# rustformers/llm

Hardware: AMD Instinct MI355X
Metric: decode tokens/s LLaMA-7B Q4_0 (higher is better)
Workload: dtype i8*i4->i32 block dots, f32 accumulate (W4A8 = ggml's Q4_0·Q8_0)

## Files before the change

### include/ggml_hip.h

```cpp
#ifndef GGML_HIP_H
#define GGML_HIP_H

#include <stdbool.h>
#include <stddef.h>
#include <stdint.h>

#ifdef __cplusplus
extern "C" {
#endif

#define GGML_API __attribute__((visibility("default")))

#define GGML_FILE_MAGIC 0x67676d6c
#define GGML_FILE_VERSION 1
#define GGML_QNT_VERSION 2
#define GGML_QNT_VERSION_FACTOR 1000
#define GGML_MAX_DIMS 4
#define GGML_MAX_NODES 4096
#define GGML_MAX_PARAMS 256
#define GGML_MAX_CONTEXTS 64
#define GGML_MAX_SRC 6
#define GGML_MAX_NAME 48
#define GGML_MAX_OP_PARAMS 32
#define GGML_DEFAULT_N_THREADS 4
// ... 358 lines not shown
GGML_API size_t ggml_hip_mul_mat_get_wsize(const struct ggml_tensor *src0, const struct ggml_tensor *src1,
                                           struct ggml_tensor *dst);
GGML_API void ggml_hip_mul_mat(const struct ggml_tensor *src0, const struct ggml_tensor *src1,
                               struct ggml_tensor *dst, void *wdata, size_t wsize);
GGML_API void *ggml_hip_host_malloc(size_t size);
GGML_API void ggml_hip_host_free(void *ptr);
GGML_API void ggml_hip_transform_tensor(void *data, struct ggml_tensor *tensor);
GGML_API void ggml_hip_free_data(struct ggml_tensor *tensor);
GGML_API void ggml_hip_assign_buffers(struct ggml_tensor *tensor);
GGML_API void ggml_hip_assign_buffers_no_scratch(struct ggml_tensor *tensor);
GGML_API void ggml_hip_assign_buffers_force_inplace(struct ggml_tensor *tensor);
GGML_API void ggml_hip_set_main_device(int main_device);
GGML_API void ggml_hip_set_mul_mat_q(bool mul_mat_q);
GGML_API void ggml_hip_set_scratch_size(size_t scratch_size);
GGML_API void ggml_hip_free_scratch(void);
GGML_API bool ggml_hip_compute_forward(struct ggml_compute_params *params, struct ggml_tensor *tensor);

GGML_API void ggml_init_cublas(void);
GGML_API void ggml_cuda_set_tensor_split(const float *tensor_split);
GGML_API void ggml_cuda_mul(const struct ggml_tensor *, const struct ggml_tensor *, struct ggml_tensor *);
GGML_API bool ggml_cuda_can_mul_mat(const struct ggml_tensor *, const struct ggml_tensor *, struct ggml_tensor *);
GGML_API size_t ggml_cuda_mul_mat_get_wsize(const struct ggml_tensor *, const struct ggml_tensor *,
                                            struct ggml_tensor *);
GGML_API void ggml_cuda_mul_mat(const struct ggml_tensor *, const struct ggml_tensor *, struct ggml_tensor *,
                                void *, size_t);
GGML_API void *ggml_cuda_host_malloc(size_t size);
GGML_API void ggml_cuda_host_free(void *ptr);
GGML_API void ggml_cuda_transform_tensor(void *data, struct ggml_tensor *tensor);
GGML_API void ggml_cuda_free_data(struct ggml_tensor *tensor);
GGML_API void ggml_cuda_assign_buffers(struct ggml_tensor *tensor);
GGML_API void ggml_cuda_assign_buffers_no_scratch(struct ggml_tensor *tensor);
GGML_API void ggml_cuda_assign_buffers_force_inplace(struct ggml_tensor *tensor);
GGML_API void ggml_cuda_set_main_device(int main_device);
GGML_API void ggml_cuda_set_mul_mat_q(bool mul_mat_q);
GGML_API void ggml_cuda_set_scratch_size(size_t scratch_size);
GGML_API void ggml_cuda_free_scratch(void);
GGML_API bool ggml_cuda_compute_forward(struct ggml_compute_params *params, struct ggml_tensor *tensor);

GGML_API int ggml_hip_device_count(void);
GGML_API int ggml_hip_slot_physical_device(int slot);
GGML_API int ggml_hip_thread_session_slot(void);
GGML_API int ggml_hip_get_main_device(void);
GGML_API void ggml_hip_bind_thread_device(int device);
GGML_API int ggml_hip_thread_pinned_device(void);
GGML_API void ggml_hip_unbind_thread_device(void);
GGML_API int ggml_hip_get_tensor_split(float *out, int cap);
GGML_API void ggml_hip_set_layer_split(const float *fractions, int n);
GGML_API int ggml_hip_get_layer_split(float *out, int cap);
GGML_API void ggml_hip_copy_between_devices(int dst_device, void *dst, int src_device, const void *src, size_t nbytes);
GGML_API void ggml_hip_synchronize(void);
GGML_API void ggml_hip_tensor_get(const struct ggml_tensor *tensor, void *host_dst, size_t offset, size_t nbytes);
GGML_API void ggml_hip_tensor_set(struct ggml_tensor *tensor, const void *host_src, size_t offset, size_t nbytes);
GGML_API void ggml_hip_memcpy(void *dst, const void *src, size_t nbytes, int kind);
GGML_API void *ggml_hip_tensor_device_ptr(const struct ggml_tensor *tensor);
enum ggml_hip_kclass {
    GGML_HIP_KCLASS_MMVQ = 0,
    GGML_HIP_KCLASS_MMQ_MFMA,
    GGML_HIP_KCLASS_ATTN,
    GGML_HIP_KCLASS_OTHER,
    GGML_HIP_KCLASS_COUNT
};
GGML_API void ggml_hip_timing_begin(void);
GGML_API void ggml_hip_timing_end(void);
GGML_API void ggml_hip_timing_query(int kclass, double *ms, int64_t *launches, double *algo_bytes);
GGML_API void ggml_hip_set_option(const char *key, int value);
GGML_API int ggml_hip_get_option(const char *key);
#define GGML_HIP_KKIND_BASE 16
GGML_API int ggml_hip_bench_plan_class(int kclass, int replays, double *ms_total, int64_t *launches_per_replay,
                                       double *algo_bytes_per_replay);
#define GGML_HIP_COMM_ID_BYTES 128
GGML_API int ggml_hip_comm_unique_id(void *id_out );
GGML_API int ggml_hip_comm_init(int rank, int world, const void *id);
GGML_API void ggml_hip_comm_destroy(void);
GGML_API int ggml_hip_comm_ranks(void);
GGML_API void ggml_hip_comm_send(const void *dev_src, size_t nbytes, int peer);
GGML_API void ggml_hip_comm_recv(void *dev_dst, size_t nbytes, int peer);
GGML_API void ggml_hip_comm_sendrecv(const void *dev_src, int send_peer, void *dev_dst, int recv_peer, size_t nbytes);
GGML_API int ggml_hip_bench_empty(int wgs, int threads, int lds_bytes, int kernarg_bytes, int n_launch, int replays,
                                  double *out);
GGML_API int64_t ggml_hip_get_stat(const char *key);
GGML_API int ggml_hip_graph_compute_begin(struct ggml_cgraph *cgraph);
GGML_API void ggml_hip_graph_compute_end(void);
GGML_API int ggml_hip_graph_prepare(struct ggml_cgraph *cgraph);
GGML_API int ggml_hip_decode_greedy_chain(struct ggml_cgraph *last, int n, int32_t *out_tokens, float *last_logits);
GGML_API int ggml_hip_decode_batch(struct ggml_cgraph *const *graphs, int n_graphs);
GGML_API int ggml_hip_topk(const struct ggml_tensor *t, int64_t row, int k, const int32_t *extra_ids, int n_extra,
                           float *out_vals, int32_t *out_ids);
GGML_API int ggml_hip_row_probs(const struct ggml_tensor *logits, int64_t row_begin, int64_t n_rows, const int32_t *targets,
                                float *out_probs);
GGML_API size_t ggml_hip_quantize(enum ggml_type type, const float *src, void *dst, int64_t n, int64_t k, int64_t *hist);
GGML_API int ggml_hip_quantize_resident(const struct ggml_tensor *src, struct ggml_tensor *dst, int64_t *hist);
GGML_API size_t ggml_hip_read_timeline(int64_t *dst, size_t max_records);
GGML_API int ggml_hip_debug_prompt_attention(const float *q, const uint16_t *mem_k, const uint16_t *mem_v, float *out, int N, int E,
                                             int Egqa, int H, int n_past, int64_t C, float scale, int fused);
GGML_API int ggml_hip_debug_prompt_attention_plan(const float *q_raw, const float *q_raw2, const float *rope, const uint16_t *mem_k,
                                                  const uint16_t *mem_v, uint16_t *x16, float *out, int N, int E, int Egqa, int H,
                                                  int n_past, int64_t C, float scale, int f16d);
GGML_API int ggml_hip_debug_exp_le0(uint16_t *out_fast, uint16_t *out_ref);
GGML_API int ggml_hip_debug_mul_mat_cols(const struct ggml_tensor *w, const float *x, float *out, int N);
GGML_API int ggml_hip_debug_mat_vec_big(const struct ggml_tensor *w0, const struct ggml_tensor *w1, const struct ggml_tensor *w2,
                                        int xsrc, int epi, const float *x, const float *norm_w, float eps, const float *res, float *out,
                                        float *y_out, int n_past, int D, float freq_base, float freq_scale, int64_t C,
                                        uint16_t *mem_k, uint16_t *mem_v);
GGML_API int ggml_hip_debug_mat_vec_kbig(const struct ggml_tensor *w0, const struct ggml_tensor *w1, const struct ggml_tensor *w2,
                                         int xsrc, int epi, const float *x, const float *xw, float eps, const float *res, float *out,
                                         float *y_out, int n_past, int D, float freq_base, float freq_scale, int64_t C,
                                         uint16_t *mem_k, uint16_t *mem_v);
GGML_API int ggml_hip_debug_mat_vec_f16(const struct ggml_tensor *w0, const struct ggml_tensor *w1, const struct ggml_tensor *w2,
                                        int xsrc, int epi, const float *x, const float *xw, float eps, const float *res, float *out,
                                        float *y_out, int n_past, int D, float freq_base, float freq_scale, int64_t C,
                                        uint16_t *mem_k, uint16_t *mem_v, int ncols);
GGML_API int ggml_hip_share_stream(int slot, int with_slot);
GGML_API const char *ggml_hip_version(void);

#ifdef __cplusplus
}
#endif

#ifdef __cplusplus
#define GGML_ABI_ASSERT(c, m) static_assert(c, m)
#else
#define GGML_ABI_ASSERT(c, m) _Static_assert(c, m)
#endif
GGML_ABI_ASSERT(sizeof(struct ggml_object) == 32, "ggml_object size (lib.rs:239)");
GGML_ABI_ASSERT(offsetof(struct ggml_object, type) == 24, "ggml_object.type");
GGML_ABI_ASSERT(sizeof(struct ggml_tensor) == 272, "ggml_tensor size (lib.rs:446)");
GGML_ABI_ASSERT(offsetof(struct ggml_tensor, ne) == 16, "ggml_tensor.ne");
GGML_ABI_ASSERT(offsetof(struct ggml_tensor, nb) == 48, "ggml_tensor.nb");
GGML_ABI_ASSERT(offsetof(struct ggml_tensor, op) == 80, "ggml_tensor.op");
GGML_ABI_ASSERT(offsetof(struct ggml_tensor, op_params) == 84, "ggml_tensor.op_params");
GGML_ABI_ASSERT(offsetof(struct ggml_tensor, is_param) == 116, "ggml_tensor.is_param");
GGML_ABI_ASSERT(offsetof(struct ggml_tensor, grad) == 120, "ggml_tensor.grad");
GGML_ABI_ASSERT(offsetof(struct ggml_tensor, src) == 128, "ggml_tensor.src");
GGML_ABI_ASSERT(offsetof(struct ggml_tensor, perf_runs) == 176, "ggml_tensor.perf_runs");
GGML_ABI_ASSERT(offsetof(struct ggml_tensor, data) == 200, "ggml_tensor.data");
GGML_ABI_ASSERT(offsetof(struct ggml_tensor, name) == 208, "ggml_tensor.name");
GGML_ABI_ASSERT(offsetof(struct ggml_tensor, extra) == 256, "ggml_tensor.extra");
GGML_ABI_ASSERT(offsetof(struct ggml_tensor, padding) == 264, "ggml_tensor.padding");
GGML_ABI_ASSERT(sizeof(struct ggml_cplan) == 16424, "ggml_cplan size");
GGML_ABI_ASSERT(offsetof(struct ggml_cplan, n_tasks) == 20, "ggml_cplan.n_tasks");
GGML_ABI_ASSERT(offsetof(struct ggml_cplan, abort_callback) == 16408, "ggml_cplan.abort_callback");
GGML_ABI_ASSERT(sizeof(struct ggml_cgraph) == 164520, "ggml_cgraph size (lib.rs:651)");
GGML_ABI_ASSERT(offsetof(struct ggml_cgraph, nodes) == 8, "ggml_cgraph.nodes");
GGML_ABI_ASSERT(offsetof(struct ggml_cgraph, leafs) == 65544, "ggml_cgraph.leafs");
GGML_ABI_ASSERT(offsetof(struct ggml_cgraph, visited_hash_table) == 98312, "ggml_cgraph.visited_hash_table");
GGML_ABI_ASSERT(offsetof(struct ggml_cgraph, perf_runs) == 164496, "ggml_cgraph.perf_runs");
GGML_ABI_ASSERT(sizeof(struct ggml_scratch) == 24, "ggml_scratch size");
GGML_ABI_ASSERT(sizeof(struct ggml_init_params) == 24, "ggml_init_params size");
GGML_ABI_ASSERT(sizeof(struct ggml_compute_params) == 32, "ggml_compute_params size");
GGML_ABI_ASSERT(offsetof(struct ggml_compute_params, wsize) == 16, "ggml_compute_params.wsize");
GGML_ABI_ASSERT(sizeof(ggml_type_traits_t) == 40, "ggml_type_traits_t size");

#endif
```

### llm_amd/csrc/backend_executor.inc

```
bool is_view_op(ggml_op op) {
    return op == GGML_OP_NONE || op == GGML_OP_RESHAPE || op == GGML_OP_VIEW || op == GGML_OP_PERMUTE ||
           op == GGML_OP_TRANSPOSE;
}

struct GraphInfo {
    std::vector<int> n_uses;
};

int node_index(const ggml_cgraph *gr, const ggml_tensor *t, const std::map<const ggml_tensor *, int> &idx) {
    (void)gr;
    auto it = idx.find(t);
    return it == idx.end() ? -1 : it->second;
}

void stage_add_target(ggml_tensor *leaf) {
    const uintptr_t p = (uintptr_t)leaf->data;
    const size_t nbytes = ggml_nbytes(leaf);
    for (const Staged &st : g_staged)
        if (st.host == p && st.nbytes == nbytes) return;
    bool offloaded = extra_of(leaf) != nullptr;
    for (auto &kv : g.tensors)
        if (kv.second->host < p + nbytes && p < kv.second->host + std::max<size_t>(kv.second->nbytes, 1)) offloaded = true;
    if (offloaded)
        die("add: tensor '%s' (%s) was offloaded to the device before being patched; LoRA adapters are applied at load time, "
// ... 31 lines not shown
                free_dev_tensor(e);
            } else {
                continue;
            }
        }
        Arena *hdr = find_arena((uintptr_t)leaf);
        const bool per_eval = r0 && hdr == r0;
        if (per_eval) {
            const size_t nbytes = ggml_nbytes(leaf);
            if (nbytes == 0) continue;
            h2d_small(dev_ptr(leaf), leaf->data, nbytes);
        } else {
            upload_tensor(leaf->data, leaf, false, true)->owner_hdr = (uintptr_t)leaf;
        }
    }
}

bool mirrored_to_host(const ggml_tensor *n) {
    if (n->backend != GGML_BACKEND_CPU || is_view_op(n->op) || n->op == GGML_OP_CPY) return false;
    if (!ggml_is_contiguous(n) || n->data == nullptr) return false;
    return !(extra_of(n) || find_tensor((uintptr_t)n->data));
}

static inline uint64_t now_ns() {
    return (uint64_t)std::chrono::duration_cast<std::chrono::nanoseconds>(
               std::chrono::steady_clock::now().time_since_epoch()).count();
}
void download_outputs(ggml_cgraph *gr) {
    const uint64_t t0 = now_ns();
    bool any = false;
    for (int i = 0; i < gr->n_nodes; i++) {
        ggml_tensor *n = gr->nodes[i];
        if (!mirrored_to_host(n)) continue;
        d2h_queue(n->data, dev_ptr(n), ggml_nbytes(n));
        g.stat_mirror_bytes += ggml_nbytes(n);
        any = true;
    }
    (void)any;
    d2h_finish();
    g.ns_mirror += now_ns() - t0;
}

void invalidate_xf16_if_overwritten_impl(const ggml_tensor *n);
void invalidate_qact_if_overwritten(const ggml_tensor *n) {
    if (g_xi8.valid && n->data != nullptr) {
        const uintptr_t c0 = (uintptr_t)g_xi8.src_data, c1 = c0 + g_xi8.src_bytes;
        const uintptr_t b0 = (uintptr_t)n->data, b1 = b0 + ggml_nbytes(n);
        if (b0 < c1 && c0 < b1) g_xi8.valid = false;
    }
    if (g_xk.valid && n->data != nullptr) {
        const uintptr_t c0 = (uintptr_t)g_xk.src_data, c1 = c0 + g_xk.src_bytes;
        const uintptr_t b0 = (uintptr_t)n->data, b1 = b0 + ggml_nbytes(n);
        if (b0 < c1 && c0 < b1) g_xk.valid = false;
    }
    invalidate_xf16_if_overwritten_impl(n);
    if (!g_qact.valid || n->data == nullptr) return;
    const uintptr_t a0 = (uintptr_t)g_qact.src_data, a1 = a0 + g_qact.src_bytes;
    const uintptr_t b0 = (uintptr_t)n->data, b1 = b0 + ggml_nbytes(n);
    if (b0 < a1 && a0 < b1) g_qact.valid = false;
}
void invalidate_xf16_if_overwritten_impl(const ggml_tensor *n) {
    if (!g_xf16.valid || n->data == nullptr) return;
    const uintptr_t a0 = (uintptr_t)g_xf16.src_data, a1 = a0 + g_xf16.src_bytes;
    const uintptr_t b0 = (uintptr_t)n->data, b1 = b0 + ggml_nbytes(n);
    if (b0 < a1 && a0 < b1) g_xf16.valid = false;
}

#include "plan_shapes.inc"
#include "plan_match.inc"
#include "plan_build.inc"
#include "plan_decode.inc"
#include "plan_prompt.inc"
#include "plan_run.inc"

void execute_graph(ggml_cgraph *gr) {
    ensure_init();
    finish_pending();
    ws_reset();
    g_qact.valid = false;
    g_xf16.valid = false;
    g_xi8.valid = false;
    g_xk.valid = false;
    if (try_decode_plan(gr)) return;
    g.stat_generic_graphs++;
    upload_inputs(gr);

    std::map<const ggml_tensor *, int> idx;
    std::vector<int> uses(gr->n_nodes, 0);
    for (int i = 0; i < gr->n_nodes; i++) idx[gr->nodes[i]] = i;
    for (int i = 0; i < gr->n_nodes; i++)
        for (int s = 0; s < GGML_MAX_SRC; s++)
            if (gr->nodes[i]->src[s]) {
                int j = node_index(gr, gr->nodes[i]->src[s], idx);
                if (j >= 0) uses[j]++;
            }
    std::vector<char> done(gr->n_nodes, 0);
    const bool fuse = g.opt_fuse != 0;
    std::vector<int> deferred_silu(gr->n_nodes, -1);
    if (fuse) {
        for (int j = 0; j < gr->n_nodes; j++) {
            ggml_tensor *mu = gr->nodes[j];
            if (mu->op != GGML_OP_MUL || !mu->src[0] || mu->src[0]->op != GGML_OP_UNARY) continue;
            const int i = node_index(gr, mu->src[0], idx);
            ggml_tensor *un = mu->src[0];
            if (i < 0 || i >= j || uses[i] != 1 || un->op_params[0] != GGML_UNARY_OP_SILU) continue;
            if (!is_contig_f32(un->src[0]) || !is_contig_f32(mu->src[1]) || !is_contig_f32(mu) ||
                ggml_nelements(mu->src[1]) != ggml_nelements(un) || ggml_nelements(mu) != ggml_nelements(un))
                continue;
            deferred_silu[i] = j;
        }
    }

    for (int i = 0; i < gr->n_nodes; i++) {
        ggml_tensor *n = gr->nodes[i];
        if (done[i] || is_view_op(n->op)) continue;
        invalidate_qact_if_overwritten(n);
        ggml_tensor *next = i + 1 < gr->n_nodes ? gr->nodes[i + 1] : nullptr;
        switch (n->op) {
            case GGML_OP_GET_ROWS: op_get_rows(n); break;
            case GGML_OP_RMS_NORM: {
                if (fuse && next && next->op == GGML_OP_MUL && next->src[0] == n && uses[i] == 1 && !done[i + 1] &&
                    is_contig_f32(next->src[1]) && ggml_nelements(next->src[1]) == n->ne[0] && next->nb[0] == 4) {
                    invalidate_qact_if_overwritten(next);
                    op_rms_norm(n, next->src[1], next);
                    done[i + 1] = 1;
                } else {
                    op_rms_norm(n, nullptr, n);
                }
            } break;
            case GGML_OP_NORM: op_norm(n); break;
            case GGML_OP_ADD: {
                if (n->src[0]->type == GGML_TYPE_F32)
                    op_bin(n, BIN_ADD);
                else
                    op_add_lowp(n);
            } break;
            case GGML_OP_MUL: {
                const int si = n->src[0] && n->src[0]->op == GGML_OP_UNARY ? node_index(gr, n->src[0], idx) : -1;
                if (si >= 0 && deferred_silu[si] == i)
                    op_unary(n->src[0], n->src[1], n);
                else
                    op_bin(n, BIN_MUL);
            } break;
            case GGML_OP_REPEAT: op_bin(n, BIN_REPEAT); break;
            case GGML_OP_UNARY: {
                if (deferred_silu[i] >= 0) break;
                if (fuse && n->op_params[0] == GGML_UNARY_OP_SILU && next && next->op == GGML_OP_MUL &&
                    next->src[0] == n && uses[i] == 1 && !done[i + 1] && is_contig_f32(next->src[1]) &&
                    ggml_nelements(next->src[1]) == ggml_nelements(n) && is_contig_f32(next)) {
                    invalidate_qact_if_overwritten(next);
                    op_unary(n, next->src[1], next);
                    done[i + 1] = 1;
                } else {
                    op_unary(n, nullptr, n);
                }
            } break;
            case GGML_OP_MUL_MAT: op_mul_mat(n); break;
            case GGML_OP_SCALE: {
                ggml_tensor *n1 = next, *n2 = i + 2 < gr->n_nodes ? gr->nodes[i + 2] : nullptr;
                ggml_tensor *n3 = i + 3 < gr->n_nodes ? gr->nodes[i + 3] : nullptr;
                if (fuse && n1 && n2 && n1->op == GGML_OP_DIAG_MASK_INF && n1->src[0] == n && n2->op == GGML_OP_SOFT_MAX &&
                    n2->src[0] == n1 && uses[i] == 1 && uses[i + 1] == 1 && n->data == n->src[0]->data &&
                    n1->data == n->data && n2->data == n->data && is_contig_f32(n)) {
                    op_scale_mask_softmax(n->src[0], n->src[1], (int)n1->op_params[0], n2);
                    done[i + 1] = done[i + 2] = 1;
                } else if (fuse && n1 && n2 && n3 && n1->op == GGML_OP_ALIBI && n1->src[0] == n &&
// ... 30 lines not shown
```

### llm_amd/csrc/backend_state.inc

```

[[noreturn]] void die(const char *fmt, ...) {
    char buf[1024];
    va_list ap;
    va_start(ap, fmt);
    vsnprintf(buf, sizeof(buf), fmt, ap);
    va_end(ap);
    fatal_note("%s", buf);
    abort();
}

int g_cur_slot();
struct Arena {
    uintptr_t base = 0;
    size_t size = 0;
    char *dev = nullptr;
    bool live = true;
    bool is_scratch = false;
};

struct DevTensor {
    uint32_t magic = 0x48495054;
    int slot = (int)(g_cur_slot());
    uintptr_t host = 0;
    size_t nbytes = 0;
    char *dev = nullptr;
    size_t dev_bytes = 0;
    bool soa = false;
    bool auto_uploaded = false;
    int refs = 1;
    bool zero_filled = false;
    uintptr_t owner_hdr = 0;
    QWeight qw{};
    char *w16 = nullptr;
    size_t w16_size = 0;
    bool ksoa = false;
    KWeight kw{};
    ggml_type type = GGML_TYPE_F32;
    int64_t ne[4] = {0, 0, 0, 0};
};

struct Timing {
    bool on = false;
    struct Rec {
        hipEvent_t a, b;
    };
    std::vector<Rec> recs[GGML_HIP_KCLASS_COUNT];
    std::vector<Rec> pool;
    double bytes[GGML_HIP_KCLASS_COUNT] = {0, 0, 0, 0};
    int64_t launches[GGML_HIP_KCLASS_COUNT] = {0, 0, 0, 0};
};

#define GGML_HIP_MAX_BACKENDS 16
struct Backend {
    int slot = 0;
    bool inited = false;
    int device = 0;
    hipStream_t stream = nullptr;
    hipStream_t own_stream = nullptr;
    std::recursive_mutex mu;
    hipEvent_t xfer_ev = nullptr;
    int opt_fuse_heads = 1, opt_attn_one = 1, opt_attn_split = 1;
    std::map<uintptr_t, Arena> arenas;
    std::map<uintptr_t, DevTensor *> tensors;
    std::map<uintptr_t, DevTensor *> auto_tensors;
    struct WsChunk {
        char *p;
        size_t size;
    };
    std::vector<WsChunk> ws_chunks;
    size_t ws_off = 0;
    Timing timing;
    int opt_fuse = 1, opt_plan = 1, opt_plan_k = 1, opt_plan_multi = 1, opt_plan_prompt = 1, opt_graph = 1, opt_big = 1, opt_kbig = 1;
    int opt_chain_k = 0, opt_prepare = 1, opt_plan_batch = 1, opt_plan_f16 = 1;
    int opt_fuse_attn = 1, opt_fuse_wo = 1, opt_warm_mb = 24, opt_affine = 1;
    int opt_act_quant = 0, opt_mmq_i8 = 0;
    int opt_mmq_min = 32, opt_k_prompt_min = 12, opt_mmq_fuse = 3, opt_mmq_cols = 1, opt_mmq_t256 = 1, opt_attn_fused = 1;
    int opt_mmq_w16 = 1, opt_w16_headroom_gb = 16;
    int opt_probe = 0;
    std::atomic<size_t> w16_bytes{0};
    uint64_t w16_gen = 1;
    int num_cus = 256;
    long long *timeline = nullptr;
    size_t timeline_bytes = 0;
    int timeline_wgs = 4;
    uint64_t stat_plan_tokens = 0, stat_generic_graphs = 0, stat_split_tokens = 0, stat_prompt_plan_tokens = 0, stat_fused_tokens = 0, stat_kplan_tokens = 0, stat_fused_heads_tokens = 0, stat_fused_wo_tokens = 0, stat_fused_affine_tokens = 0, stat_prepared_tokens = 0;
    uint64_t stat_alibi_fused = 0;
    uint64_t stat_batch_tokens = 0, stat_batch_steps = 0;
    uint64_t stat_flash_attn_nodes = 0;
    enum { MMQ_K_PLAIN, MMQ_K_DMA_P8, MMQ_K_W16_P8, MMQ_K_W16_256, MMQ_K_I8, MMQ_K_COUNT };
    uint64_t stat_mmq[MMQ_K_COUNT] = {0, 0, 0, 0, 0};
    void *chain_plan = nullptr;
    ggml_cgraph *chain_graph = nullptr;
    bool pending_wait = false;
    bool pending_light = false;
    int opt_speculate_next = 0;
    struct Spec {
        bool pending = false;
        void *plan = nullptr;
        int n_past = 0, av = 0;
        int32_t *tok_pin = nullptr;
        int *tok_dev = nullptr;
        hipEvent_t tok_ev = nullptr;
        int cooldown = 0;
    } spec;
    hipEvent_t results_ev = nullptr;
    bool results_ev_armed = false;
    size_t results_ev_copies = 0;
    uint64_t stat_spec_hits = 0, stat_spec_misses = 0;
    unsigned *ferr_pin = nullptr;
    void *ferr_plan = nullptr;
    int opt_fused_fallback = 1, opt_fused_rearm_tokens = 256;
    uint64_t fused_rearm_at = 0;
    uint64_t fused_rearm_stretch = 0;
    int fused_saved_fuse_attn = 0, fused_saved_attn_one = 0;
    uint64_t stat_fused_rearms = 0;
    uint64_t stat_cols_warm_launches = 0;
    int opt_test_fused_timeout = 0;
    uint64_t stat_fused_timeouts = 0;
    uint64_t ns_match = 0, ns_launch = 0, ns_wait = 0, ns_compute = 0, ns_mirror = 0, stat_mirror_bytes = 0;
    size_t dead_shadow_bytes = 0;
    uint64_t arena_seen = 0;
    void *prep = nullptr;
    int opt_gen = 0;
    int xcd_labels = -1;
    void *hot_line = nullptr;
    int session_records = 0;
};
enum : unsigned {
    OPT_ENV = 1,
    OPT_DROPS = 2,
    OPT_DEVICE = 4,
    OPT_ACTION = 8,
};
enum OptEffect { FX_NONE, FX_ACT_QUANT, FX_TIMELINE, FX_MMQ_W16, FX_W16_RELEASE, FX_FUSE_ATTN, FX_SPECULATE_NEXT, FX_FUSED_REARM_TOKENS, FX_TEST_FUSED_TIMEOUT, FX_SERIAL_STAGE_SLOTS };
struct OptRow {
    const char *key;
    int Backend::*field;
    unsigned flags;
    OptEffect fx = FX_NONE;
    int lo = 0, hi = -1;
};
static const OptRow g_options[] = {
    {"fuse", &Backend::opt_fuse, OPT_ENV},
    {"plan", &Backend::opt_plan, OPT_ENV},
    {"plan_k", &Backend::opt_plan_k, OPT_ENV | OPT_DROPS},
    {"plan_f16", &Backend::opt_plan_f16, OPT_ENV | OPT_DROPS},
    {"plan_multi", &Backend::opt_plan_multi, OPT_ENV | OPT_DROPS},
    {"plan_prompt", &Backend::opt_plan_prompt, OPT_ENV | OPT_DROPS},
    {"plan_batch", &Backend::opt_plan_batch, OPT_ENV | OPT_DROPS},
    {"graph", &Backend::opt_graph, OPT_ENV},
    {"big", &Backend::opt_big, OPT_ENV | OPT_DROPS},
    {"kbig", &Backend::opt_kbig, OPT_ENV | OPT_DROPS},
    {"chain_k", &Backend::opt_chain_k, OPT_ENV, FX_NONE, 0, 64},
    {"prepare", &Backend::opt_prepare, OPT_ENV},
    {"speculate_next", &Backend::opt_speculate_next, OPT_ENV, FX_SPECULATE_NEXT},
    {"fuse_attn", &Backend::opt_fuse_attn, OPT_ENV | OPT_DROPS, FX_FUSE_ATTN},
    {"fuse_wo", &Backend::opt_fuse_wo, OPT_ENV | OPT_DROPS},
    {"warm_mb", &Backend::opt_warm_mb, OPT_ENV | OPT_DROPS},
    {"affine", &Backend::opt_affine, OPT_ENV | OPT_DROPS},
    {"fuse_heads", &Backend::opt_fuse_heads, OPT_ENV | OPT_DROPS},
    {"attn_split", &Backend::opt_attn_split, OPT_ENV | OPT_DROPS},
    {"attn_one", &Backend::opt_attn_one, OPT_ENV | OPT_DROPS},
    {"fused_fallback", &Backend::opt_fused_fallback, OPT_ENV},
    {"fused_rearm_tokens", &Backend::opt_fused_rearm_tokens, OPT_ENV, FX_FUSED_REARM_TOKENS},
    {"act_quant", &Backend::opt_act_quant, OPT_ENV | OPT_DEVICE, FX_ACT_QUANT},
    {"mmq_i8", &Backend::opt_mmq_i8, OPT_ENV},
    {"mmq_min", &Backend::opt_mmq_min, OPT_ENV},
    {"k_prompt_min", &Backend::opt_k_prompt_min, OPT_ENV},
    {"mmq_fuse", &Backend::opt_mmq_fuse, OPT_ENV},
    {"mmq_cols", &Backend::opt_mmq_cols, OPT_ENV | OPT_DROPS},
    {"mmq_t256", &Backend::opt_mmq_t256, OPT_ENV | OPT_DROPS},
    {"attn_fused", &Backend::opt_attn_fused, OPT_ENV},
    {"mmq_w16", &Backend::opt_mmq_w16, OPT_ENV | OPT_DROPS | OPT_DEVICE, FX_MMQ_W16},
    {"w16_headroom_gb", &Backend::opt_w16_headroom_gb, OPT_ENV},
    {"w16_release", nullptr, OPT_DEVICE | OPT_ACTION, FX_W16_RELEASE},
    {"serial_stage_slots", nullptr, 0, FX_SERIAL_STAGE_SLOTS},
    {"timeline", nullptr, OPT_DEVICE, FX_TIMELINE},
    {"probe", &Backend::opt_probe, OPT_DROPS},
    {"test_fused_timeout", &Backend::opt_test_fused_timeout, OPT_DROPS, FX_TEST_FUSED_TIMEOUT},
};
const OptRow &opt_row(const char *key, const char *who) {
    for (const OptRow &o : g_options)
        if (!strcmp(o.key, key)) return o;
    die("%s: unknown key '%s'", who, key);
}
inline int opt_value(const OptRow &o, int v) {
    if (o.fx == FX_ACT_QUANT) return v ? 1 : 0;
    return o.lo <= o.hi ? std::min(o.hi, std::max(o.lo, v)) : v;
}
struct StatRow {
    const char *key;
    uint64_t Backend::*field;
};
static const StatRow g_counters[] = {
    {"plan_tokens", &Backend::stat_plan_tokens},
    {"fused_attn_tokens", &Backend::stat_fused_tokens},
    {"fused_heads_tokens", &Backend::stat_fused_heads_tokens},
    {"fused_wo_tokens", &Backend::stat_fused_wo_tokens},
    {"fused_affine_tokens", &Backend::stat_fused_affine_tokens},
    {"attn_split_tokens", &Backend::stat_split_tokens},
    {"kplan_tokens", &Backend::stat_kplan_tokens},
    {"prepared_tokens", &Backend::stat_prepared_tokens},
    {"prompt_plan_tokens", &Backend::stat_prompt_plan_tokens},
    {"batch_decode_tokens", &Backend::stat_batch_tokens},
    {"batch_decode_steps", &Backend::stat_batch_steps},
    {"cols_warm_launches", &Backend::stat_cols_warm_launches},
    {"fused_rearms", &Backend::stat_fused_rearms},
    {"spec_hits", &Backend::stat_spec_hits},
    {"spec_misses", &Backend::stat_spec_misses},
    {"generic_graphs", &Backend::stat_generic_graphs},
    {"alibi_fused", &Backend::stat_alibi_fused},
    {"flash_attn_nodes", &Backend::stat_flash_attn_nodes},
    {"ns_match", &Backend::ns_match},
    {"ns_launch", &Backend::ns_launch},
    {"ns_wait", &Backend::ns_wait},
    {"ns_compute", &Backend::ns_compute},
    {"ns_mirror", &Backend::ns_mirror},
    {"mirror_bytes", &Backend::stat_mirror_bytes},
};
std::recursive_mutex g_mu;
std::map<std::string, int> g_opt_log;
float g_tensor_split[GGML_HIP_MAX_BACKENDS] = {1.0f};
float g_layer_split[GGML_HIP_MAX_BACKENDS] = {0.0f};
int g_layer_split_n = 0;
Backend g_backends[GGML_HIP_MAX_BACKENDS];
std::atomic<int> g_default_slot{0};
std::atomic<int> g_dev_slots[64];
std::atomic<uint64_t> g_dev_gen[64];
std::atomic<uint64_t> g_dev_wgen[64];
thread_local Backend *g_cur = &g_backends[0];
thread_local bool tl_pinned = false;
#define g (*g_cur)
int g_cur_slot() { return (int)(g_cur - g_backends); }
std::atomic<int> g_dev_serial_stages[64];
inline int device_sharers() {
    const int n = g_dev_slots[g.device & 63].load(std::memory_order_relaxed), ser = g_dev_serial_stages[g.device & 63].load(std::memory_order_relaxed);
    return std::max(1, n - (ser > 1 ? std::min(ser, n) - 1 : 0));
}
inline int device_siblings() {
    int n = 0;
    for (int i = 0; i < GGML_HIP_MAX_BACKENDS; i++)
        if (&g_backends[i] != g_cur && g_backends[i].inited && g_backends[i].device == g.device) n++;
    return n;
}
void bind_device();
void sync_arenas();
std::atomic<int> g_calls_inside{0}, g_calls_inside_peak{0};
thread_local int tl_lock_depth = 0;
struct SlotLock {
    Backend *b;
    void enter() {
        b->mu.lock();
        if (tl_lock_depth++ == 0) {
            const int n = g_calls_inside.fetch_add(1, std::memory_order_relaxed) + 1;
            int peak = g_calls_inside_peak.load(std::memory_order_relaxed);
            while (n > peak && !g_calls_inside_peak.compare_exchange_weak(peak, n, std::memory_order_relaxed)) {}
        }
    }
    SlotLock() {
        if (!tl_pinned) g_cur = &g_backends[g_default_slot.load(std::memory_order_relaxed)];
        b = g_cur;
        enter();
        if (b->inited) bind_device();
        sync_arenas();
    }
    explicit SlotLock(Backend *slot) : b(slot) { enter(); }
    ~SlotLock() {
        if (--tl_lock_depth == 0) g_calls_inside.fetch_sub(1, std::memory_order_relaxed);
        b->mu.unlock();
    }
    SlotLock(const SlotLock &) = delete;
    SlotLock &operator=(const SlotLock &) = delete;
};
struct DevOnce {
    bool done[GGML_HIP_MAX_BACKENDS] = {};
    bool first() {
        bool &d = done[g.slot];
        if (d) return false;
        d = true;
        return true;
    }
};
template <auto Kern>
void lds_opt_in(size_t launch_lds, size_t max_bytes) {
    static DevOnce opted;
    if (launch_lds > 64 * 1024 && opted.first())
        HIP_CHECK(hipFuncSetAttribute((const void *)Kern, hipFuncAttributeMaxDynamicSharedMemorySize, (int)max_bytes));
}

int kt_of(ggml_type t) {
    switch (t) {
        case GGML_TYPE_Q2_K: return KT_Q2_K;
// ... 392 lines not shown
}

void h2d_bulk(char *dst, const void *src, size_t n) {
    staging_init();
    size_t off = 0;
    while (off < n) {
        const int b = stg.next;
        stg.next ^= 1;
        if (stg.busy[b]) {
            HIP_CHECK(hipEventSynchronize(stg.ev[b]));
            stg.busy[b] = false;
        }
        const size_t len = std::min(Staging::BIG, n - off);
        memcpy(stg.big[b], (const char *)src + off, len);
        HIP_CHECK(hipMemcpyAsync(dst + off, stg.big[b], len, hipMemcpyHostToDevice, g.stream));
        HIP_CHECK(hipEventRecord(stg.ev[b], g.stream));
        stg.busy[b] = true;
        off += len;
    }
}
void h2d_small(char *dst, const void *src, size_t n) {
    staging_init();
    const size_t need = (n + 63) & ~(size_t)63;
    if (stg.small_off + need > Staging::SMALL) {
        h2d_bulk(dst, src, n);
        return;
    }
    char *s = stg.small + stg.small_off;
    stg.small_off += need;
    memcpy(s, src, n);
    HIP_CHECK(hipMemcpyAsync(dst, s, n, hipMemcpyHostToDevice, g.stream));
}
void d2h_queue(void *host_dst, const char *src, size_t n) {
    staging_init();
    const size_t need = (n + 63) & ~(size_t)63;
    if (stg.small_off + need > Staging::SMALL) {
        const size_t PIECE = (size_t)8 << 20;
        for (int i = 0; i < 2; i++)
            if (stg.busy[i]) {
                HIP_CHECK(hipEventSynchronize(stg.ev[i]));
                stg.busy[i] = false;
            }
        auto par_copy = [](char *dst, const char *src_, size_t len) {
            const int nt = len >= ((size_t)2 << 20) ? 4 : 1;
            if (nt == 1) {
                memcpy(dst, src_, len);
                return;
            }
            std::thread th[3];
            const size_t part = (len / nt + 63) & ~(size_t)63;
            for (int t = 1; t < nt; t++) {
                const size_t o = (size_t)t * part;
                if (o < len) th[t - 1] = std::thread([=] { memcpy(dst + o, src_ + o, std::min(part, len - o)); });
            }
            memcpy(dst, src_, std::min(part, len));
            for (int t = 1; t < nt; t++)
                if (th[t - 1].joinable()) th[t - 1].join();
        };
        size_t off = 0;
        int cur = 0;
        size_t len = std::min(PIECE, n);
        HIP_CHECK(hipMemcpyAsync(stg.big[cur], src, len, hipMemcpyDeviceToHost, g.stream));
        HIP_CHECK(hipEventRecord(stg.ev[cur], g.stream));
        while (off < n) {
            const size_t noff = off + len, nlen = noff < n ? std::min(PIECE, n - noff) : 0;
            if (nlen) {
                HIP_CHECK(hipMemcpyAsync(stg.big[cur ^ 1], src + noff, nlen, hipMemcpyDeviceToHost, g.stream));
                HIP_CHECK(hipEventRecord(stg.ev[cur ^ 1], g.stream));
            }
            HIP_CHECK(hipEventSynchronize(stg.ev[cur]));
            par_copy((char *)host_dst + off, stg.big[cur], len);
            off = noff;
            len = nlen;
            cur ^= 1;
        }
        return;
    }
    char *s = stg.small + stg.small_off;
    stg.small_off += need;
    HIP_CHECK(hipMemcpyAsync(s, src, n, hipMemcpyDeviceToHost, g.stream));
    stg.pending.push_back({host_dst, s, n});
}
void d2h_finish() {
    if (g.results_ev_armed && stg.pending.size() != g.results_ev_copies) g.results_ev_armed = false;
    if (g.results_ev_armed) {
        g.results_ev_armed = false;
        HIP_CHECK(hipEventSynchronize(g.results_ev));
    } else {
        HIP_CHECK(hipStreamSynchronize(g.stream));
    }
    for (auto &p : stg.pending) memcpy(p.host_dst, p.stage, p.n);
    stg.pending.clear();
    stg.small_off = 0;
    stg.busy[0] = stg.busy[1] = false;
}

struct Timed {
    int k;
    Timing::Rec rec{};
    bool on;
    Timed(int kclass, double algo_bytes) : k(kclass), on(g.timing.on) {
        if (!on) return;
        if (!g.timing.pool.empty()) {
            rec = g.timing.pool.back();
            g.timing.pool.pop_back();
        } else {
            HIP_CHECK(hipEventCreate(&rec.a));
            HIP_CHECK(hipEventCreate(&rec.b));
        }
        HIP_CHECK(hipEventRecord(rec.a, g.stream));
        g.timing.bytes[k] += algo_bytes;
        g.timing.launches[k]++;
    }
    ~Timed() {
        if (!on) return;
        HIP_CHECK(hipEventRecord(rec.b, g.stream));
        g.timing.recs[k].push_back(rec);
    }
};

inline dim3 grid1(int64_t n, int bs = 256) { return dim3((unsigned)((n + bs - 1) / bs)); }
```

### llm_amd/csrc/backend_tools.inc

```
namespace {
template <int NARG>
struct EmptyArgs {
    long long *ts;
    int idx;
    int pad[(NARG - 12) / 4];
};
template <int NARG>
__global__ void __launch_bounds__(1024) k_empty(const EmptyArgs<NARG> a, int last_arg) {
    extern __shared__ __attribute__((aligned(16))) char smem[];
    long long t0;
    asm volatile("s_memrealtime %0\n\ts_waitcnt lgkmcnt(0)" : "=s"(t0));
    const int v = a.pad[(NARG - 12) / 4 - 1] + last_arg;
    long long t1 = v != 0x7fffffff ? (long long)wall_clock64() : 0;
    if (v == 0x12345678) smem[threadIdx.x] = 1;
    if (threadIdx.x == 0 && blockIdx.x == 0) {
        a.ts[a.idx * 4] = t0;
        a.ts[a.idx * 4 + 1] = t1;
        a.ts[a.idx * 4 + 2] = (long long)wall_clock64();
    }
}
template <int NARG>
void empty_launch(int wgs, int threads, int lds, long long *ts, int idx) {
    EmptyArgs<NARG> a;
    memset(&a, 0, sizeof(a));
// ... 403 lines not shown
        qa.rope = rope; qa.prm = prm; qa.mem_k = (__half *)dk; qa.mem_v = (__half *)dv; qa.Egqa = Ms[1]; qa.C = C; qa.D = D;
        float *ds3[3] = {(float *)dout, nullptr, nullptr};
        const int kinds[3] = {0, 1, 2};
        launch_f16(3, fw, ds3, K, src, nullptr, ncols, KE_QKV, &qa, kinds);
    } else if (epi == KE_GATE) {
        float *ds2[2] = {(float *)dout, nullptr};
        launch_f16(2, fw, ds2, K, src, nullptr, ncols, KE_GATE);
    } else if (nw == 1) {
        float *ds1[1] = {(float *)dout};
        launch_f16(1, fw, ds1, K, src, (const float *)dres, ncols);
    } else {
        float *ds[3] = {nullptr, nullptr, nullptr};
        for (int i = 0; i < nw; i++) ds[i] = (float *)debug_buf((size_t)ncols * Ms[i] * 4, nullptr, owned);
        launch_f16(nw, fw, ds, K, src, nullptr, ncols);
        int64_t at = 0;
        for (int i = 0; i < nw; i++) {
            HIP_CHECK(hipMemcpy2DAsync(dout + at * 4, (size_t)Mrow * 4, ds[i], (size_t)Ms[i] * 4, (size_t)Ms[i] * 4, (size_t)ncols, hipMemcpyDeviceToDevice, g.stream));
            at += Ms[i];
        }
    }
    if (dy && epi != KE_ROW) {
        float *ds1[1] = {(float *)debug_buf((size_t)ncols * Ms[0] * 4, nullptr, owned)};
        launch_f16(1, fw, ds1, K, RowSrc{KX_NORM, (const float *)dx, (const float *)dxw, eps, (float *)dy}, nullptr, ncols);
    }
    d2h_queue(out, dout, n_out + DEBUG_GUARD);
    if (dy) d2h_queue(y_out, dy, nx + DEBUG_GUARD);
    if (dk) {
        d2h_queue(mem_k, dk, nkv + DEBUG_GUARD);
        d2h_queue(mem_v, dv, nkv + DEBUG_GUARD);
    }
    d2h_finish();
    for (char *b : owned) HIP_CHECK(hipFree(b));
    return 0;
}

int ggml_hip_debug_prompt_attention_plan(const float *q_raw, const float *q_raw2, const float *rope, const uint16_t *mem_k,
                                         const uint16_t *mem_v, uint16_t *x16, float *out, int N, int E, int Egqa, int H, int n_past,
                                         int64_t C, float scale, int f16d) {
    SlotLock lk;
    ensure_init();
    finish_pending();
    if (!q_raw || !rope || !mem_k || !mem_v || !x16 || N < 1 || H < 1 || E % H || n_past < 0) return -1;
    const int64_t D = E / H, T = (int64_t)n_past + N;
    if (Egqa < D || Egqa % D || H % (Egqa / D) || T > C || C % 8 || !prompt_attn_fits(D, T)) return -1;
    const int64_t Hkv = Egqa / D;
    std::vector<char *> owned;
    const size_t nq = (size_t)N * E * 4, nkv = (size_t)C * Egqa * 2, nx = (size_t)N * E * 2;
    char *dq = debug_buf(nq * (q_raw2 ? 2 : 1), nullptr, owned);
    h2d_bulk(dq, q_raw, nq);
    if (q_raw2) h2d_bulk(dq + nq, q_raw2, nq);
    char *dr = debug_buf((size_t)N * 128 * 4, rope, owned);
    char *dk = debug_buf(nkv, mem_k, owned), *dv = debug_buf(nkv, mem_v, owned);
    char *dx = debug_buf(nx, nullptr, owned), *dout = debug_buf(nq, nullptr, owned);
    prompt_attention(true, (const float *)dq, (const __half *)dk, (const __half *)dv, (float *)dout, nullptr, nullptr, N, E, Egqa, H, Hkv,
                     D, n_past, C, scale, (_Float16 *)dx, f16d != 0, (const float *)dr, q_raw2 ? (int64_t)N * E : 0);
    d2h_queue(x16, dx, nx + DEBUG_GUARD);
    if (out) d2h_queue(out, dout, nq + DEBUG_GUARD);
    d2h_finish();
    for (char *b : owned) HIP_CHECK(hipFree(b));
    return 0;
}

__global__ void __launch_bounds__(256) k_debug_exp_le0(uint16_t *out_fast, uint16_t *out_ref) {
    const unsigned i = blockIdx.x * 256 + threadIdx.x;
    const float x = __half2float(__ushort_as_half((unsigned short)i));
    out_fast[i] = __half_as_ushort(__float2half_rn(exp_le0(x)));
    out_ref[i] = __half_as_ushort(__float2half_rn(expf(x)));
}
int ggml_hip_debug_exp_le0(uint16_t *out_fast, uint16_t *out_ref) {
    SlotLock lk;
    ensure_init();
    finish_pending();
    uint16_t *d;
    dev_malloc((void **)&d, 2 * 65536 * 2, "debug exp");
    hipLaunchKernelGGL(k_debug_exp_le0, dim3(256), dim3(256), 0, g.stream, d, d + 65536);
    HIP_CHECK(hipGetLastError());
    HIP_CHECK(hipStreamSynchronize(g.stream));
    HIP_CHECK(hipMemcpy(out_fast, d, 65536 * 2, hipMemcpyDeviceToHost));
    HIP_CHECK(hipMemcpy(out_ref, d + 65536, 65536 * 2, hipMemcpyDeviceToHost));
    HIP_CHECK(hipFree(d));
    return 0;
}

int ggml_hip_decode_greedy_chain(struct ggml_cgraph *last, int n, int32_t *out_tokens, float *last_logits) {
    SlotLock lk;
    return decode_greedy_chain(last, n, out_tokens, last_logits);
}

int ggml_hip_decode_batch(struct ggml_cgraph *const *graphs, int n_graphs) {
    if (!graphs || n_graphs < 2 || n_graphs > BATCH_COLS_MAX) return -1;
    for (int i = 0; i < n_graphs; i++)
        if (!graphs[i]) return -1;
    SlotLock lk;
    const uint64_t t0 = now_ns();
    const int r = decode_batch(graphs, n_graphs);
    g.ns_compute += now_ns() - t0;
    return r;
}

int64_t ggml_hip_get_stat(const char *key) {
    SlotLock lk;
    for (const StatRow &c : g_counters)
        if (!strcmp(c.key, key)) return (int64_t)(g.*c.field);
    const std::string k(key);
    if (k == "w16_bytes") return (int64_t)g.w16_bytes;
    if (k.rfind("mmq_launches_", 0) == 0) {
        static const char *names[Backend::MMQ_K_COUNT] = {"plain", "dma_p8", "w16_p8", "w16_256", "i8"};
        for (int i = 0; i < Backend::MMQ_K_COUNT; i++)
            if (k.substr(13) == names[i]) return (int64_t)g.stat_mmq[i];
        return -1;
    }
    if (k == "graph_replays") {
        int64_t n = 0;
        for (auto *p : g_plans) n += (int64_t)p->replays;
        return n;
    }
    if (k == "plans") return (int64_t)g_plans.size();
    if (k == "num_cus") {
        ensure_init();
        return (int64_t)g.num_cus;
    }
    if (k == "fused_attn_timeouts") {
        int64_t n = (int64_t)g.stat_fused_timeouts;
        if (g.inited) HIP_CHECK(hipStreamSynchronize(g.stream));
        if (g.ferr_pin) n += *(volatile unsigned *)g.ferr_pin;
        return n;
    }
    if (k == "peak_concurrent_calls") return (int64_t)g_calls_inside_peak.load();
    return -1;
}
size_t ggml_hip_read_timeline(int64_t *dst, size_t max_records) {
    SlotLock lk;
    if (!g.timeline) return 0;
    const size_t n = std::min(max_records, g.timeline_bytes / 64);
    HIP_CHECK(hipStreamSynchronize(g.stream));
    HIP_CHECK(hipMemcpy(dst, g.timeline, n * 64, hipMemcpyDeviceToHost));
    return n;
}
const char *ggml_hip_version(void) { return "libggml_hip 0.1 (gfx950)"; }

}
```

### llm_amd/csrc/hip_backend.hip

```cpp
#include <hip/hip_runtime.h>

#include <algorithm>
#include <atomic>
#include <cctype>
#include <chrono>
#include <cmath>
#include <cstdarg>
#include <cstdio>
#include <cstdlib>
#include <cstring>
#include <deque>
#include <map>
#include <mutex>
#include <string>
#include <thread>
#include <vector>

#include "ggml_hip.h"
#include "internal.h"
#include "kernels/common.h"
#include "kernels/mmvq.h"
#include "kernels/mmq.h"
#include "kernels/mmq_plain.h"
#include "kernels/mmq_dmap8.h"
// ... 71 lines not shown
        DevTensor *e = it->second;
        it = g.auto_tensors.erase(it);
        destroy_record(e);
    }
}
void register_arena_here(void *host_base, size_t size, int is_scratch) {
    const uintptr_t b = (uintptr_t)host_base;
    if (size == 0) return;
    auto it = g.arenas.find(b);
    if (it != g.arenas.end() && it->second.size == size) {
        if (!it->second.live && it->second.dev) g.dead_shadow_bytes -= it->second.size;
        if (!it->second.live) evict_overlapping(g.auto_tensors, b, size);
        it->second.live = true;
        return;
    }
    for (auto jt = g.arenas.begin(); jt != g.arenas.end();) {
        Arena &a = jt->second;
        if (a.base < b + size && b < a.base + a.size) {
            if (a.dev) {
                if (g.stream) HIP_CHECK(hipStreamSynchronize(g.stream));
                HIP_CHECK(hipFree(a.dev));
                if (!a.live) g.dead_shadow_bytes -= a.size;
            }
            jt = g.arenas.erase(jt);
        } else {
            ++jt;
        }
    }
    evict_overlapping(g.auto_tensors, b, size);
    Arena a;
    a.base = b;
    a.size = size;
    a.is_scratch = is_scratch != 0;
    g.arenas[b] = a;
}

void unregister_arena_here(void *host_base) {
    const uintptr_t b = (uintptr_t)host_base;
    auto it = g.arenas.find(b);
    if (it == g.arenas.end()) return;
    Arena &a = it->second;
    evict_overlapping(g.auto_tensors, a.base, a.size);
    for (auto jt = g.auto_tensors.begin(); jt != g.auto_tensors.end();) {
        DevTensor *e = jt->second;
        if (e->owner_hdr >= a.base && e->owner_hdr < a.base + a.size) {
            jt = g.auto_tensors.erase(jt);
            destroy_record(e);
        } else {
            ++jt;
        }
    }
    a.live = false;
    if (a.dev) {
        g.dead_shadow_bytes += a.size;
        if (g.dead_shadow_bytes > ((size_t)8 << 30)) {
            if (g.stream) HIP_CHECK(hipStreamSynchronize(g.stream));
            for (auto jt = g.arenas.begin(); jt != g.arenas.end();) {
                if (!jt->second.live) {
                    if (jt->second.dev) HIP_CHECK(hipFree(jt->second.dev));
                    jt = g.arenas.erase(jt);
                } else {
                    ++jt;
                }
            }
            g.dead_shadow_bytes = 0;
        }
    } else {
        g.arenas.erase(it);
    }
}

}

extern "C" void ggml_hip_internal_graph_compute(struct ggml_cgraph *cgraph) {
    SlotLock lk;
    const uint64_t t0 = now_ns();
    execute_graph(cgraph);
    g.ns_compute += now_ns() - t0;
}
extern "C" int ggml_hip_graph_compute_begin(struct ggml_cgraph *cgraph) {
    SlotLock lk;
    const uint64_t t0 = now_ns();
    ensure_init();
    if (g.pending_wait && g.pending_light && stg.pending.empty() && !g.results_ev_armed) {
        g.pending_wait = false;
        g.ferr_plan = nullptr;
    } else {
        finish_pending();
    }
    ws_reset();
    g_qact.valid = false;
    g_xf16.valid = false;
    g_xi8.valid = false;
    g_xk.valid = false;
    int async = 0;
    if (try_decode_plan(cgraph, true)) {
        async = 1;
    } else {
        execute_graph(cgraph);
    }
    g.ns_compute += now_ns() - t0;
    return async;
}
extern "C" int ggml_hip_graph_prepare(struct ggml_cgraph *cgraph) {
    SlotLock lk;
    ensure_init();
    return prepare_decode_plan(cgraph) ? 1 : 0;
}
extern "C" void ggml_hip_graph_compute_end(void) {
    SlotLock lk;
    const uint64_t t0 = now_ns();
    finish_pending();
    g.ns_compute += now_ns() - t0;
}

extern "C" {

void ggml_init_hipblas(void) {
    SlotLock lk;
    ensure_init();
}
void ggml_hip_set_main_device(int main_device) {
    if (main_device < 0 || main_device >= std::max(1, slot_count()))
        die("ggml_hip_set_main_device(%d): %d device slot(s) available", main_device, slot_count());
    g_default_slot.store(main_device, std::memory_order_relaxed);
    if (tl_auto_slot >= 0 && slot_physical_device(tl_auto_slot) == slot_physical_device(main_device)) {
        ggml_hip_bind_thread_device(tl_auto_slot);
        return;
    }
    ggml_hip_bind_thread_device(main_device);
}
static void auto_session_slot() {
    const int n = std::min(session_slots_env(), slot_count());
    if (n <= 1 || tl_auto_slot >= 0) return;
    if (!tl_pinned) g_cur = &g_backends[g_default_slot.load(std::memory_order_relaxed)];
    const int cur = (int)(g_cur - g_backends), phys = slot_physical_device(cur);
    int best = cur;
    {
        std::lock_guard<std::recursive_mutex> lk(g_mu);
        for (int i = 0; i < n; i++)
            if (slot_physical_device(i) == phys && g_session_threads[i] < g_session_threads[best]) best = i;
        g_session_threads[best]++;
        tl_auto_slot = best;
        (void)&tl_auto_release;
    }
    if (best != cur) ggml_hip_bind_thread_device(best);
    else tl_pinned = true, g_cur = &g_backends[cur];
}
int ggml_hip_thread_session_slot(void) { return tl_auto_slot; }
void ggml_hip_bind_thread_device(int device) {
    if (device < 0 || device >= std::max(1, slot_count()))
        die("ggml_hip_bind_thread_device(%d): %d device slot(s) available", device, slot_count());
    tl_pinned = true;
    g_cur = &g_backends[device];
    SlotLock lk(g_cur);
    g.slot = device;
    if (g.inited) bind_device();
}
int ggml_hip_thread_pinned_device(void) { return tl_pinned ? (int)(g_cur - g_backends) : -1; }
void ggml_hip_unbind_thread_device(void) {
    tl_pinned = false;
    g_cur = &g_backends[g_default_slot.load(std::memory_order_relaxed)];
}
void ggml_hip_set_tensor_split(const float *tensor_split) {
    std::lock_guard<std::recursive_mutex> lk(g_mu);
    for (int i = 0; i < GGML_HIP_MAX_BACKENDS; i++) g_tensor_split[i] = 0.0f;
    g_tensor_split[0] = tensor_split ? tensor_split[0] : 0.0f;
}
int ggml_hip_get_tensor_split(float *out, int cap) {
    std::lock_guard<std::recursive_mutex> lk(g_mu);
    const int n = std::min(cap, GGML_HIP_MAX_BACKENDS);
    for (int i = 0; i < n; i++) out[i] = g_tensor_split[i];
    return std::min(n, 1);
}
void ggml_hip_set_layer_split(const float *fractions, int n) {
    std::lock_guard<std::recursive_mutex> lk(g_mu);
    g_layer_split_n = fractions && n > 0 ? std::min(n, GGML_HIP_MAX_BACKENDS) : 0;
    for (int i = 0; i < GGML_HIP_MAX_BACKENDS; i++) g_layer_split[i] = i < g_layer_split_n ? fractions[i] : 0.0f;
}
int ggml_hip_get_layer_split(float *out, int cap) {
    std::lock_guard<std::recursive_mutex> lk(g_mu);
    const int n = std::min(cap, g_layer_split_n);
    for (int i = 0; i < n; i++) out[i] = g_layer_split[i];
    return n;
}
void ggml_hip_set_mul_mat_q(bool) {}
void ggml_hip_set_scratch_size(size_t) {}
void ggml_hip_free_scratch(void) {
    SlotLock lk;
    if (!g.inited) return;
// ... 82 lines not shown
    const int64_t cap = std::min(nblocks, piece);
    dev_malloc((void **)&din, (size_t)cap * qk * 4, "the quantizer input");
    dev_malloc((void **)&dout, (size_t)cap * bs, "the quantizer output");
    HIP_CHECK(hipMalloc((void **)&dh, 128));
    HIP_CHECK(hipMemsetAsync(dh, 0, 128, g.stream));
    for (int64_t b0 = 0; b0 < nblocks; b0 += piece) {
        const int64_t nb = std::min(piece, nblocks - b0);
        h2d_bulk(din, src + b0 * qk, (size_t)nb * qk * 4);
        if (kt >= 0)
            launch_quantize_k(din, false, kt, nb, (uint8_t *)dout);
        else
            launch_quantize_blocks(din, false, (int)type, nb, (uint8_t *)dout, dh);
        d2h_queue((char *)dst + (size_t)b0 * bs, dout, (size_t)nb * bs);
        d2h_finish();
    }
    unsigned long long hh[16];
    HIP_CHECK(hipMemcpy(hh, dh, 128, hipMemcpyDeviceToHost));
    if (hist)
        for (int i = 0; i < 16; i++) hist[i] += (int64_t)hh[i];
    HIP_CHECK(hipFree(din));
    HIP_CHECK(hipFree(dout));
    HIP_CHECK(hipFree(dh));
    return (size_t)nblocks * bs;
}
int ggml_hip_quantize_resident(const struct ggml_tensor *src, struct ggml_tensor *dst, int64_t *hist) {
    SlotLock lk;
    ensure_init();
    if (!quantizable(dst->type) || (src->type != GGML_TYPE_F32 && src->type != GGML_TYPE_F16)) return -1;
    if (!ggml_is_contiguous(src) || src->ne[2] != 1 || src->ne[3] != 1 || src->ne[0] % 32 != 0 || src->ne[0] != dst->ne[0] ||
        src->ne[1] != dst->ne[1] || dst->ne[2] != 1 || dst->ne[3] != 1 || extra_of(dst) || dst->data == nullptr)
        return -1;
    if (!extra_of(src) && !find_tensor((uintptr_t)src->data)) return -1;
    finish_pending();
    const int64_t M = src->ne[1], nb = src->ne[0] / 32, nblocks = M * nb;
    const size_t bs = ggml_type_size(dst->type);
    char *raw = nullptr;
    unsigned long long *dh = nullptr;
    dev_malloc((void **)&raw, (size_t)nblocks * bs, "the resident quantizer output");
    HIP_CHECK(hipMalloc((void **)&dh, 128));
    HIP_CHECK(hipMemsetAsync(dh, 0, 128, g.stream));
    launch_quantize_blocks(dev_ptr(src), src->type == GGML_TYPE_F16, (int)dst->type, nblocks, (uint8_t *)raw, dh);
    DevTensor *e = new DevTensor();
    e->host = (uintptr_t)dst->data;
    e->nbytes = ggml_nbytes(dst);
    e->type = dst->type;
    for (int i = 0; i < 4; i++) e->ne[i] = dst->ne[i];
    const int qt = qt_of(dst->type);
    size_t off[5];
    const size_t total = qw_layout(qt, M, nb, off);
    dev_malloc((void **)&e->dev, total, "a weight tensor");
    e->dev_bytes = total;
    relayout_launch(raw, qt, M, nb, e->dev);
    unsigned long long hh[16];
    HIP_CHECK(hipMemcpyAsync(hh, dh, 128, hipMemcpyDeviceToHost, g.stream));
    HIP_CHECK(hipStreamSynchronize(g.stream));
    if (hist)
        for (int i = 0; i < 16; i++) hist[i] += (int64_t)hh[i];
    HIP_CHECK(hipFree(raw));
    HIP_CHECK(hipFree(dh));
    e->soa = true;
    e->qw = qw_at(e->dev, qt, M, nb);
    evict_overlapping(g.auto_tensors, e->host, std::max<size_t>(e->nbytes, 1));
    evict_overlapping(g.tensors, e->host, std::max<size_t>(e->nbytes, 1));
    g.tensors[e->host] = e;
    dst->backend = GGML_BACKEND_GPU;
    dst->extra = e;
    return 0;
}

int ggml_hip_topk(const struct ggml_tensor *t, int64_t row, int k, const int32_t *extra_ids, int n_extra, float *out_vals,
                  int32_t *out_ids) {
    SlotLock lk;
    ensure_init();
    if (!t || t->type != GGML_TYPE_F32 || t->nb[0] != 4 || row < 0 || row >= t->ne[1] * t->ne[2] * t->ne[3] || t->ne[2] != 1 ||
        t->ne[3] != 1 || k < 1 || k > TOPK_MAX || k > t->ne[0] || n_extra < 0 || t->ne[0] > 0x7FFFFFFF || !out_vals || !out_ids ||
        (n_extra > 0 && !extra_ids) || t->data == nullptr)
        return -1;
    {
        DevTensor *e = extra_of(t);
        if (!e) e = find_tensor((uintptr_t)t->data);
        if (e ? e->soa : find_arena((uintptr_t)t->data) == nullptr) return -1;
    }
    finish_pending();
    const float *x = (const float *)(dev_ptr(t) + row * (int64_t)t->nb[1]);
    char *buf = ws_alloc((size_t)(k + n_extra) * 8 + (size_t)n_extra * 4 + 64);
    float *dv = (float *)buf;
    int *di = (int *)(buf + (size_t)(k + n_extra) * 4);
    int *de = di + (k + n_extra);
    if (n_extra) h2d_small((char *)de, extra_ids, (size_t)n_extra * 4);
    {
        Timed tm(GGML_HIP_KCLASS_OTHER, (double)t->ne[0] * 4 * 9);
        hipLaunchKernelGGL(k_topk, dim3(1), dim3(1024), 0, g.stream, x, (int)t->ne[0], k, (const int *)de, n_extra, dv, di);
        HIP_CHECK(hipGetLastError());
    }
    d2h_queue(out_vals, (const char *)dv, (size_t)(k + n_extra) * 4);
    d2h_queue(out_ids, (const char *)di, (size_t)(k + n_extra) * 4);
    d2h_finish();
    return 0;
}

int ggml_hip_row_probs(const struct ggml_tensor *t, int64_t row_begin, int64_t n_rows, const int32_t *targets, float *out_probs) {
    if (!t || !targets || !out_probs || n_rows < 1 || row_begin < 0 || t->type != GGML_TYPE_F32 || t->nb[0] != 4 || t->ne[2] != 1 ||
        t->ne[3] != 1 || t->ne[0] < 1 || t->ne[0] > (1 << 30) || n_rows > t->ne[1] || row_begin > t->ne[1] - n_rows ||
        n_rows > 0x7FFFFFFF || t->nb[1] % 4 != 0 || t->nb[1] < (size_t)t->ne[0] * 4 || t->data == nullptr)
        return -1;
    for (int64_t r = 0; r < n_rows; r++)
        if (targets[r] < 0 || targets[r] >= t->ne[0]) return -1;
    SlotLock lk;
    ensure_init();
    {
        DevTensor *e = extra_of(t);
        if (!e) e = find_tensor((uintptr_t)t->data);
        if (e ? e->soa : find_arena((uintptr_t)t->data) == nullptr) return -1;
    }
    finish_pending();
    const float *x = (const float *)(dev_ptr(t) + row_begin * (int64_t)t->nb[1]);
    const int V = (int)t->ne[0];
    char *buf = ws_alloc((size_t)n_rows * 8 + 64);
    float *dp = (float *)buf;
    int *dt = (int *)(buf + (size_t)n_rows * 4);
    h2d_small((char *)dt, targets, (size_t)n_rows * 4);
    {
        Timed tm(GGML_HIP_KCLASS_OTHER, (double)n_rows * V * 4);
        const long long stride = (long long)(t->nb[1] / 4);
        const bool keep = V <= ROW_PROB_KEEP * 1024, vec = keep && V % 4 == 0 && stride % 4 == 0 && (uintptr_t)x % 16 == 0;
        auto kern = vec ? k_row_prob<true, true> : keep ? k_row_prob<true, false> : k_row_prob<false, false>;
        hipLaunchKernelGGL(kern, dim3((unsigned)n_rows), dim3(1024), 0, g.stream, x, stride, V, (const int *)dt, dp);
        HIP_CHECK(hipGetLastError());
    }
    d2h_queue(out_probs, (const char *)dp, (size_t)n_rows * 4);
    d2h_finish();
    return 0;
}

void ggml_hip_free_data(struct ggml_tensor *tensor) {
    if (!tensor || !tensor->extra) return;
    DevTensor *e = (DevTensor *)tensor->extra;
    if (e->magic != 0x48495054) return;
    const int owner = (e->slot >= 0 && e->slot < GGML_HIP_MAX_BACKENDS) ? e->slot : g_cur_slot();
    SlotLock lk(&g_backends[owner]);
    free_dev_tensor(e);
    tensor->extra = nullptr;
}
void ggml_hip_assign_buffers(struct ggml_tensor *tensor) {
    tensor->backend = GGML_BACKEND_GPU;
}
void ggml_hip_assign_buffers_force_inplace(struct ggml_tensor *tensor) { tensor->backend = GGML_BACKEND_GPU; }
void ggml_hip_assign_buffers_no_scratch(struct ggml_tensor *tensor) {
    if (tensor->op == GGML_OP_NONE && !tensor->extra) auto_session_slot();
    SlotLock lk;
    tensor->backend = GGML_BACKEND_GPU;
    if (tensor->op != GGML_OP_NONE || extra_of(tensor)) return;
    tensor->extra = upload_tensor(tensor->data, tensor, true);
}
bool ggml_hip_can_mul_mat(const struct ggml_tensor *src0, const struct ggml_tensor *src1, struct ggml_tensor *dst) {
    bool q = src0->type == GGML_TYPE_F16 || src0->type == GGML_TYPE_F32;
    if (qt_of(src0->type) >= 0) q = src0->ne[0] % 32 == 0;
    if (kt_of(src0->type) >= 0) q = src0->ne[0] % 256 == 0;
    return q && src1->type == GGML_TYPE_F32 && dst->type == GGML_TYPE_F32;
}
size_t ggml_hip_mul_mat_get_wsize(const struct ggml_tensor *, const struct ggml_tensor *, struct ggml_tensor *) {
    return 0;
}
void ggml_hip_mul_mat(const struct ggml_tensor *src0, const struct ggml_tensor *src1, struct ggml_tensor *dst, void *,
                      size_t) {
    SlotLock lk;
    ensure_init();
    BK_ASSERT(dst->src[0] == src0 && dst->src[1] == src1);
    op_mul_mat(dst);
}
void ggml_hip_mul(const struct ggml_tensor *src0, const struct ggml_tensor *src1, struct ggml_tensor *dst) {
    SlotLock lk;
    ensure_init();
    BK_ASSERT(dst->src[0] == src0 && dst->src[1] == src1);
    op_bin(dst, BIN_MUL);
}
bool ggml_hip_compute_forward(struct ggml_compute_params *params, struct ggml_tensor *tensor) {
    SlotLock lk;
    if (params && (params->ith != 0 || params->type != GGML_TASK_COMPUTE)) return true;
    ensure_init();
    ggml_cgraph *gr = (ggml_cgraph *)calloc(1, sizeof(ggml_cgraph));
    gr->nodes[0] = tensor;
    gr->n_nodes = 1;
    execute_graph(gr);
    free(gr);
    return true;
}

void ggml_init_cublas(void) { ggml_init_hipblas(); }
void ggml_cuda_set_tensor_split(const float *s) { ggml_hip_set_tensor_split(s); }
void ggml_cuda_mul(const struct ggml_tensor *a, const struct ggml_tensor *b, struct ggml_tensor *d) { ggml_hip_mul(a, b, d); }
bool ggml_cuda_can_mul_mat(const struct ggml_tensor *a, const struct ggml_tensor *b, struct ggml_tensor *d) {
    return ggml_hip_can_mul_mat(a, b, d);
}
size_t ggml_cuda_mul_mat_get_wsize(const struct ggml_tensor *a, const struct ggml_tensor *b, struct ggml_tensor *d) {
    return ggml_hip_mul_mat_get_wsize(a, b, d);
}
void ggml_cuda_mul_mat(const struct ggml_tensor *a, const struct ggml_tensor *b, struct ggml_tensor *d, void *w, size_t s) {
    ggml_hip_mul_mat(a, b, d, w, s);
// ... 13 lines not shown

int ggml_hip_device_count(void) { return slot_count(); }
int ggml_hip_slot_physical_device(int slot) {
    return slot < 0 || slot >= slot_count() ? -1 : slot_physical_device(slot);
}
int ggml_hip_get_main_device(void) {
    if (!tl_pinned) g_cur = &g_backends[g_default_slot.load(std::memory_order_relaxed)];
    return (int)(g_cur - g_backends);
}
void ggml_hip_copy_between_devices(int dst_device, void *dst, int src_device, const void *src, size_t nbytes) {
    if (dst_device < 0 || src_device < 0 || dst_device >= GGML_HIP_MAX_BACKENDS || src_device >= GGML_HIP_MAX_BACKENDS)
        die("ggml_hip_copy_between_devices: bad slot");
    Backend &S = g_backends[src_device], &D = g_backends[dst_device];
    SlotLock lk_a(&g_backends[std::min(src_device, dst_device)]);
    SlotLock lk_b(&g_backends[std::max(src_device, dst_device)]);
    if (!S.inited || !D.inited) die("ggml_hip_copy_between_devices: slot not initialised");
    Backend *keep = g_cur;
    g_cur = &S;
    bind_device();
    if (S.stream != D.stream) {
        if (!S.xfer_ev) HIP_CHECK(hipEventCreateWithFlags(&S.xfer_ev, hipEventDisableTiming));
        HIP_CHECK(hipEventRecord(S.xfer_ev, S.stream));
    }
    g_cur = &D;
    bind_device();
    if (S.stream != D.stream) HIP_CHECK(hipStreamWaitEvent(D.stream, S.xfer_ev, 0));
    if (S.device == D.device)
        HIP_CHECK(hipMemcpyAsync(dst, src, nbytes, hipMemcpyDeviceToDevice, D.stream));
    else {
        static bool peer_tried[GGML_HIP_MAX_BACKENDS][GGML_HIP_MAX_BACKENDS];
        if (!peer_tried[dst_device][src_device]) {
            peer_tried[dst_device][src_device] = true;
            int can = 0;
            if (hipDeviceCanAccessPeer(&can, D.device, S.device) == hipSuccess && can) {
                const hipError_t e = hipDeviceEnablePeerAccess(S.device, 0);
                if (e != hipSuccess && e != hipErrorPeerAccessAlreadyEnabled)
                    fprintf(stderr, "ggml-hip: peer access %d -> %d not enabled (%s): copies go through the host\n", D.device, S.device,
                            hipGetErrorString(e));
            }
            (void)hipGetLastError();
        }
        HIP_CHECK(hipMemcpyPeerAsync(dst, D.device, src, S.device, nbytes, D.stream));
    }
    g_cur = keep;
    if (g.inited) bind_device();
}
int ggml_hip_share_stream(int slot, int with_slot) {
    if (slot < 0 || slot >= GGML_HIP_MAX_BACKENDS || with_slot >= GGML_HIP_MAX_BACKENDS) die("ggml_hip_share_stream: bad slot");
    Backend &B = g_backends[slot];
    if (with_slot < 0 || with_slot == slot) {
        SlotLock lk(&B);
        if (!B.own_stream) return 0;
        Backend *keep = g_cur;
        g_cur = &B;
        bind_device();
        HIP_CHECK(hipStreamSynchronize(B.stream));
        B.stream = B.own_stream;
        B.own_stream = nullptr;
        g_cur = keep;
        if (g.inited) bind_device();
        return 0;
    }
    Backend &A = g_backends[with_slot];
    SlotLock lk_a(&g_backends[std::min(slot, with_slot)]);
    SlotLock lk_b(&g_backends[std::max(slot, with_slot)]);
    if (!A.inited || !B.inited || A.device != B.device || B.own_stream || A.own_stream) return 0;
    Backend *keep = g_cur;
    g_cur = &B;
    bind_device();
    HIP_CHECK(hipStreamSynchronize(B.stream));
    B.own_stream = B.stream;
    B.stream = A.stream;
    g_cur = keep;
    if (g.inited) bind_device();
    return 1;
}
void ggml_hip_synchronize(void) {
    SlotLock lk;
    if (g.inited) HIP_CHECK(hipStreamSynchronize(g.stream));
}
void ggml_hip_tensor_get(const struct ggml_tensor *tensor, void *host_dst, size_t offset, size_t nbytes) {
    SlotLock lk;
    ensure_init();
    d2h_queue(host_dst, dev_ptr(tensor) + offset, nbytes);
    d2h_finish();
}
void ggml_hip_tensor_set(struct ggml_tensor *tensor, const void *host_src, size_t offset, size_t nbytes) {
    SlotLock lk;
    ensure_init();
    h2d_bulk(dev_ptr(tensor) + offset, host_src, nbytes);
    HIP_CHECK(hipStreamSynchronize(g.stream));
}
void ggml_hip_memcpy(void *dst, const void *src, size_t nbytes, int kind) {
    SlotLock lk;
    ensure_init();
    if (kind == 0) {
        h2d_bulk((char *)dst, src, nbytes);
        HIP_CHECK(hipStreamSynchronize(g.stream));
    } else if (kind == 1) {
        d2h_queue(dst, (const char *)src, nbytes);
        d2h_finish();
    } else {
        HIP_CHECK(hipMemcpyAsync(dst, src, nbytes, hipMemcpyDeviceToDevice, g.stream));
        HIP_CHECK(hipStreamSynchronize(g.stream));
    }
}
void *ggml_hip_tensor_device_ptr(const struct ggml_tensor *tensor) {
    SlotLock lk;
    ensure_init();
    return dev_ptr(tensor);
}
void ggml_hip_timing_begin(void) {
    SlotLock lk;
    ensure_init();
    HIP_CHECK(hipStreamSynchronize(g.stream));
    for (int k = 0; k < GGML_HIP_KCLASS_COUNT; k++) {
        for (auto &r : g.timing.recs[k]) g.timing.pool.push_back(r);
        g.timing.recs[k].clear();
        g.timing.bytes[k] = 0;
        g.timing.launches[k] = 0;
    }
    g.timing.on = true;
}
void ggml_hip_timing_end(void) {
    SlotLock lk;
    g.timing.on = false;
    if (g.inited) HIP_CHECK(hipStreamSynchronize(g.stream));
}
void ggml_hip_timing_query(int kclass, double *ms, int64_t *launches, double *algo_bytes) {
    SlotLock lk;
    double total = 0;
    if (kclass >= 0 && kclass < GGML_HIP_KCLASS_COUNT) {
        for (auto &r : g.timing.recs[kclass]) {
            float t = 0;
            HIP_CHECK(hipEventElapsedTime(&t, r.a, r.b));
            total += t;
        }
        if (ms) *ms = total;
        if (launches) *launches = g.timing.launches[kclass];
        if (algo_bytes) *algo_bytes = g.timing.bytes[kclass];
    }
}
void ggml_hip_set_option(const char *key, int value) {
    const OptRow &o = opt_row(key, "ggml_hip_set_option");
    if (!(o.flags & OPT_ACTION)) {
        std::lock_guard<std::recursive_mutex> lk(g_mu);
        g_opt_log[key] = opt_value(o, value);
    }
    for_each_slot([&] {
        if (g.inited) ggml_hip_internal_set_option_here(key, value);
    });
}
void ggml_hip_internal_set_option_here(const char *key, int value) {
    const OptRow &o = opt_row(key, "ggml_hip_set_option");
    if ((o.flags & OPT_DEVICE) && !g.inited) return;
    g.opt_gen++;
    value = opt_value(o, value);
    if (o.fx == FX_SPECULATE_NEXT) spec_cancel();
    if (o.field) {
        if ((o.flags & OPT_DROPS) && g.*o.field != value) drop_all_plans();
        g.*o.field = value;
    }
    switch (o.fx) {
        case FX_ACT_QUANT: apply_act_quant(); break;
        case FX_TIMELINE:
            drop_all_plans();
            if (g.timeline && value && (value == 1 ? 4 : value) != g.timeline_wgs) {
                HIP_CHECK(hipStreamSynchronize(g.stream));
                (void)hipFree(g.timeline);
                g.timeline = nullptr;
            }
            if (value && !g.timeline) {
                g.timeline_wgs = value == 1 ? 4 : value;
                g.timeline_bytes = (size_t)1024 * g.timeline_wgs * 8 * 8;
                HIP_CHECK(hipMalloc((void **)&g.timeline, g.timeline_bytes));
            }
            if (!value && g.timeline) {
                HIP_CHECK(hipStreamSynchronize(g.stream));
// ... 98 lines not shown
```

### llm_amd/csrc/host/llm_host.cpp

```cpp
#if defined(__x86_64__)
#include <immintrin.h>
#endif
#include "llm_host.h"

#include <algorithm>
#include <atomic>
#include <chrono>
#include <fcntl.h>
#include <sys/mman.h>
#include <sys/stat.h>
#include <unistd.h>

#include <cmath>
#include <cstring>
#include <functional>
#include <map>
#include <set>
#include <string>
#include <thread>
#include <vector>

#include "ggml_wrap.hpp"

using ggml::Backend;
using ggml::Buffer;
using ggml::ComputationGraph;
using ggml::Context;
using ggml::GraphExecutionPlan;
using ggml::Tensor;

namespace llm {

using TokenId = int32_t;

struct ModelParameters {
    size_t context_size = 2048;
    bool use_gpu = false;
    long gpu_layers = -1;
    bool has_rope_overrides = false;
    ggml::RoPEOverrides rope_overrides;
    long n_gqa = -1;
    size_t layer_begin = 0, layer_end = (size_t)-1;
    int main_device = -1;

    bool should_offload(size_t layer) const {
        if (!use_gpu) return false;
        return gpu_layers < 0 ? true : (long)layer < gpu_layers;
    }
    Backend backend(size_t layer) const { return should_offload(layer) ? Backend::Gpu : Backend::Cpu; }
};

struct InferenceSessionConfig {
    ggml::Type memory_k_type = GGML_TYPE_F16;
    ggml::Type memory_v_type = GGML_TYPE_F16;
    size_t n_batch = 8;
    size_t n_threads = 8;
};

struct OutputRequest {
    std::vector<float> *all_logits = nullptr;
    std::vector<float> *embeddings = nullptr;
    bool logits_on_device = false;
    bool intermediate_chunk = false;
};

struct GraphOutputs {
    Tensor result;
    Tensor embedding_result;
};

constexpr size_t SCRATCH_SIZE = 512ull * 1024 * 1024;

struct BuildContext {
    Context *ctx0;
    const Tensor *embd;
    const Tensor *memory_k;
    const Tensor *memory_v;
    const std::shared_ptr<Buffer> *scratch;
    const Buffer *get_scratch(size_t idx) const { return scratch[idx].get(); }
};

class InferenceSession {
   public:
    InferenceSession(const InferenceSessionConfig &config, const ModelParameters &params, size_t n_layer,
                     size_t n_embd, size_t n_vocab)
        : config(config), n_embd_(n_embd) {
        const size_t context_size = params.context_size;
        const size_t context_byte_size = [&] {
            double size = 0;
            size += (double)context_size * (double)n_layer * (double)n_embd * (double)ggml_type_sizef(config.memory_k_type);
            size += (double)context_size * (double)n_layer * (double)n_embd * (double)ggml_type_sizef(config.memory_v_type);
            return (size_t)size + (5 + 10 * n_layer) * 256;
        }();
        if (params.use_gpu) {
            if (params.main_device < 0) ggml::accelerator::initialize(0);
            ggml::accelerator::set_scratch_size(config.n_batch * 1024 * 1024);
        }
        session_ctx_ = std::make_shared<Context>(Context::new_with_allocate(context_byte_size));
        memory_size_ = context_byte_size;
        const size_t n_mem = n_layer * context_size;
        const size_t n_elements = n_embd * n_mem;
        memory_k = session_ctx_->new_tensor_1d(config.memory_k_type, n_elements).set_name("memory_k");
        memory_v = session_ctx_->new_tensor_1d(config.memory_v_type, n_elements).set_name("memory_v");
        if (params.use_gpu) {
            memory_k.offload_no_scratch();
            memory_v.offload_no_scratch();
        }
        scratch_[0] = std::make_shared<Buffer>(SCRATCH_SIZE);
        scratch_[1] = std::make_shared<Buffer>(SCRATCH_SIZE);
        const size_t buf_size_mb = n_layer >= 80 ? 1536 : n_layer >= 60 ? 1280 : 1024;
        const size_t buf_size = buf_size_mb * 1024 * 1024 + ggml_graph_overhead();
        ctx0_[0] = Context::new_with_buffer(std::make_shared<Buffer>(buf_size));
        ctx0_[1] = Context::new_with_buffer(std::make_shared<Buffer>(buf_size));
        if (const char *v = getenv("LLM_HOST_SPECULATE")) speculate = atoi(v) != 0;
        last_logits.assign(n_vocab, 0.0f);
    }
    ~InferenceSession() {
        ggml::accelerator::free_scratch();
    }

    using Builder = std::function<std::pair<ComputationGraph, GraphOutputs>(BuildContext &)>;
    static inline std::atomic<int64_t> host_ns[8] = {};
    static inline void host_ns_add(int k, double ns) { host_ns[k].fetch_add((int64_t)ns, std::memory_order_relaxed); }
    static inline double now_ns() {
        return (double)std::chrono::duration_cast<std::chrono::nanoseconds>(std::chrono::steady_clock::now().time_since_epoch()).count();
    }

    GraphOutputs compute(const std::vector<TokenId> &input_tokens, const Builder &builder,
                         const std::function<Builder(size_t )> &next_builder = nullptr,
                         const void *model_key = nullptr, size_t context_size = 0) {
        const bool single = input_tokens.size() == 1;
        double t0 = now_ns(), t1;
        auto lap = [&](int k) { t1 = now_ns(); host_ns_add(k, t1 - t0); t0 = t1; };
        Built built;
        if (single && pre_.valid && pre_.n_past == n_past && pre_.model_key == model_key) {
            cur_ = pre_.slot;
            built = std::move(pre_.b);
        } else {
            cur_ ^= 1;
            built = build_into(cur_, input_tokens.size(), builder);
        }
        pre_.valid = false;
        lap(0);
        Context &ctx0 = ctx0_[cur_];
        built.embd.write_data(input_tokens.data(), input_tokens.size() * sizeof(TokenId));
        {
// ... 295 lines not shown
                              .set_name("KQV_merged_contiguous");
                current = ctx0.op_mul_mat(layers[il].wo, current);
                ctx0.use_scratch(builder.get_scratch(1));
                Tensor input_feed_forward = ctx0.op_add(current, input_self_attention);
                current = ctx0.op_rms_norm(input_feed_forward);
                current = ctx0.op_mul(current, layers[il].ffn_norm);
                Tensor tmp = ctx0.op_mul_mat(layers[il].w3, current);
                current = ctx0.op_mul_mat(layers[il].w1, current);
                current = ctx0.op_silu(current);
                current = ctx0.op_mul(current, tmp);
                current = ctx0.op_mul_mat(layers[il].w2, current);
                current = ctx0.op_add(current, input_feed_forward);
                input_layer = current;
            }
            if (!is_last()) {
                ctx0.use_scratch(nullptr);
                Tensor out = ctx0.op_cpy(input_layer, ctx0.op_view_1d(session.stage_out, n_embd * input_len, 0));
                return std::make_pair(gf, GraphOutputs{out, out});
            }
            ctx0.use_scratch(builder.get_scratch(0));
            input_layer = ctx0.op_rms_norm(input_layer);
            input_layer = ctx0.op_mul(input_layer, norm);
            Tensor embedding_result = input_layer.share();
            ctx0.set_offloading(logits_on_device && params.use_gpu);
            input_layer = ctx0.op_mul_mat(output, input_layer);
            ctx0.use_scratch(nullptr);
            return std::make_pair(gf, GraphOutputs{input_layer, embedding_result});
        };
    }

    void evaluate(InferenceSession &session, const std::vector<TokenId> &input_tokens, OutputRequest &output_request) {
        const size_t input_len = input_tokens.size();
        const size_t session_len = session.n_past;
        const size_t ctx_size = params.context_size;
        const size_t n_vocab = hyperparameters.n_vocab, n_embd = hyperparameters.n_embd;

        InferenceSession *sp = &session;
        GraphOutputs outputs = session.compute(
            input_tokens, make_builder(sp, input_len, session_len, (input_len > 1 && !output_request.all_logits) || output_request.logits_on_device),
            [this, sp](size_t next_len) { return make_builder(sp, 1, next_len); }, this, ctx_size);
        if (!is_last()) return;
        if (output_request.intermediate_chunk) return;
        if (!output_request.logits_on_device) common::read_last_token(session, outputs.result, n_vocab, input_len);
        common::extract_logits(output_request, outputs.result, n_vocab, input_len);
        common::extract_embeddings(output_request, outputs.embedding_result, n_embd, input_len);
    }

    ggml_cgraph *stage_single(InferenceSession &session, TokenId tok, GraphOutputs &out) {
        return session.stage_single(tok, make_builder(&session, 1, session.n_past), out);
    }
    void finish_single(InferenceSession &session, ggml_cgraph *gr, const GraphOutputs &out) {
        session.commit_single(gr);
        common::read_last_token(session, out.result, hyperparameters.n_vocab, 1);
    }

    Hyperparameters hyperparameters;
    ModelParameters params;
    Tensor wte, norm, output;
    std::vector<Layer> layers;
    std::shared_ptr<Context> context;
};

}

struct llm_ggml_file;
struct llm_model {
    llm::Llama *llama;
    llm_ggml_file *file = nullptr;
    std::vector<llm::Llama *> stages;
    std::vector<int> devices;
    int device = ggml_hip_get_main_device();
};
struct llm_session {
    llm::InferenceSession *s;
    std::vector<llm::InferenceSession *> stage_sessions;
    bool shares_streams = false;
    std::vector<int> devices;
    int device = 0;
    const llm_model *model = nullptr;
};

namespace {
std::atomic<int> g_split_sessions{0};
struct HomeDevice {
    int pinned = ggml_hip_thread_pinned_device();
    int home = ggml_hip_get_main_device();
    void go(int d) const {
        if (ggml_hip_get_main_device() != d) ggml_hip_bind_thread_device(d);
    }
    ~HomeDevice() {
        if (pinned < 0)
            ggml_hip_unbind_thread_device();
        else
            go(home);
    }
};
bool may_pipeline_chunk(const llm_model *m, size_t len) {
    static const bool pipeline_on = !(getenv("LLM_HOST_PIPELINE_CHUNKS") && atoi(getenv("LLM_HOST_PIPELINE_CHUNKS")) == 0);
    return pipeline_on && m->stages.empty() && len > 1;
}
void model_evaluate(llm_model *m, llm_session *s, const std::vector<llm::TokenId> &toks, llm::OutputRequest &req) {
    HomeDevice hd;
    if (m->stages.empty()) {
        hd.go(s->device);
        if (!m->llama->is_first() || !m->llama->is_last())
            s->s->ensure_stage_rows(m->llama->hyperparameters.n_embd, toks.size());
        m->llama->evaluate(*s->s, toks, req);
        return;
    }
    const size_t G = m->stages.size();
    const size_t hop_bytes = (size_t)m->llama->hyperparameters.n_embd * toks.size() * sizeof(float);
    for (size_t i = 0; i < G; i++) {
        hd.go(m->devices[i]);
        s->stage_sessions[i]->ensure_stage_rows(m->llama->hyperparameters.n_embd, toks.size());
    }
    for (size_t i = 0; i < G; i++) {
        ggml_hip_bind_thread_device(m->devices[i]);
        llm::InferenceSession &ss = *s->stage_sessions[i];
        if (i > 0) {
            void *dst = ggml_hip_tensor_device_ptr(ss.stage_in.ptr());
            ggml_hip_bind_thread_device(m->devices[i - 1]);
            const void *src = ggml_hip_tensor_device_ptr(s->stage_sessions[i - 1]->stage_out.ptr());
            ggml_hip_copy_between_devices(m->devices[i], dst, m->devices[i - 1], src, hop_bytes);
            ggml_hip_bind_thread_device(m->devices[i]);
        }
        llm::OutputRequest none;
        m->stages[i]->evaluate(ss, toks, i + 1 == G ? req : none);
    }
}
std::vector<size_t> split_layers(size_t n_layer, int G, const float *split) {
    std::vector<double> w(G, 1.0);
    double sum = 0;
    bool any = false;
    for (int i = 0; i < G; i++) any = any || (split && split[i] > 0.0f);
    for (int i = 0; i < G; i++) {
        if (any) w[i] = std::max(0.0f, split[i]);
        sum += w[i];
    }
    std::vector<size_t> bounds(G + 1, 0);
    double acc = 0;
    for (int i = 0; i < G; i++) {
        acc += w[i];
        size_t b = (size_t)std::llround(acc / sum * (double)n_layer);
        b = std::max(b, bounds[i] + 1);
        b = std::min(b, n_layer - (size_t)(G - 1 - i));
        bounds[i + 1] = b;
    }
    bounds[G] = n_layer;
    return bounds;
}
}

extern "C" {

llm_model *llm_llama_new(const llm_llama_hparams *hp, const llm_model_params *mp, const llm_tensor_desc *tensors,
                         int n_tensors) {
    llm::Hyperparameters h;
    h.n_vocab = hp->n_vocab;
    h.n_embd = hp->n_embd;
    h.n_mult = hp->n_mult;
    h.n_head = hp->n_head;
    h.n_head_kv = hp->n_head_kv > 0 ? hp->n_head_kv : hp->n_head;
    h.n_layer = hp->n_layer;
    h.n_rot = hp->n_rot;
    h.file_type = hp->file_type;
    if (mp->n_gqa > 0 && h.n_layer >= 80) {
        if (h.n_head % (size_t)mp->n_gqa != 0) ggml::panic("assuming 70B Llama2 model based on GQA == 8");
        h.n_head_kv = h.n_head / (size_t)mp->n_gqa;
    }
    llm::ModelParameters p;
    p.context_size = mp->context_size > 0 ? mp->context_size : 2048;
    p.use_gpu = mp->use_gpu != 0;
    p.gpu_layers = mp->gpu_layers;
    p.has_rope_overrides = mp->has_rope_overrides != 0;
    p.rope_overrides.frequency_scale = mp->rope_frequency_scale;
    p.rope_overrides.frequency_base = (size_t)mp->rope_frequency_base;
    p.layer_begin = mp->layer_begin > 0 ? (size_t)mp->layer_begin : 0;
    p.layer_end = mp->layer_end > 0 ? (size_t)mp->layer_end : (size_t)-1;
    if (!p.use_gpu) {
        fprintf(stderr, "llm_llama_new: use_gpu=0 requested, but libggml_hip has no CPU compute path\n");
        abort();
    }
    std::vector<int> slots;
    std::vector<float> shares;
    {
        float split[16] = {0};
        const int nslot = std::min(ggml_hip_get_layer_split(split, 16), ggml_hip_device_count());
// ... 503 lines not shown
        delete s->s;
    }
    delete s;
}
void llm_evaluate(llm_model *m, llm_session *s, const int32_t *tokens, int n, float *all_logits, float *embeddings) {
    std::vector<llm::TokenId> toks(tokens, tokens + n);
    std::vector<float> logits, emb;
    llm::OutputRequest req;
    if (all_logits) req.all_logits = &logits;
    if (embeddings) req.embeddings = &emb;
    model_evaluate(m, s, toks, req);
    if (all_logits) memcpy(all_logits, logits.data(), logits.size() * sizeof(float));
    if (embeddings) memcpy(embeddings, emb.data(), emb.size() * sizeof(float));
}
void llm_feed_prompt(llm_model *m, llm_session *s, const int32_t *tokens, int n) {
    if (s->s->n_past + (size_t)n >= m->llama->params.context_size) {
        fprintf(stderr, "llm_feed_prompt: InferenceError::ContextFull\n");
        abort();
    }
    const size_t nb = s->s->config.n_batch;
    for (size_t i = 0; i < (size_t)n; i += nb) {
        const size_t len = std::min(nb, (size_t)n - i);
        std::vector<llm::TokenId> batch(tokens + i, tokens + i + len);
        llm::OutputRequest req;
        const bool more = i + len < (size_t)n && may_pipeline_chunk(m, len);
        req.intermediate_chunk = more;
        s->s->pipeline_chunk = more;
        model_evaluate(m, s, batch, req);
        s->s->pipeline_chunk = false;
        for (auto tk : batch) s->s->tokens.push_back(tk);
    }
}
static size_t argmax_first_scalar(const float *l, size_t n) {
    size_t best = 0;
    for (size_t i = 1; i < n; i++)
        if (l[i] > l[best]) best = i;
    return best;
}
#if defined(__x86_64__)
__attribute__((target("avx2"))) static size_t argmax_first_avx2(const float *l, size_t n) {
    if (n < 16) return argmax_first_scalar(l, n);
    __m256 mx = _mm256_set1_ps(l[0]);
    size_t i = 0;
    for (; i + 8 <= n; i += 8) {
        const __m256 v = _mm256_loadu_ps(l + i);
        mx = _mm256_blendv_ps(mx, v, _mm256_cmp_ps(v, mx, _CMP_GT_OQ));
    }
    float lanes[8];
    _mm256_storeu_ps(lanes, mx);
    float m = l[0];
    for (int k = 0; k < 8; k++) m = lanes[k] > m ? lanes[k] : m;
    for (; i < n; i++) m = l[i] > m ? l[i] : m;
    if (!(m == m)) return 0;
    const __m256 mv = _mm256_set1_ps(m);
    for (i = 0; i + 8 <= n; i += 8) {
        const int mask = _mm256_movemask_ps(_mm256_cmp_ps(_mm256_loadu_ps(l + i), mv, _CMP_EQ_OQ));
        if (mask) return i + (size_t)__builtin_ctz((unsigned)mask);
    }
    for (; i < n; i++)
        if (l[i] == m) return i;
    return 0;
}
#endif
static size_t argmax_first(const float *l, size_t n) {
#if defined(__x86_64__)
    static const bool have_avx2 = __builtin_cpu_supports("avx2");
    if (have_avx2) return argmax_first_avx2(l, n);
#endif
    return argmax_first_scalar(l, n);
}
int llm_argmax_first(const float *l, int n, int which) { return (int)(which ? argmax_first_scalar(l, (size_t)n) : argmax_first(l, (size_t)n)); }

int32_t llm_infer_next_token_greedy(llm_model *m, llm_session *s) {
    if (s->s->n_past + 1 >= m->llama->params.context_size) {
        fprintf(stderr, "llm_infer_next_token: InferenceError::ContextFull\n");
        abort();
    }
    const double t0 = llm::InferenceSession::now_ns();
    const std::vector<float> &l = s->s->last_logits;
    const llm::TokenId next = (llm::TokenId)argmax_first(l.data(), l.size());
    s->s->tokens.push_back(next);
    llm::OutputRequest req;
    const double t1 = llm::InferenceSession::now_ns();
    model_evaluate(m, s, std::vector<llm::TokenId>{next}, req);
    llm::InferenceSession::host_ns_add(5, t1 - t0);
    llm::InferenceSession::host_ns_add(6, llm::InferenceSession::now_ns() - t1);
    return next;
}
int32_t llm_infer_next_token_topk(llm_model *m, llm_session *s, int k, float temperature, uint64_t *rng, int device_topk) {
    if (s->s->n_past + 1 >= m->llama->params.context_size) {
        fprintf(stderr, "llm_infer_next_token_topk: InferenceError::ContextFull\n");
        abort();
    }
    const size_t V = s->s->last_logits.size();
    if (k < 1 || (size_t)k > V || !rng) return -1;
    const std::vector<llm::TokenId> &hist = s->s->tokens;
    std::vector<int32_t> window;
    for (size_t i = hist.size() > 64 ? hist.size() - 64 : 0; i < hist.size(); i++)
        if (std::find(window.begin(), window.end(), (int32_t)hist[i]) == window.end()) window.push_back((int32_t)hist[i]);
    std::vector<float> vals(k + window.size());
    std::vector<int32_t> ids(k + window.size());
    if (device_topk) {
        if (llm_session_topk(s, k, window.empty() ? nullptr : window.data(), (int)window.size(), vals.data(), ids.data()) != 0) return -1;
    } else {
        const std::vector<float> &l = s->s->last_logits;
        std::vector<int32_t> order(V);
        for (size_t i = 0; i < V; i++) order[i] = (int32_t)i;
        std::partial_sort(order.begin(), order.begin() + k, order.end(),
                          [&](int32_t a, int32_t b) { return l[a] > l[b] || (l[a] == l[b] && a < b); });
        for (int i = 0; i < k; i++) { ids[i] = order[i]; vals[i] = l[order[i]]; }
        for (size_t i = 0; i < window.size(); i++) { ids[k + i] = window[i]; vals[k + i] = l[window[i]]; }
    }
    struct Cand { float v; int32_t id; };
    std::vector<Cand> c;
    for (size_t i = 0; i < ids.size(); i++) {
        bool dup = false;
        for (auto &x : c) dup = dup || x.id == ids[i];
        if (dup) continue;
        float v = vals[i];
        if (std::find(window.begin(), window.end(), ids[i]) != window.end()) v = v > 0.0f ? v / 1.30f : v * 1.30f;
        c.push_back({v, ids[i]});
    }
    std::sort(c.begin(), c.end(), [](const Cand &a, const Cand &b) { return a.v > b.v || (a.v == b.v && a.id < b.id); });
    if (c.size() > (size_t)k) c.resize(k);
    double sum = 0.0;
    std::vector<double> pr(c.size());
    for (size_t i = 0; i < c.size(); i++) sum += (pr[i] = std::exp((double)(c[i].v - c[0].v) / (double)temperature));
    uint64_t x = *rng;
    x ^= x >> 12; x ^= x << 25; x ^= x >> 27;
    *rng = x;
    const double u = (double)((x * 0x2545F4914F6CDD1Dull) >> 11) / 9007199254740992.0 * sum;
    double acc = 0.0;
    llm::TokenId next = (llm::TokenId)c.back().id;
    for (size_t i = 0; i < c.size(); i++) {
        acc += pr[i];
        if (u < acc) { next = (llm::TokenId)c[i].id; break; }
    }
    s->s->tokens.push_back(next);
    llm::OutputRequest req;
    req.logits_on_device = device_topk != 0;
    model_evaluate(m, s, std::vector<llm::TokenId>{next}, req);
    return next;
}
int llm_infer_tokens_greedy_device(llm_model *m, llm_session *s, int n, int32_t *out) {
    if (n < 1) return 0;
    if (s->s->n_past + (size_t)n >= m->llama->params.context_size) {
        fprintf(stderr, "llm_infer_tokens_greedy_device: InferenceError::ContextFull\n");
        abort();
    }
    int done = 0;
    for (int attempt = 0; attempt < 2 && done < n; attempt++) {
        if (m->stages.empty() && s->s->last_graph &&
            ggml_hip_decode_greedy_chain(s->s->last_graph, n - done, out + done, s->s->last_logits.data()) == 0) {
            s->s->advance_device_chain((const llm::TokenId *)(out + done), (size_t)(n - done));
            return n;
        }
        out[done++] = llm_infer_next_token_greedy(m, s);
    }
    for (; done < n; done++) out[done] = llm_infer_next_token_greedy(m, s);
    return n;
}
int llm_evaluate_batch_via(llm_batch_entry entry, llm_model *m, llm_session *const *sessions, const int32_t *tokens, int B, float *logits) {
    if (!m || !sessions || !tokens || B < 1) return -1;
    if (!m->stages.empty() || !m->llama->is_first() || !m->llama->is_last()) return -1;
    const size_t V = m->llama->hyperparameters.n_vocab;
    for (int i = 0; i < B; i++) {
// ... 346 lines not shown
```

### llm_amd/csrc/kernels/decode.h

```cpp
#pragma once
#include "common.h"
#include "mmvq.h"
#include "ops.h"

struct DecParams {
    int n_past;
    int token;
    int store_at;
    int pad1;
    int tokens[32];
};
constexpr int BATCH_COLS_MAX = 8;
struct BatchCols {
    int pos[BATCH_COLS_MAX];
    __half *mem_k[BATCH_COLS_MAX];
    __half *mem_v[BATCH_COLS_MAX];
};

__global__ void __launch_bounds__(1024) k_argmax_next(const float *__restrict__ logits, int V, DecParams *prm,
                                                      int *__restrict__ out) {
    __shared__ float s_v[16];
    __shared__ int s_i[16];
    const int tid = threadIdx.x, lane = tid & 63, wave = tid >> 6;
    float bv = -INFINITY;
    int bi = 0x7fffffff;
    for (int i0 = tid; i0 < V; i0 += 8 * 1024) {
        float v8[8];
#pragma unroll
        for (int u = 0; u < 8; u++) {
            const int i = i0 + u * 1024;
            v8[u] = i < V ? logits[i] : -INFINITY;
        }
#pragma unroll
        for (int u = 0; u < 8; u++) {
            const int i = i0 + u * 1024;
            if (i < V && (v8[u] > bv || bi == 0x7fffffff)) {
                bv = v8[u];
                bi = i;
            }
        }
    }
    auto better = [](float v, int i, float bv_, int bi_) { return v > bv_ || (v == bv_ && i < bi_); };
#pragma unroll
    for (int off = 32; off >= 1; off >>= 1) {
        const float ov = __shfl_xor(bv, off);
        const int oi = __shfl_xor(bi, off);
        if (better(ov, oi, bv, bi)) {
            bv = ov;
            bi = oi;
        }
    }
    if (lane == 0) {
        s_v[wave] = bv;
        s_i[wave] = bi;
    }
    __syncthreads();
    if (tid == 0) {
        for (int w = 1; w < 16; w++)
            if (better(s_v[w], s_i[w], bv, bi)) {
                bv = s_v[w];
                bi = s_i[w];
            }
        prm->token = bi;
        prm->tokens[0] = bi;
        prm->n_past = prm->n_past + 1;
        out[0] = bi;
    }
}

__device__ __forceinline__ void rope_table_pair(int pos, int c, int kk, float theta_scale, float freq_scale, float *__restrict__ out) {
    float theta = freq_scale * (float)pos;
    for (int t = 0; t < kk; t++) theta *= theta_scale;
    out[c * 128 + 2 * kk] = cosf(theta);
    out[c * 128 + 2 * kk + 1] = sinf(theta);
}
__global__ void __launch_bounds__(128) k_rope_table(const DecParams *__restrict__ prm, float theta_scale, float freq_scale,
                                                    int half_d, float *__restrict__ out, unsigned *epoch = nullptr) {
    const int kk = threadIdx.x, c = blockIdx.x;
    if (epoch && kk == 0 && c == 0) {
        const unsigned e = *epoch + 1u;
        *epoch = e ? e : 1u;
    }
    if (kk >= half_d) return;
    rope_table_pair(prm->n_past + c, c, kk, theta_scale, freq_scale, out);
}
__global__ void __launch_bounds__(128) k_rope_table_batch(const BatchCols *__restrict__ bc, float theta_scale, float freq_scale,
                                                          int half_d, float *__restrict__ out) {
    const int kk = threadIdx.x, c = blockIdx.x;
    if (kk >= half_d) return;
    rope_table_pair(bc->pos[c], c, kk, theta_scale, freq_scale, out);
}

template <bool F16_D>
__device__ __forceinline__ void rmsnorm_quant_body(const float *__restrict__ x, const float *__restrict__ w, float eps, int E,
                                                   float *y_f32 , int8_t *lo, int8_t *hi, float *dq, int *sumq,
                                                   float *dT ,
                                                   int *sT ) {
    extern __shared__ __attribute__((aligned(16))) char smem[];
    float *s_y = (float *)smem;
    __shared__ double s_part[16];
    const int tid = threadIdx.x;
    {
        const int64_t r = blockIdx.x;
        x += r * E;
        if (y_f32) y_f32 += r * E;
        lo += r * (E / 2);
        hi += r * (E / 2);
        dq += r * (E / 32);
        sumq += r * (E / 32);
    }
    constexpr int PT = 8;
    const bool in_regs = E <= PT * 1024;
    float xv[PT], wv[PT];
    if (in_regs) {
#pragma unroll
        for (int k = 0; k < PT; k++) {
            const int i = tid + k * 1024;
            xv[k] = i < E ? x[i] : 0.0f;
            wv[k] = i < E ? w[i] : 0.0f;
        }
    }
    double s = 0.0;
    if (in_regs) {
#pragma unroll
        for (int k = 0; k < PT; k++)
            if (tid + k * 1024 < E) s += (double)(xv[k] * xv[k]);
    } else {
        for (int i = tid; i < E; i += 1024) {
            const float v = x[i];
            s += (double)(v * v);
        }
    }
    s = wave_sum_f64(s);
    if ((tid & 63) == 0) s_part[tid >> 6] = s;
    __syncthreads();
    double tot = 0.0;
#pragma unroll
    for (int i = 0; i < 16; i++) tot += s_part[i];
    const float mean = (float)(tot / (double)E);
    const float scale = 1.0f / sqrtf(mean + eps);
    if (in_regs) {
#pragma unroll
        for (int k = 0; k < PT; k++) {
            const int i = tid + k * 1024;
            if (i < E) {
                const float v = (xv[k] * scale) * wv[k];
                s_y[i] = v;
                if (y_f32) y_f32[i] = v;
            }
// ... 570 lines not shown
```

### llm_amd/csrc/plan_build.inc

```
static DevTensor *plan_rec(const ggml_tensor *t) {
    DevTensor *e = extra_of(t);
    if (!e) e = find_tensor((uintptr_t)t->data);
    return e;
}
static KWeight plan_kw(const ggml_tensor *t) {
    DevTensor *e = plan_rec(t);
    if (!e || !e->ksoa || (uintptr_t)t->data != e->host) die("decode plan: K-quant weight '%s' has no resident planar copy", t->name);
    return e->kw;
}
static QWeight plan_qw(const ggml_tensor *t) {
    DevTensor *e = plan_rec(t);
    if (!e || !e->soa || (uintptr_t)t->data != e->host) die("decode plan: weight '%s' has no resident SoA copy", t->name);
    return e->qw;
}
static F16W plan_f16w(const ggml_tensor *t) {
    DevTensor *e = plan_rec(t);
    if (!e || e->soa || e->ksoa) die("decode plan: F16 weight '%s' has no resident copy", t->name);
    return F16W{(const __half *)(e->dev + ((uintptr_t)t->data - e->host)), (int64_t)t->nb[1] / 2, t->ne[1]};
}
static uint64_t rec_id(const ggml_tensor *t) {
    DevTensor *e = plan_rec(t);
    return e ? (uint64_t)(uintptr_t)e->dev : 0;
}

// ... 67 lines not shown
    }
    return need;
}
template <class W, class F>
static std::vector<LayerMats<W>> plan_layer_weights(const LlamaMatch &m, F &&of) {
    std::vector<LayerMats<W>> v(m.layers.size());
    for (size_t il = 0; il < v.size(); il++)
        for (int i = 0; i < LAYER_MATS; i++) v[il].at(i) = of(m.layers[il].at(i));
    return v;
}
static bool k_prompt_weights(const LlamaMatch &m, DecodePlan *p) {
    const std::vector<const ggml_tensor *> ws = plan_matrices(m);
    for (auto *w : ws) {
        DevTensor *e = plan_rec(w);
        if (!e || !e->ksoa || (uintptr_t)w->data != e->host) return false;
    }
    if (const size_t need = w16_need(ws)) {
        size_t free_b = 0, total_b = 0;
        if (hipMemGetInfo(&free_b, &total_b) != hipSuccess || free_b < need + ((size_t)1 << 30) + w16_headroom()) return false;
        for (auto *w : ws)
            if (!ensure_w16_k(plan_rec(w))) return false;
    }
    if (!p) return true;
    auto qw_of = [&](const ggml_tensor *t) {
        DevTensor *e = plan_rec(t);
        QWeight w;
        memset(&w, 0, sizeof(w));
        w.M = e->kw.M;
        w.nb = e->kw.nsb * 8;
        w.qt = QT_Q8_0;
        w.w16 = e->w16;
        return w;
    };
    p->lw = plan_layer_weights<QWeight>(m, qw_of);
    if (m.output) p->output = qw_of(m.output);
    p->w16_gen = g.w16_gen;
    return true;
}
static void xcd_labels_probe() {
    if (g.xcd_labels >= 0) return;
    g.xcd_labels = 0;
    if (g.num_cus % 8 != 0 || g.num_cus < 16) return;
    unsigned *d = nullptr;
    dev_malloc((void **)&d, (size_t)g.num_cus * 4, "XCD probe");
    std::vector<unsigned> id((size_t)g.num_cus);
    bool ok = true;
    for (int rep = 0; rep < 2 && ok; rep++) {
        hipLaunchKernelGGL(k_xcc_ids, dim3((unsigned)g.num_cus), dim3(1024), 0, g.stream, d);
        HIP_CHECK(hipMemcpyAsync(id.data(), d, id.size() * 4, hipMemcpyDeviceToHost, g.stream));
        HIP_CHECK(hipStreamSynchronize(g.stream));
        unsigned seen = 0;
        for (int b = 0; b < 8; b++) seen |= 1u << id[(size_t)b];
        ok = __builtin_popcount(seen) == 8;
        for (int b = 8; b < g.num_cus && ok; b++) ok = id[(size_t)b] == id[(size_t)(b & 7)];
    }
    HIP_CHECK(hipFree(d));
    g.xcd_labels = ok ? 1 : 0;
}
struct PoolCarver {
    char *base;
    size_t off = 0;
    template <class T>
    void take(T *&field, size_t bytes) {
        if (base && bytes) field = (T *)(base + off);
        off = (off + bytes + 255) & ~(size_t)255;
    }
};
static void plan_pool_layout(DecodePlan *p, PoolCarver &c) {
    const LlamaMatch &m = p->m;
    const size_t R = (size_t)m.N;
    const size_t E = (size_t)m.E, F = (size_t)m.F, S = (size_t)p->att_S;
    const bool one = m.N == 1, spec = one && m.logits, multi = m.N >= 2 && !m.prompt, kq = m.kquant;
    const size_t Lg = one ? (size_t)m.L : 1;
    c.take(p->att_sc, (size_t)m.H * m.C * 4);
    c.take(p->att_pmax, (size_t)m.H * S * 4);
    c.take(p->att_part, (size_t)m.H * S * m.D * 4);
    c.take(p->att_mxg, Lg * m.H * S * 8);
    c.take(p->att_sumg, Lg * m.H * S * 16);
    c.take(p->att_partg, one ? Lg * m.H * S * m.D * 8 : 0);
    c.take(p->att_cnt, (size_t)m.H * 4);
    c.take(p->hot, 256);
    c.take(p->logits_alt, spec ? (size_t)m.V * 4 : 0);
    c.take(p->emb_alt, spec ? E * 4 : 0);
    c.take(p->epoch, 256);
    const size_t units = (size_t)((m.E + 2 * m.Egqa) / 2);
    c.take(p->gran, one ? (size_t)m.L * units * 8 : 0);
    c.take(p->dead_gran, one ? units * 8 : 0);
    c.take(p->ogran, one ? (size_t)m.L * (size_t)(m.E / 32) * OGRAN * 8 : 0);
    c.take(p->bcols, p->batch ? sizeof(BatchCols) : 0);
    c.take(p->logits_out, p->batch ? R * m.V * 4 : 0);
    c.take(p->emb_out, p->batch ? R * E * 4 : 0);
    c.take(p->prm, sizeof(DecParams));
    c.take(p->rope, std::max<size_t>(8, R) * 128 * 4);
    c.take(p->xa, R * E * 4);
    c.take(p->xb, R * E * 4);
    c.take(p->q, R * E * 4);
    c.take(p->gate, R * F * 4);
    c.take(p->e_lo, R * E / 2);
    c.take(p->e_hi, R * E / 2);
    c.take(p->e_d, R * E / 32 * 4);
    c.take(p->e_s, R * E / 32 * 4);
    c.take(p->f_lo, R * F / 2);
    c.take(p->f_hi, R * F / 2);
    c.take(p->f_d, R * F / 32 * 4);
    c.take(p->f_s, R * F / 32 * 4);
    const size_t passes = (R + 7) / 8;
    c.take(p->e_dT, multi ? passes * E / 32 * 32 : 0);
    c.take(p->e_sT, multi ? passes * E / 32 * 32 : 0);
    c.take(p->f_dT, multi ? passes * F / 32 * 32 : 0);
    c.take(p->f_sT, multi ? passes * F / 32 * 32 : 0);
    const size_t kW = std::max(E, F);
    c.take(p->k_kf, kq ? R * m.Egqa * 4 : 0);
    c.take(p->k_vf, kq ? R * m.Egqa * 4 : 0);
    c.take(p->k_att, kq || m.f16w ? R * E * 4 : 0);
    c.take(p->k_g3, kq ? R * F * 4 : 0);
    c.take(p->k_q8, kq ? R * kW : 0);
    c.take(p->k_d8, kq ? R * kW / 256 * 4 : 0);
    c.take(p->k_bs, kq ? R * kW / 256 * 32 : 0);
    c.take(p->p_tok, m.prompt ? R * 4 : 0);
}
static DecodePlan *build_plan(const LlamaMatch &m, std::vector<uint64_t> sig, bool batch = false) {
    if (m.prompt && !m.kquant) {
        const std::vector<const ggml_tensor *> ws = plan_matrices(m);
        size_t free_b = 0, total_b = 0;
        const bool room = hipMemGetInfo(&free_b, &total_b) == hipSuccess && free_b >= w16_need(ws) + w16_headroom();
        if (room)
            for (auto *w : ws) ensure_w16(plan_rec(w));
    }
    xcd_labels_probe();
    if (!g.hot_line) {
        dev_malloc(&g.hot_line, 256, "the dummy ring steps' line");
        HIP_CHECK(hipMemsetAsync(g.hot_line, 0, 256, g.stream));
    }
    DecodePlan *p = new DecodePlan();
    p->sig = std::move(sig);
    p->m = m;
    if (m.wte) (m.f16w ? (void)(p->f_wte = plan_f16w(m.wte)) : m.kquant ? (void)(p->k_wte = plan_kw(m.wte)) : (void)(p->wte = plan_qw(m.wte)));
    if (m.output) {
        if (m.f16w) p->f_output = plan_f16w(m.output);
        else if (m.kquant) p->k_output = plan_kw(m.output);
        else p->output = plan_qw(m.output);
        p->norm = (const float *)dev_ptr(m.norm);
    }
    if (m.stage_in) p->stage_in = (float *)dev_ptr(m.stage_in);
    if (m.stage_out) p->stage_out = (float *)dev_ptr(m.stage_out);
    p->batch = batch;
    if (!batch) {
        p->mem_k = (__half *)dev_ptr(m.memory_k);
        p->mem_v = (__half *)dev_ptr(m.memory_v);
    }
    if (m.f16w) p->flw = plan_layer_weights<F16W>(m, plan_f16w);
    else if (m.kquant) p->klw = plan_layer_weights<KWeight>(m, plan_kw);
    else p->lw = plan_layer_weights<QWeight>(m, plan_qw);
    for (auto &l : m.layers) p->ln.push_back({(const float *)dev_ptr(l.attn_norm), (const float *)dev_ptr(l.ffn_norm)});
    if (m.embedding && !batch) p->emb_out = (float *)dev_ptr(m.embedding);
    if (m.logits && !batch) p->logits_out = dev_ptr(m.logits);
    p->att_S = plan_att_S(m.H);
    PoolCarver sizes{nullptr};
    plan_pool_layout(p, sizes);
    dev_malloc((void **)&p->pool, sizes.off, "a decode plan's activation pool");
    HIP_CHECK(hipMemsetAsync(p->pool, 0, sizes.off, g.stream));
    PoolCarver carve{p->pool};
    plan_pool_layout(p, carve);
    if (!g.ferr_pin) {
        HIP_CHECK(hipHostMalloc((void **)&g.ferr_pin, 64, hipHostMallocDefault));
        *g.ferr_pin = 0;
// ... 5 lines not shown
```

### llm_amd/csrc/plan_decode.inc

```
struct PlanStats {
    double bytes[GGML_HIP_KCLASS_COUNT] = {0, 0, 0, 0};
    int64_t launches[GGML_HIP_KCLASS_COUNT] = {0, 0, 0, 0};
};
struct LaunchCtx {
    unsigned mask = ~0u, kind_mask = ~0u;
    PlanStats *st = nullptr;
    int ts_idx = 0;
    bool want(int k, double bytes) {
        if (!(mask & (1u << k))) return false;
        if (st) {
            st->bytes[k] += bytes;
            st->launches[k]++;
        }
        return true;
    }
    long long *next_ts() {
        if (!g.timeline) return nullptr;
        if ((size_t)(ts_idx + 1) * g.timeline_wgs * 8 * 8 > g.timeline_bytes) return nullptr;
        return g.timeline + (size_t)(ts_idx++) * g.timeline_wgs * 8;
    }
    template <class F>
    void mmvq(int kind, double bytes, F &&launch) {
        if (!(kind_mask & (1u << kind)) || !want(GGML_HIP_KCLASS_MMVQ, bytes)) return;
        Timed tm(GGML_HIP_KCLASS_MMVQ, bytes);
// ... 29 lines not shown
    }
    with_bool(a.probe || a.ts, [&](auto INSTR) {
        hipLaunchKernelGGL((k_mmvq_big<QT, EPI, XSRC, CT(INSTR)>), dim3(sh.G), dim3(threads), sh.lds, g.stream, b);
    });
}
template <int QT>
static void launch_qkv_attn(const BigArgs &ba, const FusedAttnArgs &fa, const FusedShape &sh, size_t lds) {
    with_bool(ba.probe || ba.ts, [&](auto INSTR) {
        lds_opt_in<k_qkv_attn<QT, CT(INSTR)>>(lds, ATTN_DECODE_LDS_MAX);
        hipLaunchKernelGGL((k_qkv_attn<QT, CT(INSTR)>), dim3(sh.G), dim3(1024), lds, g.stream, ba, fa);
    });
}
template <int QT>
static void launch_qkv_attn_wo(const BigArgs &ba, const FusedAttnArgs &fa, const WoTailArgs &wt, const FusedShape &sh, size_t lds) {
    const bool two = (wt.w.nb + 63) / 64 <= 2;
    with_bool(two, [&](auto TWO) {
        constexpr int STEPS = CT(TWO) ? 2 : 4;
        lds_opt_in<k_qkv_attn_wo<QT, STEPS>>(lds, ATTN_DECODE_LDS_MAX);
        hipLaunchKernelGGL((k_qkv_attn_wo<QT, STEPS>), dim3(sh.G), dim3(1024), lds, g.stream, ba, fa, wt);
    });
}
static void launch_attn_decode(const DecodePlan *p, int il, int N, int64_t rows, bool f16d, float *out_f32, long long *ts,
                               float *dT = nullptr, int *sT = nullptr) {
    const LlamaMatch &m = p->m;
    with_bool(f16d, [&](auto F16D) {
        lds_opt_in<k_attn_decode<CT(F16D)>>(attn_decode_lds(rows, m.D), ATTN_DECODE_LDS_MAX);
        hipLaunchKernelGGL(k_attn_decode<CT(F16D)>, dim3((unsigned)m.H, (unsigned)N), dim3(1024), attn_decode_lds(rows, m.D), g.stream,
                           (const float *)p->q, (const __half *)p->mem_k_at(il), (const __half *)p->mem_v_at(il), (const DecParams *)p->prm,
                           m.kq_scale, (int)m.D, (int)(m.H / m.Hkv), m.Egqa, m.C, out_f32, p->e_lo, p->e_hi, p->e_d, p->e_s, ts, (int)m.H,
                           rows, dT, sT);
    });
    HIP_CHECK(hipGetLastError());
}
static FusedAttnArgs fused_attn_args(const DecodePlan *p, int il, int S, int64_t Clds) {
    const LlamaMatch &m = p->m;
    FusedAttnArgs fa;
    memset(&fa, 0, sizeof(fa));
    fa.mem_k = p->mem_k_at(il); fa.mem_v = p->mem_v_at(il); fa.prm = p->prm; fa.epoch = p->epoch; fa.gran = p->gran_at(il);
    fa.k_pair0 = (int)(m.E / 2); fa.v_pair0 = (int)((m.E + m.Egqa) / 2);
    fa.scale = m.kq_scale; fa.D = (int)m.D; fa.n_rep = (int)(m.H / m.Hkv); fa.n_head = (int)m.H;
    fa.Egqa = m.Egqa; fa.C = m.C; fa.Clds = Clds;
    fa.err = p->ferr; fa.S = S; fa.layer = il;
    return fa;
}
static AttnSplitOneArgs split_attn_args(const DecodePlan *p, int il) {
    const LlamaMatch &m = p->m;
    AttnSplitOneArgs oa;
    memset(&oa, 0, sizeof(oa));
    AttnSplitArgs &sa = oa.a;
    sa.q = p->q; sa.mem_k = p->mem_k_at(il); sa.mem_v = p->mem_v_at(il); sa.prm = p->prm; sa.scale = m.kq_scale; sa.D = (int)m.D;
    sa.n_rep = (int)(m.H / m.Hkv); sa.n_head = (int)m.H; sa.S = p->att_S; sa.Egqa = m.Egqa; sa.C = m.C;
    sa.lo = p->e_lo; sa.hi = p->e_hi; sa.dq = p->e_d; sa.sumq = p->e_s;
    oa.mx_g = p->att_mxg_at(il); oa.sum_g = p->att_sumg_at(il); oa.part_g = p->att_partg_at(il); oa.cnt = p->att_cnt; oa.epoch = p->epoch; oa.layer = il;
    oa.err = p->ferr;
    return oa;
}
static void launch_attn_split_one(const DecodePlan *p, const AttnSplitOneArgs &oa, bool f16d) {
    const dim3 grid((unsigned)p->m.H, (unsigned)oa.a.S);
    with_bool(f16d, [&](auto F16D) {
        hipLaunchKernelGGL(k_attn_split_one<CT(F16D)>, grid, dim3(1024), attn_split_chunk_max(p->m.C, oa.a.S) * 6, g.stream, oa);
    });
}
template <class F>
static void for_each_weight_array(int qt, const QWeight &q, int64_t nb, F &&f) {
    f((const void *)q.qs, (size_t)nb * 16);
    if (qt == QT_Q8_0) f((const void *)q.qs2, (size_t)nb * 16);
    if (qt == QT_Q5_0 || qt == QT_Q5_1) f((const void *)q.qh, (size_t)nb * 4);
    f((const void *)q.d, (size_t)nb * 2);
    if (qt == QT_Q4_1 || qt == QT_Q5_1) f((const void *)q.m, (size_t)nb * 2);
}
template <class F>
static void for_each_type_run(const KWeight *const *ws, int n, F &&f) {
    for (int i = 0; i < n;) {
        int j = i + 1;
        while (j < n && ws[j]->kt == ws[i]->kt) j++;
        f(i, j);
        i = j;
    }
}
struct ResultDst {
    float *emb;
    char *logits;
};
static ResultDst plan_result_dst(const DecodePlan *p) {
    return ResultDst{p->spec_out && p->emb_out ? p->emb_alt : p->emb_out, p->spec_out ? p->logits_alt : p->logits_out};
}
template <class F>
static void plan_open_rows(DecodePlan *p, LaunchCtx &cx, bool batch, double embed_bytes, F &&embed) {
    const LlamaMatch &m = p->m;
    const int N = m.N;
    const float theta_scale = powf(m.freq_base, -2.0f / m.n_dims);
    if (!m.wte) {
        if (cx.want(GGML_HIP_KCLASS_OTHER, (double)N * m.E * 8.0))
            HIP_CHECK(hipMemcpyAsync(p->xa, p->stage_in, (size_t)N * m.E * 4, hipMemcpyDeviceToDevice, g.stream));
    } else {
        cx.other((double)N * m.E * embed_bytes, embed);
    }
    cx.other((double)N * m.D * 4.0, [&] {
        if (batch)
            hipLaunchKernelGGL(k_rope_table_batch, dim3((unsigned)N), dim3(128), 0, g.stream, (const BatchCols *)p->bcols, theta_scale, m.freq_scale,
                               (int)(m.D >> 1), p->rope);
        else
            hipLaunchKernelGGL(k_rope_table, dim3((unsigned)N), dim3(128), 0, g.stream, (const DecParams *)p->prm, theta_scale, m.freq_scale,
                               (int)(m.D >> 1), p->rope, p->epoch);
    });
}
static void launch_attn_decode_batch(const DecodePlan *p, int il, int N, bool f16d, float *out_f32);
static void plan_attn_f32(DecodePlan *p, LaunchCtx &cx, int il, bool long_ctx, bool batch) {
    const LlamaMatch &m = p->m;
    const int N = m.N;
    const double bytes = (double)N * ((double)(m.n_past + N) * m.Egqa * 4.0 + m.E * 9.0);
    if (!cx.want(GGML_HIP_KCLASS_ATTN, bytes)) return;
    Timed tm(GGML_HIP_KCLASS_ATTN, bytes);
    if (batch)
        launch_attn_decode_batch(p, il, N, true, p->k_att);
    else if (long_ctx) {
        AttnSplitOneArgs oa = split_attn_args(p, il);
        oa.out_f32 = p->k_att;
        launch_attn_split_one(p, oa, true);
    } else
        launch_attn_decode(p, il, N, m.C, true, p->k_att, nullptr);
    HIP_CHECK(hipGetLastError());
}
static bool plan_hand_on(DecodePlan *p, LaunchCtx &cx) {
    const LlamaMatch &m = p->m;
    if (m.output) return false;
    if (cx.want(GGML_HIP_KCLASS_OTHER, (double)m.N * m.E * 8.0))
        HIP_CHECK(hipMemcpyAsync(p->stage_out, p->xa, (size_t)m.N * m.E * 4, hipMemcpyDeviceToDevice, g.stream));
    return true;
}

static void plan_launch_all(DecodePlan *p, int av, LaunchCtx cx) {
    const bool long_ctx = av == AV_SPLIT;
    const LlamaMatch &m = p->m;
    const int qt = qt_of(m.wtype);
    const bool f16d = qt_f16d(qt);
    const bool big = g.opt_big != 0;
    const bool fuse_x = big;
    const int64_t E = m.E, F = m.F, nbE = E / 32, nbF = F / 32;
    const QAct actE{(const i32x4 *)p->e_lo, (const i32x4 *)p->e_hi, p->e_d, p->e_s};
    const QAct actF{(const i32x4 *)p->f_lo, (const i32x4 *)p->f_hi, p->f_d, p->f_s};
    const float theta_scale = powf(m.freq_base, -2.0f / m.n_dims);
    const double bb = (double)blk_bytes(qt);
    auto rmsq = [&](const float *x, const float *w, float *y) {
        cx.other((double)E * 9.25, [&] {
            with_bool(f16d, [&](auto F16D) {
                hipLaunchKernelGGL(k_rmsnorm_quant<CT(F16D)>, dim3(1), dim3(1024), (size_t)E * 4, g.stream, x, w, m.eps, (int)E, y,
                                   p->e_lo, p->e_hi, p->e_d, p->e_s);
            });
        });
    };
    auto matvec = [&](int kind, auto EPI, auto XSRC, auto XDEC, const DecMmvqArgs &a, float *y_out, const float *rope, int nwg, double bytes) {
        cx.mmvq(kind, bytes, [&] {
            with_qt(qt, [&](auto QT) {
                if (big)
                    launch_big<CT(QT), CT(EPI), CT(XSRC)>(BigArgs{a, y_out, cx.next_ts(), g.timeline_wgs, rope, g.opt_probe, nullptr, nullptr, 0, p->hot});
                else
                    fuse_x ? launch_dec<CT(QT), CT(EPI), CT(XDEC)>(a, nwg) : launch_dec<CT(QT), CT(EPI), XSRC_Q8>(a, nwg);
            });
        });
    };
    constexpr std::integral_constant<int, EPI_QKV> epi_qkv{};
    constexpr std::integral_constant<int, EPI_ADD> epi_add{};
    constexpr std::integral_constant<int, EPI_GATE> epi_gate{};
    constexpr std::integral_constant<int, EPI_STORE> epi_store{};
    constexpr std::integral_constant<int, XSRC_NORM> x_norm{};
    constexpr std::integral_constant<int, XSRC_Q8> x_q8{};
    constexpr std::integral_constant<int, XSRC_F32> x_f32{};
    if (m.wte)
// ... 463 lines not shown
```

### llm_amd/csrc/plan_run.inc

```
template <class F>
static void capture_into(hipGraph_t *graph, hipGraphExec_t *exec, F &&launch) {
    HIP_CHECK(hipStreamBeginCapture(g.stream, hipStreamCaptureModeThreadLocal));
    launch();
    HIP_CHECK(hipStreamEndCapture(g.stream, graph));
    HIP_CHECK(hipGraphInstantiate(exec, *graph, nullptr, nullptr, 0));
}
static void queue_results(const DecodePlan *p) {
    const LlamaMatch &m = p->m;
    if (m.logits && m.logits->backend == GGML_BACKEND_CPU) d2h_queue(m.logits->data, p->logits_out, (size_t)m.V * m.N * 4);
    if (m.embedding && m.embedding->data && p->emb_out && (size_t)m.N * (size_t)m.E * 4 <= ((size_t)128 << 10))
        d2h_queue(m.embedding->data, (const char *)p->emb_out, (size_t)m.N * (size_t)m.E * 4);
}
static void token_results_queue(DecodePlan *p) {
    if (p->m.N != 1 || p->m.prompt || !p->ferr) return;
    g.ferr_plan = p;
}
static void token_finish(bool can_rerun = true) {
    d2h_finish();
    DecodePlan *p = (DecodePlan *)g.ferr_plan;
    g.ferr_plan = nullptr;
    if (!p || !g.ferr_pin || !*(volatile unsigned *)g.ferr_pin) return;
    *(volatile unsigned *)g.ferr_pin = 0;
    g.stat_fused_timeouts++;
    spec_cancel();
    static const char *what =
        "an attention workgroup of k_qkv_attn / k_attn_split_one gave up waiting for rows of its own launch (these launches "
        "need all their workgroups resident at once: is another process, or a CU mask, holding compute units of this GPU?)";
    bool live = false;
    for (auto *q : g_plans) live = live || q == p;
    if (!live) die("%s", what);
    const bool whole = p->m.wte && p->m.output;
    if (!g.opt_fused_fallback || !can_rerun || !whole || p->m.N != 1)
        die("%s; set GGML_HIP_FUSE_ATTN=0 GGML_HIP_ATTN_ONE=0 to run the two-launch forms", what);
    static bool warned = false;
    if (!warned) fprintf(stderr, "libggml_hip: %s — re-running the token on the two-launch forms and keeping them on this device slot\n", what);
    warned = true;
    if (g.opt_fuse_attn || g.opt_attn_one) {
        g.fused_saved_fuse_attn = g.opt_fuse_attn;
        g.fused_saved_attn_one = g.opt_attn_one;
    }
    g.fused_rearm_stretch = g.fused_rearm_stretch ? g.fused_rearm_stretch * 2 : (uint64_t)std::max(0, g.opt_fused_rearm_tokens);
    g.fused_rearm_at = g.opt_fused_rearm_tokens > 0 ? g.stat_plan_tokens + g.fused_rearm_stretch : 0;
    g.opt_fuse_attn = 0;
    g.opt_attn_one = 0;
    if (!g.opt_test_fused_timeout) g.opt_affine = 0;
    g.opt_test_fused_timeout = 0;
    for (auto *q : g_plans) drop_plan_graphs(q);
    const LlamaMatch &m = p->m;
    {
        DecParams hp;
        memset(&hp, 0, sizeof(hp));
        hp.n_past = m.n_past;
        hp.token = m.embd ? ((const int32_t *)m.embd->data)[0] : 0;
        hp.tokens[0] = hp.token;
        h2d_small((char *)p->prm, &hp, sizeof(hp));
    }
    plan_launch_decode(p, attn_variant(m, p, m.n_past + 1));
    queue_results(p);
    d2h_finish();
    if (*(volatile unsigned *)g.ferr_pin) die("%s — and again on the re-run", what);
}
void finish_pending() {
    if (!g.pending_wait) return;
    const uint64_t t = now_ns();
    g.pending_wait = false;
    token_finish();
    g.ns_wait += now_ns() - t;
}

struct PrepMatch {
    ggml_cgraph *gr = nullptr;
    LlamaMatch m;
    DecodePlan *p = nullptr;
    uint64_t arena_seq = 0, wgen = 0;
    int opt_gen = 0;
};
static bool prepare_decode_plan(ggml_cgraph *gr) {
    if (!g.prep) g.prep = new PrepMatch();
    PrepMatch *pm = (PrepMatch *)g.prep;
    pm->gr = nullptr;
    if (!g.opt_plan || !g.opt_prepare || !gr) return false;
    LlamaMatch m;
    if (!match_llama_decode(gr, m) || m.prompt || m.N != 1 || !plan_weights_resident(m)) return false;
    const std::vector<uint64_t> sig = plan_signature(m);
    const uint64_t wgen = g_dev_wgen[g.device & 63].load(std::memory_order_acquire);
    DecodePlan *p = nullptr;
    for (auto *q : g_plans)
        if (q->sig == sig && q->wgen == wgen) p = q;
    if (!p) return false;
    pm->m = m;
    pm->p = p;
    pm->arena_seq = g_arena_seq.load(std::memory_order_acquire);
    pm->wgen = wgen;
    pm->opt_gen = g.opt_gen;
    pm->gr = gr;
    return true;
}

static DecodePlan *find_or_build_plan(const LlamaMatch &m, const std::vector<uint64_t> &sig, bool batch = false) {
    const uint64_t wgen = g_dev_wgen[g.device & 63].load(std::memory_order_acquire);
    {
        bool stale = false;
        for (auto *q : g_plans) stale = stale || q->wgen != wgen;
        if (stale) drop_all_plans();
    }
    DecodePlan *p = nullptr;
    for (auto *q : g_plans)
        if (q->sig == sig) p = q;
    if (!p) {
        if (g_plans.size() >= 32) drop_all_plans();
        p = build_plan(m, sig, batch);
        p->wgen = wgen;
        g_plans.push_back(p);
    } else {
        p->m = m;
    }
    return p;
}

static bool try_decode_plan(ggml_cgraph *gr, bool defer_wait = false) {
    g.chain_plan = nullptr;
    if (!g.opt_plan) return false;
    if (g.fused_rearm_at && g.stat_plan_tokens >= g.fused_rearm_at) {
        g.fused_rearm_at = 0;
        g.opt_fuse_attn = g.fused_saved_fuse_attn;
        g.opt_attn_one = g.fused_saved_attn_one;
        g.stat_fused_rearms++;
        spec_cancel();
        if (g.stream) HIP_CHECK(hipStreamSynchronize(g.stream));
        for (auto *q : g_plans) drop_plan_graphs(q);
    }
    const uint64_t t0 = now_ns();
    LlamaMatch m;
    DecodePlan *p = nullptr;
    if (PrepMatch *pm = (PrepMatch *)g.prep) {
        if (pm->gr == gr && pm->arena_seq == g_arena_seq.load(std::memory_order_acquire) && pm->opt_gen == g.opt_gen &&
            pm->wgen == g_dev_wgen[g.device & 63].load(std::memory_order_acquire))
            for (auto *q : g_plans)
                if (q == pm->p) p = q;
        if (p) {
            m = pm->m;
            p->m = m;
            g.stat_prepared_tokens++;
        }
        pm->gr = nullptr;
    }
    if (!p) {
        if (!match_llama_decode(gr, m)) return false;
        if (!plan_weights_resident(m)) {
            upload_inputs(gr);
            if (!plan_weights_resident(m)) return false;
        }
        if (m.prompt && m.kquant && !k_prompt_weights(m, nullptr)) {
            if (m.N > MULTI_MAX_N) return false;
            LlamaMatch m2;
            tl_k_prompt_off = true;
            const bool ok = match_llama_decode(gr, m2);
            tl_k_prompt_off = false;
            if (!ok) return false;
            m = m2;
        }
        p = find_or_build_plan(m, plan_signature(m));
    }
    const uint64_t t1 = now_ns();
    bool spec_hit = false;
    if (g.spec.pending) {
        g.spec.pending = false;
        const bool same = g.spec.plan == (void *)p && m.N == 1 && !m.prompt && m.embd && m.n_past == g.spec.n_past &&
                          attn_variant(m, p, m.n_past + 1) == g.spec.av && g.opt_graph && !g.timing.on;
        if (same) {
            HIP_CHECK(hipEventSynchronize(g.spec.tok_ev));
            spec_hit = *g.spec.tok_pin == ((const int32_t *)m.embd->data)[0];
        }
        if (spec_hit) {
            g.stat_spec_hits++;
        } else {
            g.stat_spec_misses++;
            g.spec.cooldown = 8;
        }
    }
    DecParams hp;
    hp.n_past = m.n_past;
    hp.token = m.embd ? ((const int32_t *)m.embd->data)[0] : 0;
    hp.store_at = hp.pad1 = 0;
    for (int i = 0; i < 32; i++) {
        hp.tokens[i] = (m.embd && i < m.N && !m.prompt) ? ((const int32_t *)m.embd->data)[i] : 0;
        if (m.wte && (hp.tokens[i] < 0 || hp.tokens[i] >= m.wte->ne[1])) die("token id %d out of range", hp.tokens[i]);
    }
    if (!spec_hit) h2d_small((char *)p->prm, &hp, sizeof(hp));
    if (m.prompt) {
        if (m.wte) {
            const int32_t *ids = (const int32_t *)m.embd->data;
            for (int i = 0; i < m.N; i++)
                if (ids[i] < 0 || ids[i] >= m.wte->ne[1]) die("token id %d out of range", ids[i]);
            h2d_small((char *)p->p_tok, ids, (size_t)m.N * 4);
        }
        plan_launch_prompt(p);
        if (m.logits && m.logits->backend == GGML_BACKEND_CPU)
            d2h_queue(m.logits->data, p->logits_out, (size_t)m.V * m.N * 4);
        const uint64_t t2p = now_ns();
        g.ns_match += t1 - t0;
        g.ns_launch += t2p - t1;
        g.stat_prompt_plan_tokens += (uint64_t)m.N;
        if (defer_wait) {
            g.pending_wait = true;
            g.pending_light = true;
            return true;
        }
        d2h_finish();
        g.ns_wait += now_ns() - t2p;
        return true;
    }
    const bool use_graph = g.opt_graph && !g.timing.on;
    {
        const uint64_t dgen = g_dev_gen[g.device & 63].load(std::memory_order_relaxed);
        if (p->dev_gen != dgen) {
            if (p->dev_gen) {
                HIP_CHECK(hipStreamSynchronize(g.stream));
                drop_plan_graphs(p);
            }
            p->dev_gen = dgen;
        }
    }
    const int av = attn_variant(m, p, m.n_past + 1);
    const bool long_ctx = av == AV_SPLIT;
    auto launch = [&] {
        if (m.N > 1 && !m.kquant && !m.f16w)
            plan_launch_multi(p);
        else
            plan_launch_decode(p, av);
    };
    if (spec_hit) {
    } else if (use_graph) {
        VariantGraphs &vg = p->graphs[av];
        if (!vg.exec) capture_into(&vg.graph, &vg.exec, launch);
        HIP_CHECK(hipGraphLaunch(vg.exec, g.stream));
        p->replays++;
    } else {
        launch();
    }
    if (spec_hit) {
        HIP_CHECK(hipMemcpyAsync(p->logits_out, p->logits_alt, (size_t)m.V * 4, hipMemcpyDeviceToDevice, g.stream));
        if (p->emb_out) HIP_CHECK(hipMemcpyAsync(p->emb_out, p->emb_alt, (size_t)m.E * 4, hipMemcpyDeviceToDevice, g.stream));
    }
    queue_results(p);
    token_results_queue(p);
    if (g.spec.cooldown > 0) g.spec.cooldown--;
    if (g.opt_speculate_next && g.spec.cooldown == 0 && use_graph && m.N == 1 && m.logits && m.wte && m.output &&
        m.n_past + 2 < m.C && p->graphs[av].exec) {
        const int av2 = attn_variant(m, p, m.n_past + 2);
        {
            if (!g.results_ev) HIP_CHECK(hipEventCreateWithFlags(&g.results_ev, hipEventDisableTiming));
            if (!g.spec.tok_ev) {
                HIP_CHECK(hipEventCreateWithFlags(&g.spec.tok_ev, hipEventDisableTiming));
                HIP_CHECK(hipHostMalloc((void **)&g.spec.tok_pin, 64, hipHostMallocDefault));
                HIP_CHECK(hipMalloc((void **)&g.spec.tok_dev, 64));
            }
            HIP_CHECK(hipEventRecord(g.results_ev, g.stream));
            g.results_ev_armed = true;
            g.results_ev_copies = stg.pending.size();
            hipLaunchKernelGGL(k_argmax_next, dim3(1), dim3(1024), 0, g.stream, (const float *)p->logits_out, (int)m.V, p->prm, g.spec.tok_dev);
            HIP_CHECK(hipMemcpyAsync(g.spec.tok_pin, g.spec.tok_dev, 4, hipMemcpyDeviceToHost, g.stream));
            HIP_CHECK(hipEventRecord(g.spec.tok_ev, g.stream));
            VariantGraphs &vg2 = p->graphs[av2];
            if (!vg2.spec_exec) {
                p->spec_out = true;
                capture_into(&vg2.spec_graph, &vg2.spec_exec, [&] { plan_launch_decode(p, av2); });
                p->spec_out = false;
            }
            HIP_CHECK(hipGraphLaunch(vg2.spec_exec, g.stream));
            g.spec.pending = true;
            g.spec.plan = p;
            g.spec.n_past = m.n_past + 1;
            g.spec.av = av2;
        }
    }
    const uint64_t t2 = now_ns();
    g.ns_match += t1 - t0;
    g.ns_launch += t2 - t1;
    g.stat_plan_tokens += (uint64_t)m.N;
    if (long_ctx) g.stat_split_tokens++;
    if (m.N == 1 && !long_ctx) {
        const FusedShape fs = fused_qkv_shape(m, av_heads_split(av));
        if (fs.ok) g.stat_fused_tokens++;
        if (fs.ok && fs.wo) g.stat_fused_wo_tokens++;
        if (fs.ok && fs.affine) g.stat_fused_affine_tokens++;
    }
    if (av >= AV_FUSED2) g.stat_fused_heads_tokens++;
    if (m.kquant) g.stat_kplan_tokens += (uint64_t)m.N;
    g.chain_plan = (m.N == 1 && m.logits && m.wte) ? (void *)p : nullptr;
    g.chain_graph = gr;
    if (defer_wait) {
        g.pending_wait = true;
        g.pending_light = m.N > 1;
        return true;
    }
    token_finish();
    g.ns_wait += now_ns() - t2;
    return true;
}

static int decode_greedy_chain(ggml_cgraph *last, int n, int32_t *out_tokens, float *last_logits) {
    finish_pending();
    if (g.spec.pending) {
        spec_cancel();
        return -1;
    }
    DecodePlan *p = (DecodePlan *)g.chain_plan;
    if (!p || g.chain_graph != last || n < 1) return -1;
    bool live = false;
    for (auto *q : g_plans) live = live || q == p;
    const LlamaMatch &m = p->m;
    if (!live || m.N != 1 || !m.logits || !m.wte || m.n_past + 1 + n > m.C) return -1;
    if (p->chain_cap < n) {
        if (p->chain_out) (void)hipFree(p->chain_out);
        p->chain_cap = std::max(n, 256);
        HIP_CHECK(hipMalloc((void **)&p->chain_out, (size_t)p->chain_cap * 4));
    }
    if (!p->chain_ring) HIP_CHECK(hipMalloc((void **)&p->chain_ring, 64 * 4));
    const bool use_graph = g.opt_graph && !g.timing.on && p->any_captured();
    int i0 = 0;
    if (use_graph && g.opt_chain_k > 1) {
        const int K = g.opt_chain_k;
        const auto long_at = [&](int i) { return attn_variant(m, p, m.n_past + 1 + i + 1) != AV_SHORT; };
        while (i0 + K <= n && !long_at(i0 + K - 1)) {
            if (!p->exec_chain || p->chain_k != K) {
                if (p->exec_chain) (void)hipGraphExecDestroy(p->exec_chain);
                if (p->graph_chain) (void)hipGraphDestroy(p->graph_chain);
                capture_into(&p->graph_chain, &p->exec_chain, [&] {
                    for (int k = 0; k < K; k++) {
                        hipLaunchKernelGGL(k_argmax_next, dim3(1), dim3(1024), 0, g.stream, (const float *)p->logits_out, (int)m.V, p->prm,
                                           p->chain_ring + k);
                        plan_launch_decode(p, AV_SHORT);
                    }
                });
                p->chain_k = K;
            }
            HIP_CHECK(hipGraphLaunch(p->exec_chain, g.stream));
            if (fused_qkv_shape(m).ok) g.stat_fused_tokens += (uint64_t)K;
            HIP_CHECK(hipMemcpyAsync(p->chain_out + i0, p->chain_ring, (size_t)K * 4, hipMemcpyDeviceToDevice, g.stream));
            i0 += K;
        }
    }
    for (int i = i0; i < n; i++) {
        hipLaunchKernelGGL(k_argmax_next, dim3(1), dim3(1024), 0, g.stream, (const float *)p->logits_out, (int)m.V, p->prm,
                           p->chain_out + i);
        const int av = attn_variant(m, p, m.n_past + 1 + i + 1);
        if (av != AV_SPLIT && fused_qkv_shape(m, av_heads_split(av)).ok) g.stat_fused_tokens++;
        if (av >= AV_FUSED2) g.stat_fused_heads_tokens++;
        if (use_graph) {
            VariantGraphs &vg = p->graphs[av];
            if (!vg.exec) capture_into(&vg.graph, &vg.exec, [&] { plan_launch_decode(p, av); });
            if (!vg.exec2) HIP_CHECK(hipGraphInstantiate(&vg.exec2, vg.graph, nullptr, nullptr, 0));
            HIP_CHECK(hipGraphLaunch((i & 1) ? vg.exec2 : vg.exec, g.stream));
        } else {
            plan_launch_decode(p, av);
        }
    }
    HIP_CHECK(hipGetLastError());
    d2h_queue(out_tokens, (const char *)p->chain_out, (size_t)n * 4);
    if (last_logits) d2h_queue(last_logits, p->logits_out, (size_t)m.V * 4);
    token_results_queue(p);
    token_finish(false);
    p->m.n_past += n;
    p->replays += use_graph ? (uint64_t)n : 0;
    g.stat_plan_tokens += (uint64_t)n;
    g.chain_plan = nullptr;
    return 0;
}

static int decode_batch(ggml_cgraph *const *graphs, int B) {
    ensure_init();
    finish_pending();
    spec_cancel();
    g.chain_plan = nullptr;
    if (PrepMatch *pm = (PrepMatch *)g.prep) pm->gr = nullptr;
    if (!g.opt_plan || !g.opt_plan_batch) return -1;
    const uint64_t t0 = now_ns();
    std::vector<LlamaMatch> ms((size_t)B);
    std::vector<uint64_t> sig;
    for (int c = 0; c < B; c++) {
        LlamaMatch &m = ms[(size_t)c];
        if (!match_llama_decode(graphs[c], m)) return -1;
        if (m.N != 1 || m.prompt || m.kquant || !m.wte || !m.output || !m.embd || !m.logits || !m.embedding) return -1;
        if (m.n_past >= m.C || (qt_of(m.wtype) < 0 && !m.f16w)) return -1;
        for (const ggml_tensor *t : {m.memory_k, m.memory_v}) {
            const DevTensor *e = (const DevTensor *)t->extra;
            if (e && e->magic == 0x48495054 && e->slot != g_cur_slot()) return -1;
        }
    }
    if (attn_decode_lds(ms[0].C, ms[0].D) > ATTN_DECODE_LDS_MAX || (!ms[0].f16w && !multi_shape_ok(ms[0], B))) return -1;
    ws_reset();
    for (int c = 0; c < B; c++) {
        const LlamaMatch &m = ms[(size_t)c];
        if (!plan_weights_resident(m)) {
            upload_inputs(graphs[c]);
            if (!plan_weights_resident(m)) return -1;
        }
        std::vector<uint64_t> s = plan_signature(m, false);
        if (c == 0) sig = std::move(s);
        else if (s != sig) return -1;
    }
    std::vector<__half *> mk((size_t)B), mv((size_t)B);
    for (int c = 0; c < B; c++) {
        mk[(size_t)c] = (__half *)dev_ptr(ms[(size_t)c].memory_k);
        mv[(size_t)c] = (__half *)dev_ptr(ms[(size_t)c].memory_v);
        for (int d = 0; d < c; d++)
            if (mk[(size_t)d] == mk[(size_t)c] || mv[(size_t)d] == mv[(size_t)c]) return -1;
    }
    LlamaMatch mb = ms[0];
    mb.N = B;
    mb.n_past = 0;
    sig[0] = (uint64_t)B;
    sig.push_back(0x6261746368ull);
    DecodePlan *p = find_or_build_plan(mb, sig, true);
    for (int c = 0; c < B; c++) mb.n_past = std::max(mb.n_past, ms[(size_t)c].n_past);
    p->m.n_past = mb.n_past;
    const uint64_t t1 = now_ns();
    DecParams hp;
    BatchCols hb;
    memset(&hp, 0, sizeof(hp));
    memset(&hb, 0, sizeof(hb));
    for (int c = 0; c < B; c++) {
        const LlamaMatch &m = ms[(size_t)c];
        hp.tokens[c] = ((const int32_t *)m.embd->data)[0];
        if (hp.tokens[c] < 0 || hp.tokens[c] >= m.wte->ne[1]) die("token id %d out of range", hp.tokens[c]);
        hb.pos[c] = m.n_past;
        hb.mem_k[c] = mk[(size_t)c];
        hb.mem_v[c] = mv[(size_t)c];
    }
    hp.n_past = hb.pos[0];
    hp.token = hp.tokens[0];
    h2d_small((char *)p->prm, &hp, sizeof(hp));
    h2d_small((char *)p->bcols, &hb, sizeof(hb));
    if (g.opt_graph && !g.timing.on) {
        VariantGraphs &vg = p->graphs[AV_SHORT];
        if (!vg.exec) capture_into(&vg.graph, &vg.exec, [&] { plan_launch_batch(p); });
        HIP_CHECK(hipGraphLaunch(vg.exec, g.stream));
        p->replays++;
    } else {
        plan_launch_batch(p);
    }
    for (int c = 0; c < B; c++) {
        const LlamaMatch &m = ms[(size_t)c];
        const char *lrow = p->logits_out + (size_t)c * m.V * 4, *erow = (const char *)p->emb_out + (size_t)c * m.E * 4;
        if (m.logits->backend == GGML_BACKEND_CPU) d2h_queue(m.logits->data, lrow, (size_t)m.V * 4);
        else HIP_CHECK(hipMemcpyAsync(dev_ptr(m.logits), lrow, (size_t)m.V * 4, hipMemcpyDeviceToDevice, g.stream));
        HIP_CHECK(hipMemcpyAsync(dev_ptr(m.embedding), erow, (size_t)m.E * 4, hipMemcpyDeviceToDevice, g.stream));
        if (m.embedding->data) d2h_queue(m.embedding->data, erow, (size_t)m.E * 4);
    }
    const uint64_t t2 = now_ns();
    g.stat_plan_tokens += (uint64_t)B;
    g.stat_batch_tokens += (uint64_t)B;
    g.stat_batch_steps++;
    d2h_finish();
    g.ns_match += t1 - t0;
    g.ns_launch += t2 - t1;
    g.ns_wait += now_ns() - t2;
// ... 3 lines not shown
```

### llm_amd/csrc/plan_shapes.inc

```

struct F16W {
    const __half *p;
    int64_t ld, M;
};
static const int LAYER_MATS = 7;
template <class W>
struct LayerMats {
    W wq{}, wk{}, wv{}, wo{}, w1{}, w2{}, w3{};
    const W &at(int i) const {
        const W *const all[LAYER_MATS] = {&wq, &wk, &wv, &wo, &w1, &w2, &w3};
        return *all[i];
    }
    W &at(int i) { return const_cast<W &>(static_cast<const LayerMats *>(this)->at(i)); }
};
struct LayerW : LayerMats<const ggml_tensor *> {
    const ggml_tensor *attn_norm = nullptr, *ffn_norm = nullptr;
    const ggml_tensor *cur = nullptr;
    bool k_store = false, v_store = false;
};
static const int PROMPT_PLAN_MAX = 4096;
#define MULTI_MAX_N 31
struct LlamaMatch {
    int L = 0;
    int64_t E = 0, H = 0, Hkv = 0, D = 0, F = 0, V = 0, C = 0, Egqa = 0;
    int n_past = 0, n_dims = 0;
    int N = 1;
    bool prompt = false;
    bool kquant = false;
    bool f16w = false;
    float eps = 0, freq_base = 0, freq_scale = 0, kq_scale = 0;
    ggml_type wtype = GGML_TYPE_F32;
    const ggml_tensor *wte = nullptr, *norm = nullptr, *output = nullptr, *embd = nullptr, *memory_k = nullptr,
                      *memory_v = nullptr;
    ggml_tensor *logits = nullptr, *embedding = nullptr;
    const ggml_tensor *stage_in = nullptr, *stage_out = nullptr;
    std::vector<LayerW> layers;
};
enum { AV_SHORT = 0, AV_SPLIT = 1, AV_FUSED2 = 2, AV_FUSED3 = 3, AV_FUSED4 = 4, AV_COUNT = 5 };
static inline int av_heads_split(int av) { return av >= AV_FUSED2 ? av : 1; }
struct VariantGraphs {
    hipGraph_t graph = nullptr;
    hipGraphExec_t exec = nullptr, exec2 = nullptr;
    hipGraph_t spec_graph = nullptr;
    hipGraphExec_t spec_exec = nullptr;
    void drop() {
        for (hipGraphExec_t e : {exec, exec2, spec_exec})
            if (e) (void)hipGraphExecDestroy(e);
        for (hipGraph_t gr : {graph, spec_graph})
            if (gr) (void)hipGraphDestroy(gr);
        *this = VariantGraphs{};
    }
};
struct DecodePlan {
    std::vector<uint64_t> sig;
    LlamaMatch m;
    using LW = LayerMats<QWeight>;
    using KLW = LayerMats<KWeight>;
    using FLW = LayerMats<F16W>;
    std::vector<LW> lw;
    std::vector<KLW> klw;
    std::vector<FLW> flw;
    struct LayerNorms {
        const float *attn_norm, *ffn_norm;
    };
    std::vector<LayerNorms> ln;
    F16W f_wte{}, f_output{};
    KWeight k_wte{}, k_output{};
    float *k_kf = nullptr, *k_vf = nullptr, *k_att = nullptr, *k_g3 = nullptr;
    int8_t *k_q8 = nullptr;
    float *k_d8 = nullptr;
    int16_t *k_bs = nullptr;
    QWeight wte, output;
    const float *norm = nullptr;
    __half *mem_k = nullptr, *mem_v = nullptr;
    __half *mem_k_at(int il) const { return mem_k + (size_t)il * m.C * m.Egqa; }
    __half *mem_v_at(int il) const { return mem_v + (size_t)il * m.C * m.Egqa; }
    int64_t kv_off(int il) const { return (int64_t)il * m.C * m.Egqa; }
    bool batch = false;
    BatchCols *bcols = nullptr;
    char *pool = nullptr;
    DecParams *prm = nullptr;
    float *rope = nullptr;
    unsigned *epoch = nullptr;
    const void *hot = nullptr;
    unsigned *ferr = nullptr;
    unsigned long long *gran = nullptr;
    unsigned long long *gran_at(int il) const { return gran + (size_t)il * (size_t)((m.E + 2 * m.Egqa) / 2); }
    unsigned long long *ogran = nullptr;
    unsigned long long *dead_gran = nullptr;
    uint64_t dev_gen = 0;
    uint64_t wgen = 0;
    float *xa = nullptr, *xb = nullptr, *q = nullptr, *gate = nullptr, *logits = nullptr;
    int8_t *e_lo = nullptr, *e_hi = nullptr, *f_lo = nullptr, *f_hi = nullptr;
    float *e_d = nullptr, *f_d = nullptr;
    int *e_s = nullptr, *f_s = nullptr;
    float *e_dT = nullptr, *f_dT = nullptr;
    int *e_sT = nullptr, *f_sT = nullptr;
    float *p_te = nullptr, *p_qf = nullptr, *p_kf = nullptr, *p_vf = nullptr, *p_mg = nullptr, *p_g1 = nullptr, *p_g3 = nullptr, *p_sc = nullptr;
    _Float16 *p_x16 = nullptr, *p_p16 = nullptr;
    int *p_tok = nullptr;
    float *stage_in = nullptr, *stage_out = nullptr;
    float *emb_out = nullptr;
    char *logits_out = nullptr;
    char *logits_alt = nullptr;
    float *emb_alt = nullptr;
    bool spec_out = false;
    int *chain_out = nullptr;
    int *chain_ring = nullptr;
    int chain_cap = 0;
    VariantGraphs graphs[AV_COUNT];
    bool any_captured() const {
        for (const VariantGraphs &v : graphs)
            if (v.exec) return true;
        return false;
    }
    float *att_sc = nullptr, *att_pmax = nullptr, *att_part = nullptr;
    unsigned long long *att_mxg = nullptr, *att_sumg = nullptr, *att_partg = nullptr;
    unsigned long long *att_mxg_at(int il) const { return att_mxg + (size_t)il * m.H * att_S; }
    unsigned long long *att_sumg_at(int il) const { return att_sumg + (size_t)il * m.H * att_S * 2; }
    unsigned long long *att_partg_at(int il) const { return att_partg + (size_t)il * m.H * att_S * m.D; }
    unsigned *att_cnt = nullptr;
    int att_S = 1;
    hipGraph_t graph_chain = nullptr;
    hipGraphExec_t exec_chain = nullptr;
    int chain_k = 0;
    uint64_t replays = 0;
    uint64_t w16_gen = 0;
};

std::vector<DecodePlan *> g_plans_[GGML_HIP_MAX_BACKENDS];
#define g_plans (g_plans_[g.slot])

void drop_plan_graphs(DecodePlan *p) {
    for (VariantGraphs &v : p->graphs) v.drop();
    if (p->exec_chain) (void)hipGraphExecDestroy(p->exec_chain);
    if (p->graph_chain) (void)hipGraphDestroy(p->graph_chain);
    p->exec_chain = nullptr;
    p->graph_chain = nullptr;
    p->chain_k = 0;
}
void destroy_plan(DecodePlan *p) {
    drop_plan_graphs(p);
    if (p->chain_ring) (void)hipFree(p->chain_ring);
    if (p->pool) (void)hipFree(p->pool);
    delete p;
}
void spec_cancel() {
    if (!g.spec.pending) return;
    g.spec.pending = false;
    if (g.stream) HIP_CHECK(hipStreamSynchronize(g.stream));
}
void drop_all_plans() {
    spec_cancel();
    if (g_plans.empty()) return;
    if (g.stream) HIP_CHECK(hipStreamSynchronize(g.stream));
    for (auto *p : g_plans) destroy_plan(p);
    g_plans.clear();
    g.ferr_plan = nullptr;
}
static inline size_t attn_decode_lds(int64_t C, int64_t D) { return (size_t)(C + D) * 4 + (size_t)C * 2; }
static const size_t ATTN_DECODE_LDS_MAX = 150 * 1024;
static int big_waves(int64_t units, int G, int min_waves) {
    static const int forced = getenv("GGML_HIP_BIG_WAVES") ? atoi(getenv("GGML_HIP_BIG_WAVES")) : 0;
    if (forced >= 8 && forced <= BIG_W) return std::max(forced, min_waves);
    auto score = [&](int W) {
        const int64_t per_round = (int64_t)G * W, rounds = (units + per_round - 1) / per_round;
        return (double)units / (double)(rounds * per_round) * (1.0 - 0.015 * (BIG_W - W));
    };
    int best = BIG_W;
    for (int W = BIG_W - 1; W >= std::max(8, min_waves); W--)
        if (score(W) > score(best) + 1e-9) best = W;
    return best;
}
static int big_min_waves(int xsrc, int epi, int64_t nb) {
    int min_waves = 8;
    if (xsrc == XSRC_Q8) min_waves = (int)((nb + 63) / 64);
    if (xsrc == XSRC_F32) min_waves = (int)((nb * 32 + 24 * 64 - 1) / (24 * 64));
    if (xsrc == XSRC_NORM) min_waves = epi == EPI_QKV ? 10 : 8;
    return std::max(min_waves, 8);
}
static inline int big_groups(int64_t units, int cus) { return (int)std::min<int64_t>(cus, std::max<int64_t>(1, (units + BIG_W - 1) / BIG_W)); }
static inline int64_t big_rounds(int64_t units, int G, int W) { return (units + (int64_t)G * W - 1) / ((int64_t)G * W); }
struct BigShape {
    bool ok;
    int G, W;
    size_t lds;
};
static BigShape big_shape(int xsrc, int epi, int64_t nb, int64_t units) {
    BigShape s;
    s.G = big_groups(units, g.num_cus);
    s.W = big_waves(units, s.G, big_min_waves(xsrc, epi, nb));
    s.ok = big_rounds(units, s.G, s.W) <= 64;
    s.lds = (size_t)((nb + 63) / 64 * 64) * 40;
    return s;
}
struct FusedShape {
    bool ok = false;
    int G = 0, W = 0, S = 1;
    bool wo = false;
    bool affine = false;
};
static FusedShape fused_qkv_shape(const LlamaMatch &m, int S = 1) {
    FusedShape s;
    if (!g.opt_fuse_attn || !g.opt_big || m.kquant || m.f16w || m.N != 1 || m.D > 128 || m.D % 32 != 0) return s;
    const int H = (int)m.H * S;
    const int64_t units = (m.E + 2 * m.Egqa) / 2;
    if (H + 1 > g.num_cus) return s;
    if (device_sharers() > 1 && (int64_t)device_sharers() * H > g.num_cus / 4) return s;
    s.S = S;
    const int G0 = big_groups(units, g.num_cus), Gp = big_groups(units, g.num_cus - H);
    const int Wp = big_waves(units, Gp, big_min_waves(XSRC_NORM, EPI_QKV, m.E / 32));
    if (big_rounds(units, Gp, Wp) > 64) return s;
    if (S == 1 && g.opt_fuse_attn < 2 && (Gp * 10 < G0 * 7 || Gp < 2 * H)) return s;
    if (S > 1) {
        const double qkv_bytes = (double)(m.E + 2 * m.Egqa) * (double)(m.E / 32) * (double)blk_bytes(qt_of(m.wtype));
        const bool q5 = qt_of(m.wtype) == QT_Q5_0 || qt_of(m.wtype) == QT_Q5_1;
        if (Gp < g.num_cus / 4) return s;
        if (g.opt_fuse_attn < 2 && (Gp * 100 < G0 * 45 || qkv_bytes * (q5 ? 1.7 : 1.0) > 90e6)) return s;
    }
    s.ok = true;
    s.G = H + Gp;
    s.W = Wp;
    if (g.opt_fuse_wo && device_sharers() == 1) {
        const int64_t nbE = m.E / 32, rows = (m.E + Gp - 1) / Gp;
        if (rows <= 16 * WO_RW && (nbE + 63) / 64 <= 4 && nbE * OGRAN <= 1024 * WO_NG_MAX) s.wo = true;
    }
    if (g.opt_affine && g.xcd_labels == 1 && device_sharers() == 1 && m.H % 8 == 0 && Gp % 8 == 0 && m.Egqa == m.E &&
        (m.D == 32 || m.D == 64 || m.D == 128) && m.E == m.H * m.D)
        s.affine = true;
    return s;
}
static inline int64_t attn_split_min(bool fused = true) { return g.opt_attn_split > 1 ? g.opt_attn_split : fused ? ATTN_SPLIT_MIN_FUSED : ATTN_SPLIT_MIN; }
static inline int64_t attn_split_min_of(const LlamaMatch &m) { return attn_split_min(fused_qkv_shape(m).ok); }
static inline int plan_att_S(int64_t H) { return (int)std::max<int64_t>(1, std::min<int64_t>(16, g.num_cus / std::max<int64_t>(1, H))); }
static inline bool attn_split_from_min(int64_t H) { return g.opt_attn_split && g.opt_big && plan_att_S(H) >= 2; }
// ... 99 lines not shown
```

### llm_amd/ggml.py

```python
import ctypes as C
import os

import numpy as np

_HERE = os.path.dirname(os.path.abspath(__file__))
LIB_PATH = os.environ.get("GGML_HIP_LIB") or os.path.join(_HERE, "libggml_hip.so")

TYPE_F32, TYPE_F16, TYPE_Q4_0, TYPE_Q4_1, TYPE_Q5_0, TYPE_Q5_1, TYPE_Q8_0, TYPE_Q8_1 = 0, 1, 2, 3, 6, 7, 8, 9
TYPE_Q2_K, TYPE_Q3_K, TYPE_Q4_K, TYPE_Q5_K, TYPE_Q6_K, TYPE_Q8_K = 10, 11, 12, 13, 14, 15
TYPE_I8, TYPE_I16, TYPE_I32 = 16, 17, 18
BACKEND_CPU, BACKEND_GPU, BACKEND_GPU_SPLIT = 0, 10, 20
OP_NONE, OP_MUL_MAT = 0, 21
MAX_NODES, MAX_SRC, MAX_NAME, HASHTABLE = 4096, 6, 48, 8273
KCLASS_MMVQ, KCLASS_MMQ_MFMA, KCLASS_ATTN, KCLASS_OTHER = 0, 1, 2, 3
COMM_ID_BYTES = 128
KKIND_BASE = 16

TYPE_NAMES = {TYPE_F32: "f32", TYPE_F16: "f16", TYPE_Q4_0: "q4_0", TYPE_Q4_1: "q4_1", TYPE_Q5_0: "q5_0",
              TYPE_Q5_1: "q5_1", TYPE_Q8_0: "q8_0", TYPE_Q2_K: "q2_K", TYPE_Q3_K: "q3_K", TYPE_Q4_K: "q4_K", TYPE_Q5_K: "q5_K",
              TYPE_Q6_K: "q6_K", TYPE_I32: "i32"}
BLOCK_BYTES = {TYPE_F32: 4, TYPE_F16: 2, TYPE_Q4_0: 18, TYPE_Q4_1: 20, TYPE_Q5_0: 22, TYPE_Q5_1: 24, TYPE_Q8_0: 34,
               TYPE_Q8_1: 40, TYPE_Q2_K: 84, TYPE_Q3_K: 110, TYPE_Q4_K: 144, TYPE_Q5_K: 176, TYPE_Q6_K: 210, TYPE_Q8_K: 292,
               TYPE_I8: 1, TYPE_I16: 2, TYPE_I32: 4}
BLOCK_ELEMS = {TYPE_F32: 1, TYPE_F16: 1, TYPE_Q4_0: 32, TYPE_Q4_1: 32, TYPE_Q5_0: 32, TYPE_Q5_1: 32, TYPE_Q8_0: 32,
# ... 146 lines not shown
    "ggml_quantize_q5_K": (C.c_size_t, [C.c_void_p, C.c_void_p, C.c_int, C.c_int, C.c_void_p]),
    "ggml_quantize_q6_K": (C.c_size_t, [C.c_void_p, C.c_void_p, C.c_int, C.c_int, C.c_void_p]),
    "ggml_quantize_chunk": (C.c_size_t, [C.c_int, C.c_void_p, C.c_void_p, C.c_int, C.c_int, C.c_void_p]),
    "ggml_internal_get_type_traits": (ggml_type_traits_t, [C.c_int]),
    "ggml_cpu_has_blas": (C.c_int, []),
    "ggml_cpu_has_gpublas": (C.c_int, []),
}
_HOOKS = {
    "init_XXblas": (None, []),
    "PFX_set_tensor_split": (None, [C.c_void_p]),
    "PFX_mul": (None, [TP, TP, TP]),
    "PFX_can_mul_mat": (C.c_bool, [TP, TP, TP]),
    "PFX_mul_mat_get_wsize": (C.c_size_t, [TP, TP, TP]),
    "PFX_mul_mat": (None, [TP, TP, TP, C.c_void_p, C.c_size_t]),
    "PFX_host_malloc": (C.c_void_p, [C.c_size_t]),
    "PFX_host_free": (None, [C.c_void_p]),
    "PFX_transform_tensor": (None, [C.c_void_p, TP]),
    "PFX_free_data": (None, [TP]),
    "PFX_assign_buffers": (None, [TP]),
    "PFX_assign_buffers_no_scratch": (None, [TP]),
    "PFX_assign_buffers_force_inplace": (None, [TP]),
    "PFX_set_main_device": (None, [C.c_int]),
    "PFX_set_mul_mat_q": (None, [C.c_bool]),
    "PFX_set_scratch_size": (None, [C.c_size_t]),
    "PFX_free_scratch": (None, []),
    "PFX_compute_forward": (C.c_bool, [C.POINTER(ggml_compute_params), TP]),
}
for _k, _v in _HOOKS.items():
    if _k == "init_XXblas":
        PROTOTYPES["ggml_init_hipblas"] = _v
        PROTOTYPES["ggml_init_cublas"] = _v
    else:
        PROTOTYPES[_k.replace("PFX", "ggml_hip")] = _v
        PROTOTYPES[_k.replace("PFX", "ggml_cuda")] = _v
PROTOTYPES.update({
    "ggml_hip_device_count": (C.c_int, []),
    "ggml_hip_slot_physical_device": (C.c_int, [C.c_int]),
    "ggml_hip_thread_session_slot": (C.c_int, []),
    "ggml_hip_synchronize": (None, []),
    "ggml_hip_tensor_get": (None, [TP, C.c_void_p, C.c_size_t, C.c_size_t]),
    "ggml_hip_tensor_set": (None, [TP, C.c_void_p, C.c_size_t, C.c_size_t]),
    "ggml_hip_tensor_device_ptr": (C.c_void_p, [TP]),
    "ggml_hip_memcpy": (None, [C.c_void_p, C.c_void_p, C.c_size_t, C.c_int]),
    "ggml_hip_timing_begin": (None, []),
    "ggml_hip_timing_end": (None, []),
    "ggml_hip_timing_query": (None, [C.c_int, C.POINTER(C.c_double), C.POINTER(C.c_int64), C.POINTER(C.c_double)]),
    "ggml_hip_set_option": (None, [C.c_char_p, C.c_int]),
    "ggml_hip_get_option": (C.c_int, [C.c_char_p]),
    "ggml_hip_get_stat": (C.c_int64, [C.c_char_p]),
    "ggml_hip_read_timeline": (C.c_size_t, [C.c_void_p, C.c_size_t]),
    "ggml_hip_get_main_device": (C.c_int, []),
    "ggml_hip_bind_thread_device": (None, [C.c_int]),
    "ggml_hip_thread_pinned_device": (C.c_int, []),
    "ggml_hip_unbind_thread_device": (None, []),
    "ggml_hip_get_tensor_split": (C.c_int, [C.c_void_p, C.c_int]),
    "ggml_hip_set_layer_split": (None, [C.c_void_p, C.c_int]),
    "ggml_hip_get_layer_split": (C.c_int, [C.c_void_p, C.c_int]),
    "ggml_hip_copy_between_devices": (None, [C.c_int, C.c_void_p, C.c_int, C.c_void_p, C.c_size_t]),
    "ggml_hip_share_stream": (C.c_int, [C.c_int, C.c_int]),
    "ggml_hip_debug_prompt_attention": (C.c_int, [C.c_void_p, C.c_void_p, C.c_void_p, C.c_void_p, C.c_int, C.c_int, C.c_int, C.c_int,
                                                  C.c_int, C.c_int64, C.c_float, C.c_int]),
    "ggml_hip_debug_prompt_attention_plan": (C.c_int, [C.c_void_p, C.c_void_p, C.c_void_p, C.c_void_p, C.c_void_p, C.c_void_p, C.c_void_p,
                                                       C.c_int, C.c_int, C.c_int, C.c_int, C.c_int, C.c_int64, C.c_float, C.c_int]),
    "ggml_hip_debug_mul_mat_cols": (C.c_int, [C.c_void_p, C.c_void_p, C.c_void_p, C.c_int]),
    "ggml_hip_debug_mat_vec_big": (C.c_int, [C.c_void_p, C.c_void_p, C.c_void_p, C.c_int, C.c_int, C.c_void_p, C.c_void_p, C.c_float,
                                             C.c_void_p, C.c_void_p, C.c_void_p, C.c_int, C.c_int, C.c_float, C.c_float, C.c_int64,
                                             C.c_void_p, C.c_void_p]),
    "ggml_hip_debug_mat_vec_kbig": (C.c_int, [C.c_void_p, C.c_void_p, C.c_void_p, C.c_int, C.c_int, C.c_void_p, C.c_void_p, C.c_float,
                                              C.c_void_p, C.c_void_p, C.c_void_p, C.c_int, C.c_int, C.c_float, C.c_float, C.c_int64,
                                              C.c_void_p, C.c_void_p]),
    "ggml_hip_debug_mat_vec_f16": (C.c_int, [C.c_void_p, C.c_void_p, C.c_void_p, C.c_int, C.c_int, C.c_void_p, C.c_void_p, C.c_float,
                                             C.c_void_p, C.c_void_p, C.c_void_p, C.c_int, C.c_int, C.c_float, C.c_float, C.c_int64,
                                             C.c_void_p, C.c_void_p, C.c_int]),
    "ggml_hip_debug_exp_le0": (C.c_int, [C.c_void_p, C.c_void_p]),
    "ggml_hip_decode_greedy_chain": (C.c_int, [C.c_void_p, C.c_int, C.c_void_p, C.c_void_p]),
    "ggml_hip_decode_batch": (C.c_int, [C.c_void_p, C.c_int]),
    "ggml_hip_topk": (C.c_int, [C.c_void_p, C.c_int64, C.c_int, C.c_void_p, C.c_int, C.c_void_p, C.c_void_p]),
    "ggml_hip_row_probs": (C.c_int, [C.c_void_p, C.c_int64, C.c_int64, C.c_void_p, C.c_void_p]),
    "ggml_hip_quantize": (C.c_size_t, [C.c_int, C.c_void_p, C.c_void_p, C.c_int64, C.c_int64, C.c_void_p]),
    "ggml_hip_quantize_resident": (C.c_int, [C.c_void_p, C.c_void_p, C.c_void_p]),
    "ggml_hip_graph_compute_begin": (C.c_int, [C.c_void_p]),
    "ggml_hip_graph_prepare": (C.c_int, [C.c_void_p]),
    "ggml_hip_graph_compute_end": (None, []),
    "ggml_hip_bench_plan_class": (C.c_int, [C.c_int, C.c_int, C.POINTER(C.c_double), C.POINTER(C.c_int64),
                                            C.POINTER(C.c_double)]),
    "ggml_hip_comm_unique_id": (C.c_int, [C.c_void_p]),
    "ggml_hip_comm_init": (C.c_int, [C.c_int, C.c_int, C.c_void_p]),
    "ggml_hip_comm_destroy": (None, []),
    "ggml_hip_comm_ranks": (C.c_int, []),
    "ggml_hip_comm_send": (None, [C.c_void_p, C.c_size_t, C.c_int]),
    "ggml_hip_comm_recv": (None, [C.c_void_p, C.c_size_t, C.c_int]),
    "ggml_hip_comm_sendrecv": (None, [C.c_void_p, C.c_int, C.c_void_p, C.c_int, C.c_size_t]),
    "ggml_hip_bench_empty": (C.c_int, [C.c_int, C.c_int, C.c_int, C.c_int, C.c_int, C.c_int, C.POINTER(C.c_double)]),
    "ggml_hip_version": (C.c_char_p, []),
})

_lib = None


def lib():
    global _lib
    if _lib is None:
        if not os.path.exists(LIB_PATH):
            raise RuntimeError(
                f"{LIB_PATH} is missing: run `python -c 'import __graft_entry__ as g; g.build()'` "
                "(hipcc --offload-arch=gfx950). There is no CPU / pure-Python fallback for the compute path.")
        L = C.CDLL(LIB_PATH)
        for name, (res, args) in PROTOTYPES.items():
            f = getattr(L, name)
            f.restype = res
            f.argtypes = args
        _lib = L
    return _lib


def has_gpu():
    try:
        return lib().ggml_hip_device_count() > 0
    except Exception:
        return False


def row_bytes(t, k):
    return k // BLOCK_ELEMS[t] * BLOCK_BYTES[t]


def quantize(t, x):
    x = np.ascontiguousarray(x, dtype=np.float32)
    if t == TYPE_F32:
        return x.view(np.uint8).reshape(-1).copy()
    if t == TYPE_F16:
        out = np.zeros(x.size, dtype=np.uint16)
        lib().ggml_fp32_to_fp16_row(x.ctypes.data, out.ctypes.data, x.size)
        return out.view(np.uint8)
    k = x.shape[-1]
    out = np.zeros(row_bytes(t, x.size), dtype=np.uint8)
    hist = np.zeros(16, dtype=np.int64)
    fn = getattr(lib(), "ggml_quantize_" + TYPE_NAMES[t])
    got = fn(x.ctypes.data, out.ctypes.data, x.size, k, hist.ctypes.data)
    assert got == out.size, (got, out.size)
    return out


def quantize_on_device(t, x):
    x = np.ascontiguousarray(x, dtype=np.float32)
    out = np.zeros(row_bytes(t, x.size), dtype=np.uint8)
    hist = np.zeros(16, dtype=np.int64)
    got = lib().ggml_hip_quantize(t, x.ctypes.data, out.ctypes.data, x.size, x.shape[-1], hist.ctypes.data)
    assert got == out.size, (got, out.size)
    return out, hist


def topk(tensor, row, k, extra_ids=()):
    extra = np.ascontiguousarray(extra_ids, dtype=np.int32)
    vals = np.zeros(k + extra.size, dtype=np.float32)
    ids = np.zeros(k + extra.size, dtype=np.int32)
    ptr = tensor.ptr if isinstance(tensor, Tensor) else tensor
    rc = lib().ggml_hip_topk(ptr, row, k, extra.ctypes.data if extra.size else None, extra.size, vals.ctypes.data, ids.ctypes.data)
    if rc != 0:
        raise ValueError("ggml_hip_topk: bad arguments")
    return vals, ids


def row_probs(node, targets, row_begin=0):
    targets = np.ascontiguousarray(targets, dtype=np.int32)
    out = np.zeros(targets.size, dtype=np.float32)
# ... 200 lines not shown
```

Before: 842.0.

## Add fused token-tail kernel with double-buffered results and greedy speculative next-step launch

Adds a k_token_tail kernel that copies logits and embeddings into pinned host slots and computes the greedy argmax in one launch. The results and slots are double-buffered (parity sets) so the next decode step can be launched speculatively on device while the host reads the current result. A greedy hint from the host sampler enables this by default. KV rows are saved before speculation and restored if it is cancelled, which adds extra kernels, buffers and bookkeeping plus risk around result-pointer redirection and cancellation paths.

```diff
diff --git a/include/ggml_hip.h b/include/ggml_hip.h
--- a/include/ggml_hip.h
+++ b/include/ggml_hip.h
@@ -464,6 +464,7 @@
 GGML_API int ggml_hip_graph_compute_begin(struct ggml_cgraph *cgraph);
 GGML_API void ggml_hip_graph_compute_end(void);
 GGML_API int ggml_hip_graph_prepare(struct ggml_cgraph *cgraph);
+GGML_API void ggml_hip_expect_greedy_next(void);
 GGML_API int ggml_hip_decode_greedy_chain(struct ggml_cgraph *last, int n, int32_t *out_tokens, float *last_logits);
 GGML_API int ggml_hip_decode_batch(struct ggml_cgraph *const *graphs, int n_graphs);
 GGML_API int ggml_hip_topk(const struct ggml_tensor *t, int64_t row, int k, const int32_t *extra_ids, int n_extra,
@@ -479,6 +480,8 @@
                                                   const uint16_t *mem_v, uint16_t *x16, float *out, int N, int E, int Egqa, int H,
                                                   int n_past, int64_t C, float scale, int f16d);
 GGML_API int ggml_hip_debug_exp_le0(uint16_t *out_fast, uint16_t *out_ref);
+GGML_API int ggml_hip_debug_token_tail(const float *logits, int V, const float *emb, int E, int n_past, int misalign,
+                                       int32_t *id_tail, int32_t *id_argmax, float *slot_logits, float *slot_emb, int32_t *prm_out);
 GGML_API int ggml_hip_debug_mul_mat_cols(const struct ggml_tensor *w, const float *x, float *out, int N);
 GGML_API int ggml_hip_debug_mat_vec_big(const struct ggml_tensor *w0, const struct ggml_tensor *w1, const struct ggml_tensor *w2,
                                         int xsrc, int epi, const float *x, const float *norm_w, float eps, const float *res, float *out,
diff --git a/llm_amd/csrc/backend_executor.inc b/llm_amd/csrc/backend_executor.inc
--- a/llm_amd/csrc/backend_executor.inc
+++ b/llm_amd/csrc/backend_executor.inc
@@ -137,6 +137,8 @@
     g_xi8.valid = false;
     g_xk.valid = false;
     if (try_decode_plan(gr)) return;
+    spec_cancel();
+    res_settle();
     g.stat_generic_graphs++;
     upload_inputs(gr);
 
diff --git a/llm_amd/csrc/backend_state.inc b/llm_amd/csrc/backend_state.inc
--- a/llm_amd/csrc/backend_state.inc
+++ b/llm_amd/csrc/backend_state.inc
@@ -93,19 +93,25 @@
     ggml_cgraph *chain_graph = nullptr;
     bool pending_wait = false;
     bool pending_light = false;
-    int opt_speculate_next = 0;
+    int opt_speculate_next = 0, opt_token_tail = 1;
+    bool greedy_hint = false;
     struct Spec {
         bool pending = false;
         void *plan = nullptr;
         int n_past = 0, av = 0;
-        int32_t *tok_pin = nullptr;
-        int *tok_dev = nullptr;
-        hipEvent_t tok_ev = nullptr;
+        int parity = 0;
+        int32_t fed_id = 0;
+        bool fed_id_valid = false;
         int cooldown = 0;
     } spec;
-    hipEvent_t results_ev = nullptr;
-    bool results_ev_armed = false;
-    size_t results_ev_copies = 0;
+    struct TailWait {
+        void *plan = nullptr;
+        int q = 0;
+        void *logits_dst = nullptr, *emb_dst = nullptr;
+        bool staged = false;
+    } tail;
+    void *res_plan = nullptr;
+    uint64_t stat_tail_tokens = 0, stat_result_copies = 0, stat_tail_hits = 0, stat_tail_misses = 0;
     uint64_t stat_spec_hits = 0, stat_spec_misses = 0;
     unsigned *ferr_pin = nullptr;
     void *ferr_plan = nullptr;
@@ -154,6 +160,7 @@
     {"chain_k", &Backend::opt_chain_k, OPT_ENV, FX_NONE, 0, 64},
     {"prepare", &Backend::opt_prepare, OPT_ENV},
     {"speculate_next", &Backend::opt_speculate_next, OPT_ENV, FX_SPECULATE_NEXT},
+    {"token_tail", &Backend::opt_token_tail, OPT_ENV, FX_SPECULATE_NEXT},
     {"fuse_attn", &Backend::opt_fuse_attn, OPT_ENV | OPT_DROPS, FX_FUSE_ATTN},
     {"fuse_wo", &Backend::opt_fuse_wo, OPT_ENV | OPT_DROPS},
     {"warm_mb", &Backend::opt_warm_mb, OPT_ENV | OPT_DROPS},
@@ -208,6 +215,10 @@
     {"fused_rearms", &Backend::stat_fused_rearms},
     {"spec_hits", &Backend::stat_spec_hits},
     {"spec_misses", &Backend::stat_spec_misses},
+    {"tail_tokens", &Backend::stat_tail_tokens},
+    {"tail_hits", &Backend::stat_tail_hits},
+    {"tail_misses", &Backend::stat_tail_misses},
+    {"result_copies", &Backend::stat_result_copies},
     {"generic_graphs", &Backend::stat_generic_graphs},
     {"alibi_fused", &Backend::stat_alibi_fused},
     {"flash_attn_nodes", &Backend::stat_flash_attn_nodes},
@@ -766,13 +777,7 @@
     stg.pending.push_back({host_dst, s, n});
 }
 void d2h_finish() {
-    if (g.results_ev_armed && stg.pending.size() != g.results_ev_copies) g.results_ev_armed = false;
-    if (g.results_ev_armed) {
-        g.results_ev_armed = false;
-        HIP_CHECK(hipEventSynchronize(g.results_ev));
-    } else {
-        HIP_CHECK(hipStreamSynchronize(g.stream));
-    }
+    HIP_CHECK(hipStreamSynchronize(g.stream));
     for (auto &p : stg.pending) memcpy(p.host_dst, p.stage, p.n);
     stg.pending.clear();
     stg.small_off = 0;
diff --git a/llm_amd/csrc/backend_tools.inc b/llm_amd/csrc/backend_tools.inc
--- a/llm_amd/csrc/backend_tools.inc
+++ b/llm_amd/csrc/backend_tools.inc
@@ -509,6 +509,47 @@
     return 0;
 }
 
+int ggml_hip_debug_token_tail(const float *logits, int V, const float *emb, int E, int n_past, int misalign, int32_t *id_tail,
+                              int32_t *id_argmax, float *slot_logits, float *slot_emb, int32_t *prm_out) {
+    if (!logits || V < 1 || (emb && E < 1) || misalign < 0 || misalign > 3 || !id_tail || !id_argmax || !slot_logits || !prm_out) return -1;
+    SlotLock lk;
+    ensure_init();
+    finish_pending();
+    const size_t lb = ((size_t)(V + 4) * 4 + 255) & ~(size_t)255, eb = ((size_t)(std::max(E, 1) + 4) * 4 + 255) & ~(size_t)255;
+    const size_t emb_off = ((size_t)V * 4 + 255) & ~(size_t)255, id_off = emb_off + eb;
+    char *d = nullptr, *slot = nullptr;
+    dev_malloc((void **)&d, lb + eb + 1024, "debug token tail");
+    HIP_CHECK(hipHostMalloc((void **)&slot, id_off + 256, hipHostMallocDefault));
+    memset(slot, 0xff, id_off + 256);
+    float *dl = (float *)d + misalign, *de = (float *)(d + lb) + misalign;
+    DecParams *pa = (DecParams *)(d + lb + eb), *pb = pa + 1;
+    int *ida = (int *)(pb + 1);
+    DecParams hp;
+    memset(&hp, 0, sizeof(hp));
+    hp.n_past = n_past;
+    HIP_CHECK(hipStreamSynchronize(g.stream));
+    HIP_CHECK(hipMemcpy(dl, logits, (size_t)V * 4, hipMemcpyHostToDevice));
+    if (emb) HIP_CHECK(hipMemcpy(de, emb, (size_t)E * 4, hipMemcpyHostToDevice));
+    HIP_CHECK(hipMemcpy(pa, &hp, sizeof(hp), hipMemcpyHostToDevice));
+    HIP_CHECK(hipMemcpy(pb, &hp, sizeof(hp), hipMemcpyHostToDevice));
+    hipLaunchKernelGGL(k_argmax_next, dim3(1), dim3(1024), 0, g.stream, (const float *)dl, V, pa, ida);
+    hipLaunchKernelGGL(k_token_tail, dim3(TOKEN_TAIL_WGS), dim3(1024), 0, g.stream, (const float *)dl, V, emb ? (const float *)de : (const float *)nullptr,
+                       E, pb, slot, (int)emb_off, (int)id_off);
+    HIP_CHECK(hipGetLastError());
+    HIP_CHECK(hipStreamSynchronize(g.stream));
+    HIP_CHECK(hipMemcpy(id_argmax, ida, 4, hipMemcpyDeviceToHost));
+    HIP_CHECK(hipMemcpy(&hp, pb, sizeof(hp), hipMemcpyDeviceToHost));
+    prm_out[0] = hp.n_past;
+    prm_out[1] = hp.token;
+    prm_out[2] = hp.tokens[0];
+    *id_tail = *(const int32_t *)(slot + id_off);
+    memcpy(slot_logits, slot, (size_t)V * 4);
+    if (emb && slot_emb) memcpy(slot_emb, slot + emb_off, (size_t)E * 4);
+    HIP_CHECK(hipHostFree(slot));
+    HIP_CHECK(hipFree(d));
+    return 0;
+}
+
 int ggml_hip_decode_greedy_chain(struct ggml_cgraph *last, int n, int32_t *out_tokens, float *last_logits) {
     SlotLock lk;
     return decode_greedy_chain(last, n, out_tokens, last_logits);
diff --git a/llm_amd/csrc/hip_backend.hip b/llm_amd/csrc/hip_backend.hip
--- a/llm_amd/csrc/hip_backend.hip
+++ b/llm_amd/csrc/hip_backend.hip
@@ -177,7 +177,7 @@
     SlotLock lk;
     const uint64_t t0 = now_ns();
     ensure_init();
-    if (g.pending_wait && g.pending_light && stg.pending.empty() && !g.results_ev_armed) {
+    if (g.pending_wait && g.pending_light && stg.pending.empty()) {
         g.pending_wait = false;
         g.ferr_plan = nullptr;
     } else {
@@ -201,6 +201,10 @@
     SlotLock lk;
     ensure_init();
     return prepare_decode_plan(cgraph) ? 1 : 0;
+}
+extern "C" void ggml_hip_expect_greedy_next(void) {
+    SlotLock lk;
+    g.greedy_hint = true;
 }
 extern "C" void ggml_hip_graph_compute_end(void) {
     SlotLock lk;
@@ -449,7 +453,7 @@
         if (e ? e->soa : find_arena((uintptr_t)t->data) == nullptr) return -1;
     }
     finish_pending();
-    const float *x = (const float *)(dev_ptr(t) + row * (int64_t)t->nb[1]);
+    const float *x = (const float *)(result_dev_ptr(t) + row * (int64_t)t->nb[1]);
     char *buf = ws_alloc((size_t)(k + n_extra) * 8 + (size_t)n_extra * 4 + 64);
     float *dv = (float *)buf;
     int *di = (int *)(buf + (size_t)(k + n_extra) * 4);
@@ -481,7 +485,7 @@
         if (e ? e->soa : find_arena((uintptr_t)t->data) == nullptr) return -1;
     }
     finish_pending();
-    const float *x = (const float *)(dev_ptr(t) + row_begin * (int64_t)t->nb[1]);
+    const float *x = (const float *)(result_dev_ptr(t) + row_begin * (int64_t)t->nb[1]);
     const int V = (int)t->ne[0];
     char *buf = ws_alloc((size_t)n_rows * 8 + 64);
     float *dp = (float *)buf;
@@ -661,18 +665,23 @@
 void ggml_hip_tensor_get(const struct ggml_tensor *tensor, void *host_dst, size_t offset, size_t nbytes) {
     SlotLock lk;
     ensure_init();
-    d2h_queue(host_dst, dev_ptr(tensor) + offset, nbytes);
+    finish_pending();
+    spec_guard_read(dev_ptr(tensor) + offset, nbytes);
+    d2h_queue(host_dst, result_dev_ptr(tensor) + offset, nbytes);
     d2h_finish();
 }
 void ggml_hip_tensor_set(struct ggml_tensor *tensor, const void *host_src, size_t offset, size_t nbytes) {
     SlotLock lk;
     ensure_init();
+    spec_guard_read(dev_ptr(tensor) + offset, nbytes);
     h2d_bulk(dev_ptr(tensor) + offset, host_src, nbytes);
     HIP_CHECK(hipStreamSynchronize(g.stream));
 }
 void ggml_hip_memcpy(void *dst, const void *src, size_t nbytes, int kind) {
     SlotLock lk;
     ensure_init();
+    if (kind != 1) spec_guard_read((const char *)dst, nbytes);
+    if (kind != 0) spec_guard_read((const char *)src, nbytes);
     if (kind == 0) {
         h2d_bulk((char *)dst, src, nbytes);
         HIP_CHECK(hipStreamSynchronize(g.stream));
diff --git a/llm_amd/csrc/host/llm_host.cpp b/llm_amd/csrc/host/llm_host.cpp
--- a/llm_amd/csrc/host/llm_host.cpp
+++ b/llm_amd/csrc/host/llm_host.cpp
@@ -62,6 +62,7 @@
     std::vector<float> *embeddings = nullptr;
     bool logits_on_device = false;
     bool intermediate_chunk = false;
+    bool greedy_next = false;
 };
 
 struct GraphOutputs {
@@ -523,6 +524,8 @@
 
 namespace {
 std::atomic<int> g_split_sessions{0};
+extern "C" void ggml_hip_expect_greedy_next(void) __attribute__((weak));
+
 struct HomeDevice {
     int pinned = ggml_hip_thread_pinned_device();
     int home = ggml_hip_get_main_device();
@@ -544,6 +547,7 @@
     HomeDevice hd;
     if (m->stages.empty()) {
         hd.go(s->device);
+        if (req.greedy_next && toks.size() == 1 && ggml_hip_expect_greedy_next) ggml_hip_expect_greedy_next();
         if (!m->llama->is_first() || !m->llama->is_last())
             s->s->ensure_stage_rows(m->llama->hyperparameters.n_embd, toks.size());
         m->llama->evaluate(*s->s, toks, req);
@@ -1213,6 +1217,7 @@
     s->s->tokens.push_back(next);
     llm::OutputRequest req;
     const double t1 = llm::InferenceSession::now_ns();
+    req.greedy_next = true;
     model_evaluate(m, s, std::vector<llm::TokenId>{next}, req);
     llm::InferenceSession::host_ns_add(5, t1 - t0);
     llm::InferenceSession::host_ns_add(6, llm::InferenceSession::now_ns() - t1);
diff --git a/llm_amd/csrc/kernels/decode.h b/llm_amd/csrc/kernels/decode.h
--- a/llm_amd/csrc/kernels/decode.h
+++ b/llm_amd/csrc/kernels/decode.h
@@ -17,8 +17,7 @@
     __half *mem_v[BATCH_COLS_MAX];
 };
 
-__global__ void __launch_bounds__(1024) k_argmax_next(const float *__restrict__ logits, int V, DecParams *prm,
-                                                      int *__restrict__ out) {
+__device__ __forceinline__ int argmax_first_block(const float *__restrict__ logits, int V) {
     __shared__ float s_v[16];
     __shared__ int s_i[16];
     const int tid = threadIdx.x, lane = tid & 63, wave = tid >> 6;
@@ -61,10 +60,65 @@
                 bv = s_v[w];
                 bi = s_i[w];
             }
+    }
+    return bi;
+}
+__global__ void __launch_bounds__(1024) k_argmax_next(const float *__restrict__ logits, int V, DecParams *prm,
+                                                      int *__restrict__ out) {
+    const int bi = argmax_first_block(logits, V);
+    if (threadIdx.x == 0) {
         prm->token = bi;
         prm->tokens[0] = bi;
         prm->n_past = prm->n_past + 1;
         out[0] = bi;
+    }
+}
+__global__ void __launch_bounds__(256) k_kv_row_save(const DecParams *__restrict__ prm, const __half *__restrict__ mem_k,
+                                                     const __half *__restrict__ mem_v, __half *__restrict__ save, int L, int C, int Egqa) {
+    const int pos = prm->n_past;
+    if (pos < 0 || pos >= C) return;
+    const long n = (long)L * Egqa;
+    for (long i = (long)blockIdx.x * 256 + threadIdx.x; i < n; i += (long)gridDim.x * 256) {
+        const long il = i / Egqa, c = i % Egqa;
+        save[i] = mem_k[(il * C + pos) * Egqa + c];
+        save[n + i] = mem_v[(il * Egqa + c) * C + pos];
+    }
+}
+__global__ void __launch_bounds__(256) k_kv_row_restore(int pos, __half *__restrict__ mem_k, __half *__restrict__ mem_v,
+                                                        const __half *__restrict__ save, int L, int C, int Egqa) {
+    if (pos < 0 || pos >= C) return;
+    const long n = (long)L * Egqa;
+    for (long i = (long)blockIdx.x * 256 + threadIdx.x; i < n; i += (long)gridDim.x * 256) {
+        const long il = i / Egqa, c = i % Egqa;
+        mem_k[(il * C + pos) * Egqa + c] = save[i];
+        mem_v[(il * Egqa + c) * C + pos] = save[n + i];
+    }
+}
+constexpr int TOKEN_TAIL_WGS = 8;
+__global__ void __launch_bounds__(1024) k_token_tail(const float *__restrict__ logits, int V, const float *__restrict__ emb, int E,
+                                                     DecParams *prm, char *__restrict__ slot, int emb_off, int id_off) {
+    const int gtid = blockIdx.x * 1024 + threadIdx.x, total = gridDim.x * 1024;
+    float *sl = (float *)slot, *se = (float *)(slot + emb_off);
+    if (((uintptr_t)logits & 15) == 0) {
+        const int V4 = V >> 2;
+        for (int i = gtid; i < V4; i += total) ((float4 *)sl)[i] = ((const float4 *)logits)[i];
+        if (gtid < (V & 3)) sl[(V4 << 2) + gtid] = logits[(V4 << 2) + gtid];
+    } else {
+        for (int i = gtid; i < V; i += total) sl[i] = logits[i];
+    }
+    if (emb) {
+        if (((uintptr_t)emb & 15) == 0 && (E & 3) == 0)
+            for (int i = gtid; i < (E >> 2); i += total) ((float4 *)se)[i] = ((const float4 *)emb)[i];
+        else
+            for (int i = gtid; i < E; i += total) se[i] = emb[i];
+    }
+    if (blockIdx.x != 0) return;
+    const int bi = argmax_first_block(logits, V);
+    if (threadIdx.x == 0) {
+        prm->token = bi;
+        prm->tokens[0] = bi;
+        prm->n_past = prm->n_past + 1;
+        *(int *)(slot + id_off) = bi;
     }
 }
 
diff --git a/llm_amd/csrc/plan_build.inc b/llm_amd/csrc/plan_build.inc
--- a/llm_amd/csrc/plan_build.inc
+++ b/llm_amd/csrc/plan_build.inc
@@ -173,6 +173,8 @@
     c.take(p->hot, 256);
     c.take(p->logits_alt, spec ? (size_t)m.V * 4 : 0);
     c.take(p->emb_alt, spec ? E * 4 : 0);
+    c.take(p->kv_save[0], spec ? (size_t)m.L * m.Egqa * 4 : 0);
+    c.take(p->kv_save[1], spec ? (size_t)m.L * m.Egqa * 4 : 0);
     c.take(p->epoch, 256);
     const size_t units = (size_t)((m.E + 2 * m.Egqa) / 2);
     c.take(p->gran, one ? (size_t)m.L * units * 8 : 0);
diff --git a/llm_amd/csrc/plan_decode.inc b/llm_amd/csrc/plan_decode.inc
--- a/llm_amd/csrc/plan_decode.inc
+++ b/llm_amd/csrc/plan_decode.inc
@@ -135,9 +135,7 @@
     float *emb;
     char *logits;
 };
-static ResultDst plan_result_dst(const DecodePlan *p) {
-    return ResultDst{p->spec_out && p->emb_out ? p->emb_alt : p->emb_out, p->spec_out ? p->logits_alt : p->logits_out};
-}
+static ResultDst plan_result_dst(const DecodePlan *p) { return ResultDst{p->res_emb(p->out_set), p->res_logits(p->out_set)}; }
 template <class F>
 static void plan_open_rows(DecodePlan *p, LaunchCtx &cx, bool batch, double embed_bytes, F &&embed) {
     const LlamaMatch &m = p->m;
diff --git a/llm_amd/csrc/plan_run.inc b/llm_amd/csrc/plan_run.inc
--- a/llm_amd/csrc/plan_run.inc
+++ b/llm_amd/csrc/plan_run.inc
@@ -5,24 +5,49 @@
     HIP_CHECK(hipStreamEndCapture(g.stream, graph));
     HIP_CHECK(hipGraphInstantiate(exec, *graph, nullptr, nullptr, 0));
 }
+static bool emb_row_mirrored(const DecodePlan *p) {
+    const LlamaMatch &m = p->m;
+    return m.embedding && m.embedding->data && p->emb_out && (size_t)m.N * (size_t)m.E * 4 <= ((size_t)128 << 10);
+}
 static void queue_results(const DecodePlan *p) {
     const LlamaMatch &m = p->m;
+    if (m.N == 1 && !m.prompt) g.stat_result_copies += (m.logits && m.logits->backend == GGML_BACKEND_CPU ? 1 : 0) + (emb_row_mirrored(p) ? 1 : 0);
     if (m.logits && m.logits->backend == GGML_BACKEND_CPU) d2h_queue(m.logits->data, p->logits_out, (size_t)m.V * m.N * 4);
-    if (m.embedding && m.embedding->data && p->emb_out && (size_t)m.N * (size_t)m.E * 4 <= ((size_t)128 << 10))
-        d2h_queue(m.embedding->data, (const char *)p->emb_out, (size_t)m.N * (size_t)m.E * 4);
+    if (emb_row_mirrored(p)) d2h_queue(m.embedding->data, (const char *)p->emb_out, (size_t)m.N * (size_t)m.E * 4);
 }
 static void token_results_queue(DecodePlan *p) {
     if (p->m.N != 1 || p->m.prompt || !p->ferr) return;
     g.ferr_plan = p;
 }
+static void tail_deliver(const Backend::TailWait &tw) {
+    DecodePlan *tp = (DecodePlan *)tw.plan;
+    const char *sl = tp->slot[tw.q];
+    if (tw.logits_dst) memcpy(tw.logits_dst, sl, (size_t)tp->m.V * 4);
+    if (tw.emb_dst) memcpy(tw.emb_dst, sl + tp->slot_emb_off, (size_t)tp->m.E * 4);
+    if (g.spec.pending && g.spec.plan == tw.plan && g.spec.parity == (tw.q ^ 1)) {
+        g.spec.fed_id = *(const int32_t *)(sl + tp->slot_id_off);
+        g.spec.fed_id_valid = true;
+    }
+}
 static void token_finish(bool can_rerun = true) {
-    d2h_finish();
+    const Backend::TailWait tw = g.tail;
+    g.tail = Backend::TailWait{};
+    if (tw.plan) {
+        HIP_CHECK(hipEventSynchronize(((DecodePlan *)tw.plan)->slot_ev[tw.q]));
+        if (!stg.pending.empty()) d2h_finish();
+        else if (tw.staged) stg.small_off = 0;
+    } else {
+        d2h_finish();
+    }
     DecodePlan *p = (DecodePlan *)g.ferr_plan;
     g.ferr_plan = nullptr;
-    if (!p || !g.ferr_pin || !*(volatile unsigned *)g.ferr_pin) return;
+    if (!p || !g.ferr_pin || !*(volatile unsigned *)g.ferr_pin) {
+        if (tw.plan) tail_deliver(tw);
+        return;
+    }
+    spec_cancel();
     *(volatile unsigned *)g.ferr_pin = 0;
     g.stat_fused_timeouts++;
-    spec_cancel();
     static const char *what =
         "an attention workgroup of k_qkv_attn / k_attn_split_one gave up waiting for rows of its own launch (these launches "
         "need all their workgroups resident at once: is another process, or a CU mask, holding compute units of this GPU?)";
@@ -54,8 +79,11 @@
         hp.token = m.embd ? ((const int32_t *)m.embd->data)[0] : 0;
         hp.tokens[0] = hp.token;
         h2d_small((char *)p->prm, &hp, sizeof(hp));
+        g.stat_result_copies++;
+        p->prm_ahead = false;
     }
     plan_launch_decode(p, attn_variant(m, p, m.n_past + 1));
+    g.res_plan = nullptr;
     queue_results(p);
     d2h_finish();
     if (*(volatile unsigned *)g.ferr_pin) die("%s — and again on the re-run", what);
@@ -118,8 +146,19 @@
     return p;
 }
 
+static void tail_slots(DecodePlan *p) {
+    if (p->slot[0]) return;
+    p->slot_emb_off = ((size_t)p->m.V * 4 + 255) & ~(size_t)255;
+    p->slot_id_off = p->slot_emb_off + (((size_t)p->m.E * 4 + 255) & ~(size_t)255);
+    for (int q = 0; q < 2; q++) {
+        HIP_CHECK(hipHostMalloc((void **)&p->slot[q], p->slot_id_off + 256, hipHostMallocDefault));
+        HIP_CHECK(hipEventCreateWithFlags(&p->slot_ev[q], hipEventDisableTiming));
+    }
+}
 static bool try_decode_plan(ggml_cgraph *gr, bool defer_wait = false) {
     g.chain_plan = nullptr;
+    const bool greedy_next = g.greedy_hint;
+    g.greedy_hint = false;
     if (!g.opt_plan) return false;
     if (g.fused_rearm_at && g.stat_plan_tokens >= g.fused_rearm_at) {
         g.fused_rearm_at = 0;
@@ -164,21 +203,23 @@
     }
     const uint64_t t1 = now_ns();
     bool spec_hit = false;
+    int hit_q = 0;
     if (g.spec.pending) {
         g.spec.pending = false;
         const bool same = g.spec.plan == (void *)p && m.N == 1 && !m.prompt && m.embd && m.n_past == g.spec.n_past &&
                           attn_variant(m, p, m.n_past + 1) == g.spec.av && g.opt_graph && !g.timing.on;
-        if (same) {
-            HIP_CHECK(hipEventSynchronize(g.spec.tok_ev));
-            spec_hit = *g.spec.tok_pin == ((const int32_t *)m.embd->data)[0];
-        }
+        spec_hit = same && g.spec.fed_id_valid && g.spec.fed_id == ((const int32_t *)m.embd->data)[0];
+        hit_q = g.spec.parity;
         if (spec_hit) {
-            g.stat_spec_hits++;
+            if (g.opt_speculate_next) g.stat_spec_hits++;
         } else {
-            g.stat_spec_misses++;
+            if (g.opt_speculate_next) g.stat_spec_misses++;
             g.spec.cooldown = 8;
-        }
-    }
+            spec_take_back();
+        }
+        (spec_hit ? g.stat_tail_hits : g.stat_tail_misses)++;
+    }
+    if (!spec_hit) res_settle();
     DecParams hp;
     hp.n_past = m.n_past;
     hp.token = m.embd ? ((const int32_t *)m.embd->data)[0] : 0;
@@ -187,7 +228,11 @@
         hp.tokens[i] = (m.embd && i < m.N && !m.prompt) ? ((const int32_t *)m.embd->data)[i] : 0;
         if (m.wte && (hp.tokens[i] < 0 || hp.tokens[i] >= m.wte->ne[1])) die("token id %d out of range", hp.tokens[i]);
     }
-    if (!spec_hit) h2d_small((char *)p->prm, &hp, sizeof(hp));
+    if (!spec_hit) {
+        h2d_small((char *)p->prm, &hp, sizeof(hp));
+        p->prm_ahead = false;
+        if (m.N == 1 && !m.prompt) g.stat_result_copies++;
+    }
     if (m.prompt) {
         if (m.wte) {
             const int32_t *ids = (const int32_t *)m.embd->data;
@@ -230,7 +275,36 @@
         else
             plan_launch_decode(p, av);
     };
+    if (g.spec.cooldown > 0) g.spec.cooldown--;
+    const bool tail = g.opt_token_tail && (g.opt_speculate_next || greedy_next) && g.spec.cooldown == 0 && use_graph && m.N == 1 && m.logits && m.wte &&
+                      m.output && m.embd && p->logits_alt && m.n_past + 2 < m.C;
+    const auto launch_tail = [&](int v, int q) {
+        VariantGraphs &vg = p->graphs[v];
+        if (!vg.tail_exec[q]) {
+            tail_slots(p);
+            p->out_set = q;
+            capture_into(&vg.tail_graph[q], &vg.tail_exec[q], [&] {
+                hipLaunchKernelGGL(k_kv_row_save, dim3(kv_row_grid(p)), dim3(256), 0, g.stream, (const DecParams *)p->prm, (const __half *)p->mem_k,
+                                   (const __half *)p->mem_v, p->kv_save[q], (int)m.L, (int)m.C, (int)m.Egqa);
+                plan_launch_decode(p, v);
+                hipLaunchKernelGGL(k_token_tail, dim3(TOKEN_TAIL_WGS), dim3(1024), 0, g.stream, (const float *)p->res_logits(q), (int)m.V,
+                                   (size_t)m.E * 4 <= ((size_t)128 << 10) ? (const float *)p->res_emb(q) : (const float *)nullptr, (int)m.E, p->prm, p->slot[q],
+                                   (int)p->slot_emb_off, (int)p->slot_id_off);
+            });
+            p->out_set = 0;
+        }
+        HIP_CHECK(hipGraphLaunch(vg.tail_exec[q], g.stream));
+        HIP_CHECK(hipEventRecord(p->slot_ev[q], g.stream));
+        p->prm_ahead = true;
+    };
+    int tail_q = -1;
     if (spec_hit) {
+        tail_q = hit_q;
+        p->replays++;
+    } else if (tail) {
+        tail_q = 0;
+        launch_tail(av, tail_q);
+        p->replays++;
     } else if (use_graph) {
         VariantGraphs &vg = p->graphs[av];
         if (!vg.exec) capture_into(&vg.graph, &vg.exec, launch);
@@ -239,41 +313,28 @@
     } else {
         launch();
     }
-    if (spec_hit) {
-        HIP_CHECK(hipMemcpyAsync(p->logits_out, p->logits_alt, (size_t)m.V * 4, hipMemcpyDeviceToDevice, g.stream));
-        if (p->emb_out) HIP_CHECK(hipMemcpyAsync(p->emb_out, p->emb_alt, (size_t)m.E * 4, hipMemcpyDeviceToDevice, g.stream));
-    }
-    queue_results(p);
+    if (tail_q >= 0) {
+        g.stat_tail_tokens++;
+        g.tail.plan = p;
+        g.tail.q = tail_q;
+        g.tail.logits_dst = m.logits->backend == GGML_BACKEND_CPU ? m.logits->data : nullptr;
+        g.tail.emb_dst = emb_row_mirrored(p) ? m.embedding->data : nullptr;
+        g.tail.staged = !spec_hit;
+        p->cur_set = tail_q;
+        g.res_plan = p;
+    } else {
+        queue_results(p);
+    }
     token_results_queue(p);
-    if (g.spec.cooldown > 0) g.spec.cooldown--;
-    if (g.opt_speculate_next && g.spec.cooldown == 0 && use_graph && m.N == 1 && m.logits && m.wte && m.output &&
-        m.n_past + 2 < m.C && p->graphs[av].exec) {
+    if (tail) {
         const int av2 = attn_variant(m, p, m.n_past + 2);
-        {
-            if (!g.results_ev) HIP_CHECK(hipEventCreateWithFlags(&g.results_ev, hipEventDisableTiming));
-            if (!g.spec.tok_ev) {
-                HIP_CHECK(hipEventCreateWithFlags(&g.spec.tok_ev, hipEventDisableTiming));
-                HIP_CHECK(hipHostMalloc((void **)&g.spec.tok_pin, 64, hipHostMallocDefault));
-                HIP_CHECK(hipMalloc((void **)&g.spec.tok_dev, 64));
-            }
-            HIP_CHECK(hipEventRecord(g.results_ev, g.stream));
-            g.results_ev_armed = true;
-            g.results_ev_copies = stg.pending.size();
-            hipLaunchKernelGGL(k_argmax_next, dim3(1), dim3(1024), 0, g.stream, (const float *)p->logits_out, (int)m.V, p->prm, g.spec.tok_dev);
-            HIP_CHECK(hipMemcpyAsync(g.spec.tok_pin, g.spec.tok_dev, 4, hipMemcpyDeviceToHost, g.stream));
-            HIP_CHECK(hipEventRecord(g.spec.tok_ev, g.stream));
-            VariantGraphs &vg2 = p->graphs[av2];
-            if (!vg2.spec_exec) {
-                p->spec_out = true;
-                capture_into(&vg2.spec_graph, &vg2.spec_exec, [&] { plan_launch_decode(p, av2); });
-                p->spec_out = false;
-            }
-            HIP_CHECK(hipGraphLaunch(vg2.spec_exec, g.stream));
-            g.spec.pending = true;
-            g.spec.plan = p;
-            g.spec.n_past = m.n_past + 1;
-            g.spec.av = av2;
-        }
+        launch_tail(av2, tail_q ^ 1);
+        g.spec.pending = true;
+        g.spec.plan = p;
+        g.spec.n_past = m.n_past + 1;
+        g.spec.av = av2;
+        g.spec.parity = tail_q ^ 1;
+        g.spec.fed_id_valid = false;
     }
     const uint64_t t2 = now_ns();
     g.ns_match += t1 - t0;
@@ -302,16 +363,24 @@
 
 static int decode_greedy_chain(ggml_cgraph *last, int n, int32_t *out_tokens, float *last_logits) {
     finish_pending();
-    if (g.spec.pending) {
-        spec_cancel();
-        return -1;
-    }
     DecodePlan *p = (DecodePlan *)g.chain_plan;
     if (!p || g.chain_graph != last || n < 1) return -1;
     bool live = false;
     for (auto *q : g_plans) live = live || q == p;
     const LlamaMatch &m = p->m;
     if (!live || m.N != 1 || !m.logits || !m.wte || m.n_past + 1 + n > m.C) return -1;
+    if (p->prm_ahead) {
+        if (!m.embd) return -1;
+        DecParams hp;
+        memset(&hp, 0, sizeof(hp));
+        hp.n_past = m.n_past;
+        hp.token = hp.tokens[0] = ((const int32_t *)m.embd->data)[0];
+        h2d_small((char *)p->prm, &hp, sizeof(hp));
+        p->prm_ahead = false;
+    }
+    spec_cancel();
+    const float *first_logits = (const float *)plan_cur_logits(p);
+    g.res_plan = nullptr;
     if (p->chain_cap < n) {
         if (p->chain_out) (void)hipFree(p->chain_out);
         p->chain_cap = std::max(n, 256);
@@ -322,6 +391,10 @@
     int i0 = 0;
     if (use_graph && g.opt_chain_k > 1) {
         const int K = g.opt_chain_k;
+        if ((const char *)first_logits != p->logits_out) {
+            HIP_CHECK(hipMemcpyAsync(p->logits_out, first_logits, (size_t)m.V * 4, hipMemcpyDeviceToDevice, g.stream));
+            first_logits = (const float *)p->logits_out;
+        }
         const auto long_at = [&](int i) { return attn_variant(m, p, m.n_past + 1 + i + 1) != AV_SHORT; };
         while (i0 + K <= n && !long_at(i0 + K - 1)) {
             if (!p->exec_chain || p->chain_k != K) {
@@ -343,8 +416,8 @@
         }
     }
     for (int i = i0; i < n; i++) {
-        hipLaunchKernelGGL(k_argmax_next, dim3(1), dim3(1024), 0, g.stream, (const float *)p->logits_out, (int)m.V, p->prm,
-                           p->chain_out + i);
+        hipLaunchKernelGGL(k_argmax_next, dim3(1), dim3(1024), 0, g.stream, i == 0 ? first_logits : (const float *)p->logits_out, (int)m.V,
+                           p->prm, p->chain_out + i);
         const int av = attn_variant(m, p, m.n_past + 1 + i + 1);
         if (av != AV_SPLIT && fused_qkv_shape(m, av_heads_split(av)).ok) g.stat_fused_tokens++;
         if (av >= AV_FUSED2) g.stat_fused_heads_tokens++;
@@ -374,6 +447,7 @@
     finish_pending();
     spec_cancel();
     g.chain_plan = nullptr;
+    res_settle();
     if (PrepMatch *pm = (PrepMatch *)g.prep) pm->gr = nullptr;
     if (!g.opt_plan || !g.opt_plan_batch) return -1;
     const uint64_t t0 = now_ns();
diff --git a/llm_amd/csrc/plan_shapes.inc b/llm_amd/csrc/plan_shapes.inc
--- a/llm_amd/csrc/plan_shapes.inc
+++ b/llm_amd/csrc/plan_shapes.inc
@@ -41,12 +41,12 @@
 struct VariantGraphs {
     hipGraph_t graph = nullptr;
     hipGraphExec_t exec = nullptr, exec2 = nullptr;
-    hipGraph_t spec_graph = nullptr;
-    hipGraphExec_t spec_exec = nullptr;
+    hipGraph_t tail_graph[2] = {nullptr, nullptr};
+    hipGraphExec_t tail_exec[2] = {nullptr, nullptr};
     void drop() {
-        for (hipGraphExec_t e : {exec, exec2, spec_exec})
+        for (hipGraphExec_t e : {exec, exec2, tail_exec[0], tail_exec[1]})
             if (e) (void)hipGraphExecDestroy(e);
-        for (hipGraph_t gr : {graph, spec_graph})
+        for (hipGraph_t gr : {graph, tail_graph[0], tail_graph[1]})
             if (gr) (void)hipGraphDestroy(gr);
         *this = VariantGraphs{};
     }
@@ -104,7 +104,15 @@
     char *logits_out = nullptr;
     char *logits_alt = nullptr;
     float *emb_alt = nullptr;
-    bool spec_out = false;
+    int cur_set = 0;
+    int out_set = 0;
+    char *res_logits(int q) const { return q ? logits_alt : logits_out; }
+    float *res_emb(int q) const { return emb_out ? (q ? emb_alt : emb_out) : nullptr; }
+    char *slot[2] = {nullptr, nullptr};
+    hipEvent_t slot_ev[2] = {nullptr, nullptr};
+    size_t slot_emb_off = 0, slot_id_off = 0;
+    __half *kv_save[2] = {nullptr, nullptr};
+    bool prm_ahead = false;
     int *chain_out = nullptr;
     int *chain_ring = nullptr;
     int chain_cap = 0;
@@ -143,14 +151,62 @@
     drop_plan_graphs(p);
     if (p->chain_ring) (void)hipFree(p->chain_ring);
     if (p->pool) (void)hipFree(p->pool);
+    for (int q = 0; q < 2; q++) {
+        if (p->slot[q]) (void)hipHostFree(p->slot[q]);
+        if (p->slot_ev[q]) (void)hipEventDestroy(p->slot_ev[q]);
+    }
+    if (g.res_plan == (void *)p) g.res_plan = nullptr;
     delete p;
+}
+char *result_dev_ptr(const ggml_tensor *t) {
+    char *d = dev_ptr(t);
+    DecodePlan *p = (DecodePlan *)g.res_plan;
+    if (!p || p->cur_set != 1 || !p->logits_alt) return d;
+    const size_t lb = (size_t)p->m.V * 4, eb = (size_t)p->m.E * 4;
+    if (p->logits_out && d >= p->logits_out && d < p->logits_out + lb) return p->logits_alt + (d - p->logits_out);
+    if (p->emb_out && d >= (char *)p->emb_out && d < (char *)p->emb_out + eb) return (char *)p->emb_alt + (d - (char *)p->emb_out);
+    return d;
+}
+static void res_settle() {
+    DecodePlan *p = nullptr;
+    for (auto *q : g_plans)
+        if ((void *)q == g.res_plan) p = q;
+    g.res_plan = nullptr;
+    if (!p || p->cur_set != 1 || !p->logits_alt || !p->logits_out) return;
+    HIP_CHECK(hipMemcpyAsync(p->logits_out, p->logits_alt, (size_t)p->m.V * 4, hipMemcpyDeviceToDevice, g.stream));
+    if (p->emb_out) HIP_CHECK(hipMemcpyAsync(p->emb_out, p->emb_alt, (size_t)p->m.E * 4, hipMemcpyDeviceToDevice, g.stream));
+    p->cur_set = 0;
+}
+static inline char *plan_cur_logits(const DecodePlan *p) { return p->res_logits(g.res_plan == (const void *)p ? p->cur_set : 0); }
+static inline int kv_row_grid(const DecodePlan *p) { return (int)std::min<int64_t>(256, ((int64_t)p->m.L * p->m.Egqa + 255) / 256); }
+static void spec_take_back() {
+    DecodePlan *p = nullptr;
+    for (auto *q : g_plans)
+        if ((void *)q == g.spec.plan) p = q;
+    if (!p || !p->kv_save[g.spec.parity] || !p->mem_k) return;
+    hipLaunchKernelGGL(k_kv_row_restore, dim3(kv_row_grid(p)), dim3(256), 0, g.stream, g.spec.n_past, p->mem_k, p->mem_v,
+                       (const __half *)p->kv_save[g.spec.parity], (int)p->m.L, (int)p->m.C, (int)p->m.Egqa);
+    HIP_CHECK(hipGetLastError());
 }
 void spec_cancel() {
     if (!g.spec.pending) return;
     g.spec.pending = false;
+    spec_take_back();
     if (g.stream) HIP_CHECK(hipStreamSynchronize(g.stream));
 }
+void spec_guard_read(const char *d, size_t n) {
+    if (!g.spec.pending) return;
+    DecodePlan *p = nullptr;
+    for (auto *q : g_plans)
+        if ((void *)q == g.spec.plan) p = q;
+    if (!p || !p->mem_k) return;
+    const size_t kvb = (size_t)p->m.L * p->m.C * p->m.Egqa * 2;
+    const char *k = (const char *)p->mem_k, *v = (const char *)p->mem_v;
+    if ((d < k + kvb && k < d + n) || (d < v + kvb && v < d + n)) spec_cancel();
+}
+void finish_pending();
 void drop_all_plans() {
+    finish_pending();
     spec_cancel();
     if (g_plans.empty()) return;
     if (g.stream) HIP_CHECK(hipStreamSynchronize(g.stream));
diff --git a/llm_amd/ggml.py b/llm_amd/ggml.py
--- a/llm_amd/ggml.py
+++ b/llm_amd/ggml.py
@@ -252,6 +252,9 @@
     "ggml_hip_graph_compute_begin": (C.c_int, [C.c_void_p]),
     "ggml_hip_graph_prepare": (C.c_int, [C.c_void_p]),
     "ggml_hip_graph_compute_end": (None, []),
+    "ggml_hip_expect_greedy_next": (None, []),
+    "ggml_hip_debug_token_tail": (C.c_int, [C.c_void_p, C.c_int, C.c_void_p, C.c_int, C.c_int, C.c_int, C.c_void_p, C.c_void_p,
+                                            C.c_void_p, C.c_void_p, C.c_void_p]),
     "ggml_hip_bench_plan_class": (C.c_int, [C.c_int, C.c_int, C.POINTER(C.c_double), C.POINTER(C.c_int64),
                                             C.POINTER(C.c_double)]),
     "ggml_hip_comm_unique_id": (C.c_int, [C.c_void_p]),
```

Result: faster. 864.1 (median of 6 runs) (+2.6%).
